# pygda-team/pygda

Measured on AMD Instinct MI355X. Metric: edges_aggregated_per_sec, higher is better.
Workload: dtype f32

## Files before the change

### include/gda_hip.h

```cpp
#ifndef GDA_HIP_H
#define GDA_HIP_H

#include <stddef.h>
#include <stdint.h>

#ifdef __cplusplus
extern "C" {
#endif

#define GDA_OK 0
#define GDA_E_NULL (-1)
#define GDA_E_SIZE (-2)
#define GDA_E_WORKSPACE (-3)
#define GDA_E_UNSUPPORTED (-4)
#define GDA_E_ALIAS (-5)
#define GDA_E_RCCL (-100)

typedef void* gda_stream_t;

int gda_abi_version(void);
const char* gda_status_string(int status);

size_t gda_graph_workspace_bytes(int64_t E, int64_t N);
int gda_build_csr_norm(const int64_t* src, const int64_t* dst, const float* w,
// ... 47 lines not shown

int gda_spmm_csr_interior_kstep_f32(const int32_t* rowptr, const int32_t* colidx, const float* val,
                                    int64_t n_rows, int64_t n_int, int64_t d, int K, int transposed,
                                    const float* x, float* y, float* tmp, float* sacc, const float* bias,
                                    gda_stream_t stream);

int gda_interior_max_rows(void);
int gda_interior_max_width(void);
size_t gda_interior_plan_bytes(void);
size_t gda_interior_kstep_lds_workspace_bytes(int64_t n_int, int64_t d);
int gda_interior_plan_build(const int32_t* rowptr, const int32_t* colidx, const float* val,
                            const int64_t* n_int_dev, void* plan, size_t plan_bytes, int64_t* status_dev,
                            gda_stream_t stream);
int gda_interior_kstep_lds_f32(const int32_t* rowptr, const int32_t* colidx, const float* val,
                               int64_t n_rows, int64_t n_int, int64_t d, int K, int transposed,
                               const void* plan, const float* x, float* y, const float* bias,
                               void* workspace, size_t workspace_bytes, gda_stream_t stream);
int gda_interior_kstep_lds_act_f32(const int32_t* rowptr, const int32_t* colidx, const float* val,
                                   int64_t n_rows, int64_t n_int, int64_t d, int K, const void* plan,
                                   const float* x, float* y0, float* y1, const float* bias,
                                   float p, uint64_t seed, const int64_t* step_dev, uint32_t site0, uint32_t site1,
                                   void* workspace, size_t workspace_bytes, gda_stream_t stream);

int gda_kstep_max_rows(void);
size_t gda_kstep_plan_bytes(int slots);
int gda_kstep_plan_host(const int32_t* rowptr_host, const int32_t* colidx_host, const float* val_host,
                        int64_t n_rows, void* plan_host, size_t plan_bytes);
int gda_kstep_plan_host_ex(const int32_t* rowptr_host, const int32_t* colidx_host, const float* val_host,
                           int64_t n_rows, int flags, void* plan_host, size_t plan_bytes);
int gda_kstep_lds_f32(const void* plan, int slots, int64_t n_rows, int64_t d, int K,
                      const float* x, int64_t ldx, int x_colmajor, float* y, int64_t ldy, int y_colmajor,
                      const float* bias, float* colsum, float* scratchT, gda_stream_t stream);
int gda_kstep_lds_colmajor_f32(const void* plan, int slots, int64_t n_rows, int64_t d, int K,
                               const float* xT, int64_t ldx, float* yT, int64_t ldy,
                               const float* bias, float* colsum, gda_stream_t stream);
int gda_transpose_f32(const float* in, int64_t ldi, float* out, int64_t ldo, int64_t rows, int64_t cols,
                      gda_stream_t stream);

int gda_gat_fwd_f32(const int32_t* rowptr, const int32_t* colidx, int64_t n_rows, int64_t d,
                    const float* h, const float* a_src, const float* a_dst, float slope,
                    float* out, float* alpha, gda_stream_t stream);
int gda_gat_bwd_f32(const int32_t* rowptr, const int32_t* colidx,
                    const int32_t* t_rowptr, const int32_t* t_colidx, const int32_t* t_to_fwd,
                    int64_t n_rows, int64_t d, const float* h, const float* a_src, const float* a_dst,
                    float slope, const float* alpha, const float* gout,
                    float* gh, float* ga_src, float* ga_dst, float* dpre, gda_stream_t stream);

int gda_faconv_fwd_f32(const int32_t* rowptr, const int32_t* colidx, const float* val, int64_t n_rows, int64_t d,
                       const float* h, int64_t ldh, const float* s, const float* r, int64_t ldsr, float eps,
                       const float* bias, float* out, int64_t ldo, float* t, gda_stream_t stream);
int gda_faconv_bwd_f32(const int32_t* rowptr, const int32_t* colidx, const float* val,
                       const int32_t* t_rowptr, const int32_t* t_colidx, const int32_t* t_to_fwd,
                       int64_t n_rows, int64_t d, const float* h, int64_t ldh, const float* t,
                       const float* gout, int64_t ldgo, float eps, float* gh, int64_t ldgh, float* gs,
                       float* gr, int64_t ldgsr, float* dpre, gda_stream_t stream);

size_t gda_closs_workspace_bytes(int64_t n, int64_t c);
int gda_closs_fwd_f32(const float* z, int64_t ldz, const int64_t* y, int64_t n, int64_t c, float* loss, float* weight,
                      float* factor, void* workspace, size_t workspace_bytes, gda_stream_t stream);
int gda_closs_bwd_f32(const float* z, int64_t ldz, const int64_t* y, const float* factor, const float* gloss,
                      int64_t n, int64_t c, float* gz, int64_t ldgz, gda_stream_t stream);
size_t gda_colstats_workspace_bytes(int64_t n, int64_t d);
int gda_weighted_moments_f32(const float* x, int64_t ldx, const float* w, int64_t n, int64_t d, float* mean,
                             float* std, void* workspace, size_t workspace_bytes, gda_stream_t stream);
int gda_std_mean_match_fwd_f32(const float* x, int64_t ldx, int64_t n, int64_t d, const float* mean_s,
                               const float* std_s, float* loss, float* mean_t, float* std_t, float* coef,
                               void* workspace, size_t workspace_bytes, gda_stream_t stream);
int gda_std_mean_match_bwd_f32(const float* x, int64_t ldx, int64_t n, int64_t d, const float* mean_t,
                               const float* coef, const float* gloss, float* gx, int64_t ldgx, gda_stream_t stream);

#define GDA_ACDNE_MAX_HALF 128
size_t gda_acdne_ppmi_workspace_bytes(int64_t n);
int gda_acdne_ppmi_f32(const int32_t* rowptr, const int32_t* col, const float* cnt, int64_t n, int step, float* pval,
                       float* buf_a, float* buf_b, float* buf_c, void* workspace, size_t workspace_bytes,
                       gda_stream_t stream);
int gda_acdne_xnei_f32(const float* na, int64_t n, int64_t ld, const int32_t* xrowptr, const int32_t* xcol,
                       const float* xval, int64_t f, float* out, int64_t ldo, gda_stream_t stream);
size_t gda_acdne_prox_workspace_bytes(int64_t h);
int gda_acdne_prox_f32(const float* ppmi_s, int64_t ld_s, int64_t ns, const float* ppmi_t, int64_t ld_t, int64_t nt,
                       const int64_t* pidx, const float* z, int64_t h, int64_t e, float pair_weight, double* loss,
                       float* gz, void* workspace, size_t workspace_bytes, gda_stream_t stream);
size_t gda_acdne_heads_workspace_bytes(int64_t h, int64_t e, int64_t c);
int gda_acdne_heads_f32(const float* z, const float* gprox, int64_t h, int64_t e, int64_t c, const float* const* w,
                        const int64_t* y, int64_t ny, const int64_t* rows, const float* alpha, const double* prox,
                        float pair_weight, float* dz, float* const* g, double* loss, double* loss_acc,
                        void* workspace, size_t workspace_bytes, gda_stream_t stream);
int gda_acdne_predict_f32(const float* z, int64_t n, int64_t e, const float* wc, const float* bc, int64_t c,
                          float* prob, gda_stream_t stream);

size_t gda_dmgnn_prox_workspace_bytes(int64_t h, int64_t e);
int gda_dmgnn_prox_f32(const float* ppmi_s, int64_t ld_s, int64_t ns, const float* ppmi_t, int64_t ld_t, int64_t nt,
                       const int64_t* pidx, const float* z, int64_t h, int64_t e, float pair_weight, double* loss,
                       float* gz, float* a_blocks, void* workspace, size_t workspace_bytes, gda_stream_t stream);
size_t gda_dmgnn_heads_workspace_bytes(int64_t h, int64_t e, int64_t c);
int gda_dmgnn_heads_f32(const float* z, const float* gprox, const float* a_blocks, int64_t h, int64_t e, int64_t c,
                        const float* const* w, const int64_t* y, int64_t ny, const int64_t* rows, const float* alpha,
                        const double* prox, float pair_weight, float* dz, float* const* g, double* loss,
                        double* loss_acc, void* workspace, size_t workspace_bytes, gda_stream_t stream);
size_t gda_dmgnn_predict_workspace_bytes(int64_t n, int64_t c);
int gda_dmgnn_predict_f32(const float* z, int64_t n, int64_t e, const float* wc, const float* bc, int64_t c,
                          const float* ppmi, int64_t ld, float* out, void* workspace, size_t workspace_bytes,
                          gda_stream_t stream);

size_t gda_mmd_workspace_bytes(int times, int64_t n, int64_t d);
int gda_mmd_fwd_f32(const float* src, int64_t ld_src, const float* tgt, int64_t ld_tgt,
                    int64_t d, const int64_t* src_idx, const int64_t* tgt_idx,
                    int times, int64_t n, float kernel_mul, int kernel_num, float fix_sigma,
                    float* loss, float* bandwidth, float* l2_saved,
                    void* workspace, size_t workspace_bytes, gda_stream_t stream);
int gda_mmd_bwd_f32(const float* src, int64_t ld_src, const float* tgt, int64_t ld_tgt,
                    int64_t d, const int64_t* src_idx, const int64_t* tgt_idx,
                    int times, int64_t n, float kernel_mul, int kernel_num,
                    const float* bandwidth, const float* l2_saved, const float* grad_loss,
                    float* grad_rows, void* workspace, size_t workspace_bytes, gda_stream_t stream);
int gda_mmd_fwd_ex_f32(const float* src, int64_t ld_src, const float* tgt, int64_t ld_tgt,
                       int64_t d, const int64_t* src_idx, const int64_t* tgt_idx,
                       int times, int64_t n, float kernel_mul, int kernel_num, float fix_sigma,
                       float scale, const float* add, float* loss, float* bandwidth, float* l2_saved,
                       void* workspace, size_t workspace_bytes, gda_stream_t stream);
int gda_mmd_fwd_gather_f32(const float* src, int64_t ld_src, const float* tgt, int64_t ld_tgt,
                           int64_t d, const int64_t* src_idx, const int64_t* tgt_idx,
                           int times, int64_t n, float kernel_mul, int kernel_num, float fix_sigma,
                           float scale, const float* add, float* rows_src, float* rows_tgt,
                           float* loss, float* bandwidth, float* l2_saved,
                           void* workspace, size_t workspace_bytes, gda_stream_t stream);
int gda_mmd_bwd_ex_f32(const float* src, int64_t ld_src, const float* tgt, int64_t ld_tgt,
                       int64_t d, const int64_t* src_idx, const int64_t* tgt_idx,
                       int times, int64_t n, float kernel_mul, int kernel_num,
                       const float* bandwidth, const float* l2_saved, const float* grad_loss, float scale,
                       float* grad_rows,
                       const int32_t* sel_s_rowptr, const int32_t* sel_s_col, int64_t n_src_rows, float* gsrc,
                       const int32_t* sel_t_rowptr, const int32_t* sel_t_col, int64_t n_tgt_rows, float* gtgt,
                       void* workspace, size_t workspace_bytes, gda_stream_t stream);

int gda_mmd_fused_nseg(int times, int64_t n, int64_t d, float kernel_mul, int kernel_num);
int gda_mmd_fused_layout(int times, int64_t n, int64_t d, int64_t* out, int n_out);
int gda_mmd_fused_fwd_f32(const float* src, int64_t ld_src, const float* tgt, int64_t ld_tgt,
                          int64_t d, const int64_t* src_idx, const int64_t* tgt_idx,
                          int times, int64_t n, float kernel_mul, int kernel_num, float fix_sigma,
                          float scale, const float* add, float* rows_src, float* rows_tgt,
                          float* loss, float* bandwidth, float* grad_part, int nseg,
                          void* workspace, size_t workspace_bytes, gda_stream_t stream);
int gda_mmd_fused_bwd_f32(const float* grad_part, int nseg, int times, int64_t n, int64_t d,
                          const float* grad_loss, float scale, float* grad_rows,
                          const int32_t* sel_s_rowptr, const int32_t* sel_s_col, int64_t n_src_rows, float* gsrc,
                          const int32_t* sel_t_rowptr, const int32_t* sel_t_col, int64_t n_tgt_rows, float* gtgt,
                          gda_stream_t stream);
int gda_mmd_fused_bwd_mask_f32(const float* grad_part, int nseg, int times, int64_t n, int64_t d,
                               const float* grad_loss, float scale, float* grad_rows,
                               const int32_t* sel_s_rowptr, const int32_t* sel_s_col, int64_t n_src_rows, float* gsrc,
                               const int32_t* sel_t_rowptr, const int32_t* sel_t_col, int64_t n_tgt_rows, float* gtgt,
                               const float* mask_src, float p_src, const float* mask_tgt, float p_tgt,
                               gda_stream_t stream);

int gda_mmd_chunked_plan(int times, int64_t n, int64_t d, float kernel_mul, int kernel_num, int64_t* out, int n_out);
size_t gda_mmd_chunked_workspace_bytes(int times, int64_t n, int64_t d);
int gda_mmd_chunked_fwd_f32(const float* src, int64_t ld_src, const float* tgt, int64_t ld_tgt,
                            int64_t d, const int64_t* src_idx, const int64_t* tgt_idx,
                            int times, int64_t n, float kernel_mul, int kernel_num, float fix_sigma,
                            float scale, const float* add, float* rows_src, float* rows_tgt, int64_t ld_rows,
                            float* loss, float* bandwidth, float* grad_part, int64_t ld_part, int nseg,
                            void* workspace, size_t workspace_bytes, gda_stream_t stream);
int gda_mmd_fused_bwd_ld_f32(const float* grad_part, int64_t ld_part, int nseg, int times, int64_t n, int64_t d,
                             const float* grad_loss, float scale, float* grad_rows,
                             const int32_t* sel_s_rowptr, const int32_t* sel_s_col, int64_t n_src_rows, float* gsrc,
                             const int32_t* sel_t_rowptr, const int32_t* sel_t_col, int64_t n_tgt_rows, float* gtgt,
                             const float* mask_src, float p_src, const float* mask_tgt, float p_tgt,
                             gda_stream_t stream);

int gda_grl_disc_ce_fwd_f32(const float* feat_src, int64_t ld_src, int64_t n_src,
                            const float* feat_tgt, int64_t ld_tgt, int64_t n_tgt,
                            int64_t h, int C, const float* W, const float* b,
                            const int64_t* labels, float* probs, float* loss,
                            void* workspace, size_t workspace_bytes, gda_stream_t stream);
int gda_grl_disc_ce_bwd_f32(const float* feat_src, int64_t ld_src, int64_t n_src,
                            const float* feat_tgt, int64_t ld_tgt, int64_t n_tgt,
                            int64_t h, int C, const float* W, const int64_t* labels,
                            const float* probs, const float* grad_loss, float alpha,
                            float* gfeat_src, float* gfeat_tgt, float* gW, float* gb,
                            void* workspace, size_t workspace_bytes, gda_stream_t stream);
size_t gda_grl_disc_workspace_bytes(int64_t n_rows, int64_t h, int C);

size_t gda_grl_mlp_ce_workspace_bytes(int64_t h, int64_t a);
int gda_grl_mlp_ce_fwd_f32(const float* es, int64_t ld_s, int64_t n_s, const float* et, int64_t ld_t, int64_t n_t,
                           int64_t h, int64_t a, const float* W1, const float* b1, const float* W2, const float* b2,
                           float dropout_p, uint64_t seed, const int64_t* step, uint32_t site,
                           float* losses, void* workspace, size_t workspace_bytes, gda_stream_t stream);
int gda_grl_mlp_ce_bwd_f32(const float* es, int64_t ld_s, int64_t n_s, const float* et, int64_t ld_t, int64_t n_t,
                           int64_t h, int64_t a, const float* W1, const float* b1, const float* W2, const float* b2,
                           float dropout_p, uint64_t seed, const int64_t* step, uint32_t site,
                           const float* grad_losses, int grad_stride, float alpha, const float* alpha_dev,
                           float* g_es, float* g_et, float* gW1, float* gb1, float* gW2, float* gb2,
                           void* workspace, size_t workspace_bytes, gda_stream_t stream);
int gda_mlp_head_fwd_f32(int head, const float* es, int64_t ld_s, int64_t n_s, const float* et, int64_t ld_t, int64_t n_t,
                         int64_t h, int64_t a, const float* W1, const float* b1, const float* W2, const float* b2,
                         float dropout_p, uint64_t seed, const int64_t* step, uint32_t site,
                         float* losses, void* workspace, size_t workspace_bytes, gda_stream_t stream);
int gda_mlp_head_bwd_f32(int head, const float* es, int64_t ld_s, int64_t n_s, const float* et, int64_t ld_t, int64_t n_t,
                         int64_t h, int64_t a, const float* W1, const float* b1, const float* W2, const float* b2,
                         float dropout_p, uint64_t seed, const int64_t* step, uint32_t site,
                         const float* grad_losses, int grad_stride, float alpha, const float* alpha_dev,
                         float* g_es, float* g_et, float* gW1, float* gb1, float* gW2, float* gb2,
                         void* workspace, size_t workspace_bytes, gda_stream_t stream);

size_t gda_lsgan_head_workspace_bytes(int64_t a);
int gda_lsgan_head_fwd_f32(const float* Z, int64_t ldz, int64_t rows, int64_t a, const float* w2, const float* b2,
                           float target, float* pre, float* loss, void* workspace, size_t workspace_bytes,
                           gda_stream_t stream);
int gda_lsgan_head_bwd_f32(const float* Z, int64_t ldz, int64_t rows, int64_t a, const float* w2, const float* pre,
                           float target, const float* grad_loss, float* gZ, int64_t ldg, float* gw2, float* gb2,
                           void* workspace, size_t workspace_bytes, gda_stream_t stream);

size_t gda_wgan_critic_workspace_bytes(int64_t n_s, int64_t n_t, int64_t n_i, int h, int a);
int gda_wgan_critic_f32(const float* es, int64_t n_s, const float* et, int64_t n_t, int h,
                        const int32_t* idx_s, const int32_t* idx_t, const float* alpha, int64_t n_i,
                        const float* W1, const float* b1, const float* w2, const float* b2, int a,
                        float dropout_p, uint64_t seed, const int64_t* step, uint32_t site,
                        float gp_weight, float* loss, float* gW1, float* gb1, float* gw2, float* gb2,
                        void* workspace, size_t workspace_bytes, gda_stream_t stream);

int gda_relu_dropout_fwd_f32(const float* x, float* y, int64_t n, float p, uint64_t seed,
                             const int64_t* step, uint32_t site, gda_stream_t stream);
int gda_relu_dropout_bwd_f32(const float* gy, const float* y, float* gx, int64_t n, float p,
                             gda_stream_t stream);
int gda_relu_dropout_tiled_fwd_f32(const float* x, int64_t period, int64_t copies, float* y, float p, uint64_t seed,
                                   const int64_t* step, uint32_t site, gda_stream_t stream);
int gda_relu_dropout_fwd_cm_f32(const float* xT, int64_t ldT, float* y, int64_t n, int64_t d, float p,
                               uint64_t seed, const int64_t* step, uint32_t site, gda_stream_t stream);
int gda_relu_dropout_bwd_cm_f32(const float* gy, const float* y, float* gxT, int64_t ldT, int64_t n, int64_t d,
                               float p, gda_stream_t stream);

int gda_relu_dropout_pair_fwd_f32(const float* x, float* y, int64_t n, int64_t d, float p, uint64_t seed,
                                  const int64_t* step, uint32_t site_a, uint32_t site_b, gda_stream_t stream);
size_t gda_relu_dropout_pair_workspace_bytes(int64_t d);
int gda_relu_dropout_pair_bwd_f32(const float* gy, const float* y, float* gx, int64_t n, int64_t d, float p,
                                  float* colsum, void* workspace, size_t workspace_bytes, gda_stream_t stream);
int gda_stack2_f32(const float* a, const float* b, float* out, int64_t half_elems, gda_stream_t stream);
int gda_relu_dropout_bwd2_f32(const float* ga, const float* gb, const float* y, float* gx, int64_t half_elems,
                              float p, gda_stream_t stream);

size_t gda_colsum_workspace_bytes(int64_t n, int64_t d);
int gda_colsum_f32(const float* x, int64_t ldx, int64_t n, int64_t d, float* out, void* workspace,
                   size_t workspace_bytes, gda_stream_t stream);

size_t gda_mixup_combine_workspace_bytes(int64_t n, int64_t h);
int gda_mixup_combine_fwd_f32(const float* P, const float* Pb, const float* CC, int first, const float* bias,
                              const int64_t* perm, int64_t n, int64_t h, float lam, float p, uint64_t seed,
                              const int64_t* step, uint32_t site_x, uint32_t site_m, float* XX, uint8_t* mask,
                              gda_stream_t stream);
int gda_mixup_combine_bwd_f32(const float* gXX, const float* XX, const uint8_t* mask, const int64_t* inv_perm,
                              int first, int64_t n, int64_t h, float lam, float p, float* gP, float* gPb,
                              float* gCC, float* gbias, void* workspace, size_t workspace_bytes,
                              gda_stream_t stream);

int gda_gather_rows_f32(const float* x, int64_t ldx, int64_t d, const int64_t* idx,
                        int64_t n_out, float* out, int64_t ldo, gda_stream_t stream);

int gda_segment_mean_fwd_f32(const float* x, int64_t ldx, const int64_t* seg_ptr, int64_t G, int64_t d,
                             float* out, int64_t ldo, gda_stream_t stream);
int gda_segment_mean_bwd_f32(const float* gout, int64_t ldg, const int64_t* seg_ptr, const int64_t* batch,
                             int64_t n, int64_t d, float* gx, int64_t ldx, gda_stream_t stream);

typedef struct gda_sampler gda_sampler;
int gda_sampler_create(const int64_t* src_host, const int64_t* dst_host, int64_t E, int64_t N,
                       gda_sampler** out);
void gda_sampler_destroy(gda_sampler* s);
int gda_sampler_set_threads(gda_sampler* s, int workers);
int gda_sampler_sample(gda_sampler* s, const int64_t* seeds_host, int64_t n_seeds,
                       const int32_t* fanouts, int L, uint64_t rng_seed,
                       int64_t* n_nodes_out, int64_t* n_edges_out);
int gda_sampler_fetch(const gda_sampler* s, int64_t* nodes_out, int64_t* esrc_out,
                      int64_t* edst_out);
int gda_sampler_csr_norm(const gda_sampler* s, int32_t* rowptr, int32_t* colidx, float* val,
                         int32_t* t_rowptr, int32_t* t_colidx, float* t_val);

size_t gda_dsampler_graph_workspace_bytes(int64_t E, int64_t N);
int gda_dsampler_build_graph(const int64_t* src, const int64_t* dst, int64_t E, int64_t N,
                             int64_t* in_ptr, int32_t* in_src, int32_t* status,
                             void* workspace, size_t workspace_bytes, gda_stream_t stream);
int gda_dsampler_caps(int64_t n_seeds, const int32_t* fanouts_host, int L, int64_t max_in_degree, int64_t E,
                      int64_t N, int64_t* node_cap, int64_t* edge_cap);
size_t gda_dsampler_workspace_bytes(int64_t n_seeds, const int32_t* fanouts_host, int L, int64_t max_in_degree,
                                    int64_t E, int64_t N);
int gda_dsampler_sample(const int64_t* in_ptr, const int32_t* in_src, int64_t N, int64_t E, int64_t max_in_degree,
                        const int64_t* seeds, int64_t n_seeds, const int32_t* fanouts_host, int L, uint64_t rng_seed,
                        int64_t* nodes, int64_t* esrc, int64_t* edst,
                        int32_t* rowptr, int32_t* colidx, float* val,
                        int32_t* t_rowptr, int32_t* t_colidx, float* t_val,
                        int64_t* counts, void* workspace, size_t workspace_bytes, gda_stream_t stream);

int gda_copy_from_pinned(void* dst, const void* src_host, size_t bytes, gda_stream_t stream);

int gda_event_create(void** event_out);
int gda_event_destroy(void* event);
int gda_event_record(void* event, gda_stream_t stream);
int gda_event_synchronize(void* event);
int gda_stream_wait_event(gda_stream_t stream, void* event);
int gda_dsampler_batch(const int64_t* in_ptr, const int32_t* in_src, int64_t N, int64_t E, int64_t max_in_degree,
                       const int64_t* seeds, int64_t n_seeds, int64_t* seeds_dev,
                       const int32_t* fanouts_host, int L, uint64_t rng_seed,
                       int64_t* nodes, int64_t* esrc, int64_t* edst,
                       int32_t* rowptr, int32_t* colidx, float* val,
                       int32_t* t_rowptr, int32_t* t_colidx, float* t_val,
                       int64_t* counts, void* plan_fwd, void* plan_bwd, size_t plan_bytes,
                       int64_t* counts_host, void* wait_event, void* done_event,
                       void* workspace, size_t workspace_bytes, gda_stream_t stream);
// ... 301 lines not shown
```

### pygda_amd/_lib.py

```python
import ctypes
import os
from ctypes import c_char_p, c_float, c_int, c_int64, c_size_t, c_void_p

import torch

HERE = os.path.dirname(os.path.abspath(__file__))
LIB_PATH = os.path.join(HERE, "libgda_hip.so")

class _P(c_void_p):

    @classmethod
    def from_param(cls, obj):
        if isinstance(obj, torch.Tensor):
            return c_void_p(obj.data_ptr())
        if obj is None:
            return None
        if isinstance(obj, str):
            raise TypeError("a str is not a pointer argument")
        return c_void_p.from_param(obj)


_SIGNATURES = {
    "gda_abi_version": (c_int, []),
    "gda_status_string": (c_char_p, [c_int]),
    "gda_graph_workspace_bytes": (c_size_t, [c_int64, c_int64]),
    "gda_build_csr_norm": (c_int, [_P, _P, _P, c_int64, c_int64, c_float, c_int, c_int, c_int,
                                   _P, _P, _P, _P, _P, _P, _P, c_size_t, _P]),
    "gda_build_csr_norm_map": (c_int, [_P, _P, _P, c_int64, c_int64, c_float, c_int, c_int, c_int,
                                       _P, _P, _P, _P, _P, _P, _P, _P, c_size_t, _P]),
    "gda_gat_fwd_f32": (c_int, [_P, _P, c_int64, c_int64, _P, _P, _P, c_float, _P, _P, _P]),
    "gda_gat_bwd_f32": (c_int, [_P, _P, _P, _P, _P, c_int64, c_int64, _P, _P, _P, c_float, _P, _P,
                                _P, _P, _P, _P, _P]),
    "gda_faconv_fwd_f32": (c_int, [_P, _P, _P, c_int64, c_int64, _P, c_int64, _P, _P, c_int64, c_float, _P, _P,
                                   c_int64, _P, _P]),
    "gda_faconv_bwd_f32": (c_int, [_P, _P, _P, _P, _P, _P, c_int64, c_int64, _P, c_int64, _P, _P, c_int64, c_float,
                                   _P, c_int64, _P, _P, c_int64, _P, _P]),
    "gda_closs_workspace_bytes": (c_size_t, [c_int64, c_int64]),
    "gda_closs_fwd_f32": (c_int, [_P, c_int64, _P, c_int64, c_int64, _P, _P, _P, _P, c_size_t, _P]),
    "gda_closs_bwd_f32": (c_int, [_P, c_int64, _P, _P, _P, c_int64, c_int64, _P, c_int64, _P]),
    "gda_colstats_workspace_bytes": (c_size_t, [c_int64, c_int64]),
    "gda_weighted_moments_f32": (c_int, [_P, c_int64, _P, c_int64, c_int64, _P, _P, _P, c_size_t, _P]),
    "gda_std_mean_match_fwd_f32": (c_int, [_P, c_int64, c_int64, c_int64, _P, _P, _P, _P, _P, _P, _P, c_size_t, _P]),
    "gda_std_mean_match_bwd_f32": (c_int, [_P, c_int64, c_int64, c_int64, _P, _P, _P, _P, c_int64, _P]),
    "gda_acdne_ppmi_workspace_bytes": (c_size_t, [c_int64]),
    "gda_acdne_ppmi_f32": (c_int, [_P, _P, _P, c_int64, c_int, _P, _P, _P, _P, _P, c_size_t, _P]),
    "gda_acdne_xnei_f32": (c_int, [_P, c_int64, c_int64, _P, _P, _P, c_int64, _P, c_int64, _P]),
    "gda_acdne_prox_workspace_bytes": (c_size_t, [c_int64]),
    "gda_acdne_prox_f32": (c_int, [_P, c_int64, c_int64, _P, c_int64, c_int64, _P, _P, c_int64, c_int64, c_float, _P, _P,
                                   _P, c_size_t, _P]),
    "gda_acdne_heads_workspace_bytes": (c_size_t, [c_int64, c_int64, c_int64]),
    "gda_acdne_heads_f32": (c_int, [_P, _P, c_int64, c_int64, c_int64, _P, _P, c_int64, _P, _P, _P, c_float, _P, _P, _P,
                                    _P, _P, c_size_t, _P]),
    "gda_acdne_predict_f32": (c_int, [_P, c_int64, c_int64, _P, _P, c_int64, _P, _P]),
    "gda_dmgnn_prox_workspace_bytes": (c_size_t, [c_int64, c_int64]),
    "gda_dmgnn_prox_f32": (c_int, [_P, c_int64, c_int64, _P, c_int64, c_int64, _P, _P, c_int64, c_int64, c_float, _P, _P,
                                   _P, _P, c_size_t, _P]),
    "gda_dmgnn_heads_workspace_bytes": (c_size_t, [c_int64, c_int64, c_int64]),
    "gda_dmgnn_heads_f32": (c_int, [_P, _P, _P, c_int64, c_int64, c_int64, _P, _P, c_int64, _P, _P, _P, c_float, _P, _P,
                                    _P, _P, _P, c_size_t, _P]),
    "gda_dmgnn_predict_workspace_bytes": (c_size_t, [c_int64, c_int64]),
    "gda_dmgnn_predict_f32": (c_int, [_P, c_int64, c_int64, _P, _P, c_int64, _P, c_int64, _P, _P, c_size_t, _P]),
    "gda_asn_recon_chunks": (c_int, [c_int64]),
    "gda_asn_recon_workspace_bytes": (c_size_t, [c_int64, c_int64]),
    "gda_asn_recon_f32": (c_int, [_P, c_int64, c_int64, c_int64, _P, _P, _P, _P, _P, _P, c_float, c_float, _P, _P,
                                  c_int64, _P, c_size_t, _P]),
    "gda_asn_rows_workspace_bytes": (c_size_t, [c_int64, c_int64, c_int64]),
    "gda_asn_kld_f32": (c_int, [_P, c_int64, _P, c_int64, c_int64, c_int64, ctypes.c_double, _P, _P, _P, _P, c_size_t,
                                _P]),
    "gda_asn_reparam_fwd_f32": (c_int, [_P, c_int64, _P, c_int64, c_int64, c_int64, _P, c_int, ctypes.c_uint64, _P,
                                        ctypes.c_uint32, _P, _P]),
    "gda_asn_reparam_bwd_f32": (c_int, [_P, _P, _P, c_int64, c_int64, c_int64, _P, _P]),
    "gda_asn_dropout_fwd_f32": (c_int, [_P, c_int64, c_float, ctypes.c_uint64, _P, ctypes.c_uint32, _P, _P, _P]),
    "gda_asn_mask_mul_f32": (c_int, [_P, _P, c_int64, _P, _P]),
    "gda_asn_diff_fwd_f32": (c_int, [_P, c_int64, _P, c_int64, c_int64, c_int64, c_int64, _P, _P, _P, c_size_t, _P]),
    "gda_asn_diff_bwd_f32": (c_int, [_P, c_int64, _P, c_int64, c_int64, c_int64, c_int64, _P, _P, _P, _P, _P]),
    "gda_asn_ppmi_count": (c_int, [_P, c_int64, c_int64, _P, _P]),
    "gda_asn_ppmi_fill": (c_int, [_P, c_int64, c_int64, _P, c_int64, _P, _P, _P, _P, _P]),
    "gda_jhgda_prox_workspace_bytes": (c_size_t, [c_int64, c_int64]),
    "gda_jhgda_prox_f32": (c_int, [_P, c_int64, c_int64, c_int64, _P, _P, _P, _P, _P, c_int64, _P, _P, c_int64, _P,
                                   c_int64, _P, c_size_t, _P]),
    "gda_jhgda_pool_rows_fwd_f32": (c_int, [_P, c_int64, c_int64, c_int64, _P, c_int64, _P, _P, _P]),
    "gda_jhgda_pool_rows_bwd_f32": (c_int, [_P, c_int64, _P, c_int64, _P, c_int64, _P, c_int64, c_int64, _P, c_int64,
                                            _P]),
    "gda_csr_to_coo": (c_int, [_P, _P, c_int64, c_int64, _P, _P, _P]),
    "gda_spmm_csr_f32": (c_int, [_P, _P, _P, c_int64, c_int64, _P, c_int64, _P, c_int64, _P, _P]),
    "gda_spmm_csr_tout_f32": (c_int, [_P, _P, _P, c_int64, c_int64, _P, c_int64, _P, c_int64, _P, _P]),
    "gda_spmm_csr_kstep_f32": (c_int, [_P, _P, _P, c_int64, c_int64, c_int, _P, c_int64, _P, c_int64,
                                       _P, _P, _P]),
    "gda_spmm_csr_interior_kstep_f32": (c_int, [_P, _P, _P, c_int64, c_int64, c_int64, c_int, c_int, _P, _P, _P, _P, _P, _P]),
    "gda_interior_max_rows": (c_int, []),
    "gda_interior_max_width": (c_int, []),
    "gda_interior_plan_bytes": (c_size_t, []),
    "gda_interior_kstep_lds_workspace_bytes": (c_size_t, [c_int64, c_int64]),
    "gda_interior_plan_build": (c_int, [_P, _P, _P, _P, _P, c_size_t, _P, _P]),
    "gda_interior_kstep_lds_f32": (c_int, [_P, _P, _P, c_int64, c_int64, c_int64, c_int, c_int, _P, _P, _P, _P, _P,
                                           c_size_t, _P]),
    "gda_interior_kstep_lds_act_f32": (c_int, [_P, _P, _P, c_int64, c_int64, c_int64, c_int, _P, _P, _P, _P, _P,
                                               ctypes.c_float, ctypes.c_uint64, _P, ctypes.c_uint32, ctypes.c_uint32,
                                               _P, c_size_t, _P]),
    "gda_row_split_workspace_bytes": (c_size_t, [c_int64]),
    "gda_row_split_build": (c_int, [_P, c_int64, ctypes.c_int32, _P, _P, _P, _P, _P, c_size_t, _P]),
    "gda_spmm_csr_split_f32": (c_int, [_P, _P, _P, c_int64, c_int64, c_int, _P, c_int64, _P, c_int64,
                                       _P, _P, _P, _P]),
    "gda_mmd_workspace_bytes": (c_size_t, [c_int, c_int64, c_int64]),
    "gda_mmd_fwd_f32": (c_int, [_P, c_int64, _P, c_int64, c_int64, _P, _P, c_int, c_int64, c_float,
                                c_int, c_float, _P, _P, _P, _P, c_size_t, _P]),
    "gda_mmd_bwd_f32": (c_int, [_P, c_int64, _P, c_int64, c_int64, _P, _P, c_int, c_int64, c_float,
                                c_int, _P, _P, _P, _P, _P, c_size_t, _P]),
    "gda_mmd_fwd_ex_f32": (c_int, [_P, c_int64, _P, c_int64, c_int64, _P, _P, c_int, c_int64, c_float, c_int, c_float,
                                   c_float, _P, _P, _P, _P, _P, c_size_t, _P]),
    "gda_mmd_fwd_gather_f32": (c_int, [_P, c_int64, _P, c_int64, c_int64, _P, _P, c_int, c_int64, c_float, c_int, c_float,
                                       c_float, _P, _P, _P, _P, _P, _P, _P, c_size_t, _P]),
    "gda_mmd_bwd_ex_f32": (c_int, [_P, c_int64, _P, c_int64, c_int64, _P, _P, c_int, c_int64, c_float, c_int,
                                   _P, _P, _P, c_float, _P, _P, _P, c_int64, _P, _P, _P, c_int64, _P,
                                   _P, c_size_t, _P]),
    "gda_mmd_fused_nseg": (c_int, [c_int, c_int64, c_int64, c_float, c_int]),
    "gda_mmd_fused_layout": (c_int, [c_int, c_int64, c_int64, _P, c_int]),
    "gda_mmd_fused_fwd_f32": (c_int, [_P, c_int64, _P, c_int64, c_int64, _P, _P, c_int, c_int64, c_float, c_int, c_float,
                                      c_float, _P, _P, _P, _P, _P, _P, c_int, _P, c_size_t, _P]),
    "gda_mmd_fused_bwd_f32": (c_int, [_P, c_int, c_int, c_int64, c_int64, _P, c_float, _P,
                                      _P, _P, c_int64, _P, _P, _P, c_int64, _P, _P]),
    "gda_mmd_fused_bwd_mask_f32": (c_int, [_P, c_int, c_int, c_int64, c_int64, _P, c_float, _P,
                                           _P, _P, c_int64, _P, _P, _P, c_int64, _P, _P, c_float, _P, c_float, _P]),
    "gda_copy_from_pinned": (c_int, [_P, _P, c_size_t, _P]),
    "gda_softmax_entropy_fwd_f32": (c_int, [_P, c_int64, c_int64, c_int, c_float, _P, _P, c_size_t, _P]),
    "gda_softmax_entropy_bwd_f32": (c_int, [_P, c_int64, c_int64, c_int, c_float, _P, _P, c_int64, _P]),
    "gda_mmd_chunked_plan": (c_int, [c_int, c_int64, c_int64, c_float, c_int, _P, c_int]),
    "gda_mmd_chunked_workspace_bytes": (c_size_t, [c_int, c_int64, c_int64]),
    "gda_mmd_chunked_fwd_f32": (c_int, [_P, c_int64, _P, c_int64, c_int64, _P, _P, c_int, c_int64, c_float, c_int, c_float,
                                        c_float, _P, _P, _P, c_int64, _P, _P, _P, c_int64, c_int, _P, c_size_t, _P]),
    "gda_mmd_fused_bwd_ld_f32": (c_int, [_P, c_int64, c_int, c_int, c_int64, c_int64, _P, c_float, _P,
                                         _P, _P, c_int64, _P, _P, _P, c_int64, _P, _P, c_float, _P, c_float, _P]),
    "gda_gemm_tall_fwd_ex_f32": (c_int, [c_int64, c_int64, c_int64, _P, c_int64, _P, _P, c_int64, _P, c_int64, _P, c_int,
                                         c_float, ctypes.c_uint64, _P, ctypes.c_uint32, ctypes.c_uint32, _P]),
    "gda_gemm_tall_wgrad_gather_f32": (c_int, [c_int64, c_int64, _P, c_int64, _P, c_int64, _P, _P, c_int64, _P, _P, c_size_t, _P]),
    "gda_gemm_nn_mask_f32": (c_int, [c_int64, c_int64, c_int64, _P, c_int64, _P, c_int64, _P, c_int64, _P, c_int64, c_float, _P]),
    "gda_gemm_act_cm_f32": (c_int, [c_int64, c_int64, c_int64, _P, c_int64, _P, c_int64, _P, _P, c_int64, c_float,
                                    ctypes.c_uint64, _P, ctypes.c_uint32, _P]),
    "gda_gemm_act_cm_bwd_f32": (c_int, [c_int64, c_int64, c_int64, _P, c_int64, _P, c_int64, _P, c_float, _P, _P, _P, c_size_t,
                                        _P]),
    "gda_gemm_skinny_act_cm_f32": (c_int, [c_int64, c_int64, c_int64, _P, c_int64, _P, c_int64, _P, c_int64, c_float,
                                           ctypes.c_uint64, _P, ctypes.c_uint32, _P]),
    "gda_grl_disc_workspace_bytes": (c_size_t, [c_int64, c_int64, c_int]),
    "gda_grl_mlp_ce_workspace_bytes": (c_size_t, [c_int64, c_int64]),
    "gda_lsgan_head_workspace_bytes": (c_size_t, [c_int64]),
    "gda_lsgan_head_fwd_f32": (c_int, [_P, c_int64, c_int64, c_int64, _P, _P, c_float, _P, _P, _P, c_size_t, _P]),
    "gda_lsgan_head_bwd_f32": (c_int, [_P, c_int64, c_int64, c_int64, _P, _P, c_float, _P, _P, c_int64, _P, _P,
                                       _P, c_size_t, _P]),
    "gda_grl_mlp_ce_fwd_f32": (c_int, [_P, c_int64, c_int64, _P, c_int64, c_int64, c_int64, c_int64, _P, _P, _P, _P,
                                       c_float, ctypes.c_uint64, _P, ctypes.c_uint32, _P, _P, c_size_t, _P]),
    "gda_grl_mlp_ce_bwd_f32": (c_int, [_P, c_int64, c_int64, _P, c_int64, c_int64, c_int64, c_int64, _P, _P, _P, _P,
                                       c_float, ctypes.c_uint64, _P, ctypes.c_uint32, _P, c_int, c_float, _P,
                                       _P, _P, _P, _P, _P, _P, _P, c_size_t, _P]),
    "gda_mlp_head_fwd_f32": (c_int, [c_int, _P, c_int64, c_int64, _P, c_int64, c_int64, c_int64, c_int64, _P, _P, _P, _P,
                                     c_float, ctypes.c_uint64, _P, ctypes.c_uint32, _P, _P, c_size_t, _P]),
    "gda_mlp_head_bwd_f32": (c_int, [c_int, _P, c_int64, c_int64, _P, c_int64, c_int64, c_int64, c_int64, _P, _P, _P, _P,
                                     c_float, ctypes.c_uint64, _P, ctypes.c_uint32, _P, c_int, c_float, _P,
                                     _P, _P, _P, _P, _P, _P, _P, c_size_t, _P]),
    "gda_grl_disc_ce_fwd_f32": (c_int, [_P, c_int64, c_int64, _P, c_int64, c_int64, c_int64, c_int,
                                        _P, _P, _P, _P, _P, _P, c_size_t, _P]),
    "gda_grl_disc_ce_bwd_f32": (c_int, [_P, c_int64, c_int64, _P, c_int64, c_int64, c_int64, c_int,
                                        _P, _P, _P, _P, c_float, _P, _P, _P, _P, _P, c_size_t, _P]),
    "gda_relu_dropout_fwd_f32": (c_int, [_P, _P, c_int64, c_float, ctypes.c_uint64, _P, ctypes.c_uint32, _P]),
    "gda_relu_dropout_bwd_f32": (c_int, [_P, _P, _P, c_int64, c_float, _P]),
    "gda_relu_dropout_tiled_fwd_f32": (c_int, [_P, c_int64, c_int64, _P, c_float, ctypes.c_uint64, _P, ctypes.c_uint32, _P]),
    "gda_gather_rows_f32": (c_int, [_P, c_int64, c_int64, _P, c_int64, _P, c_int64, _P]),
    "gda_segment_mean_fwd_f32": (c_int, [_P, c_int64, _P, c_int64, c_int64, _P, c_int64, _P]),
    "gda_segment_mean_bwd_f32": (c_int, [_P, c_int64, _P, _P, c_int64, c_int64, _P, c_int64, _P]),
    "gda_sampler_create": (c_int, [_P, _P, c_int64, c_int64, ctypes.POINTER(c_void_p)]),
    "gda_sampler_destroy": (None, [_P]),
    "gda_sampler_set_threads": (c_int, [_P, c_int]),
    "gda_sampler_sample": (c_int, [_P, _P, c_int64, _P, c_int, ctypes.c_uint64,
                                   ctypes.POINTER(c_int64), ctypes.POINTER(c_int64)]),
    "gda_sampler_fetch": (c_int, [_P, _P, _P, _P]),
    "gda_sampler_csr_norm": (c_int, [_P, _P, _P, _P, _P, _P, _P]),
    "gda_dsampler_graph_workspace_bytes": (c_size_t, [c_int64, c_int64]),
    "gda_dsampler_build_graph": (c_int, [_P, _P, c_int64, c_int64, _P, _P, _P, _P, c_size_t, _P]),
    "gda_dsampler_caps": (c_int, [c_int64, _P, c_int, c_int64, c_int64, c_int64, _P, _P]),
    "gda_dsampler_workspace_bytes": (c_size_t, [c_int64, _P, c_int, c_int64, c_int64, c_int64]),
    "gda_dsampler_sample": (c_int, [_P, _P, c_int64, c_int64, c_int64, _P, c_int64, _P, c_int, ctypes.c_uint64,
                                    _P, _P, _P, _P, _P, _P, _P, _P, _P, _P, _P, c_size_t, _P]),
    "gda_event_create": (c_int, [_P]),
    "gda_event_destroy": (c_int, [_P]),
    "gda_event_record": (c_int, [_P, _P]),
    "gda_event_synchronize": (c_int, [_P]),
    "gda_stream_wait_event": (c_int, [_P, _P]),
    "gda_dsampler_batch": (c_int, [_P, _P, c_int64, c_int64, c_int64, _P, c_int64, _P, _P, c_int, ctypes.c_uint64,
                                   _P, _P, _P, _P, _P, _P, _P, _P, _P, _P, _P, _P, c_size_t, _P, _P, _P, _P, c_size_t, _P]),
    "gda_dsampler_batch_ex": (c_int, [_P, _P, c_int64, c_int64, c_int64, _P, c_int64, _P, _P, c_int, ctypes.c_uint64,
                                      _P, _P, _P, _P, _P, _P, _P, _P, _P, _P, _P, _P, c_size_t, _P, _P, _P, c_int64, _P,
                                      c_size_t, _P]),
    "gda_selection_csr_host": (c_int, [_P, c_int, c_int64, c_int64, c_int64, c_int64, _P, _P]),
    "gda_ppmi_build_host": (c_int, [_P, _P, c_int64, c_int64, c_int, c_int, ctypes.c_uint64,
                                    ctypes.POINTER(c_void_p)]),
    "gda_ppmi_workspace_bytes": (c_size_t, [c_int64, c_int64, c_int, c_int]),
    "gda_ppmi_build": (c_int, [_P, _P, c_int64, c_int64, c_int, c_int, ctypes.c_uint64, _P, _P, _P, _P, _P,
                               c_size_t, _P]),
    "gda_edge_list_size": (c_int64, [_P]),
    "gda_edge_list_fetch": (c_int, [_P, _P, _P, _P]),
    "gda_edge_list_destroy": (None, [_P]),
    "gda_spmm_csr_axpby_f32": (c_int, [_P, _P, _P, c_int64, c_int64, _P, c_int64, _P, c_int64, c_float, c_float,
                                       _P, c_int64, c_float, _P, _P, _P]),
    "gda_kstep_max_rows": (c_int, []),
    "gda_kstep_plan_bytes": (c_size_t, [c_int]),
    "gda_kstep_plan_host": (c_int, [_P, _P, _P, c_int64, _P, c_size_t]),
    "gda_kstep_plan_host_ex": (c_int, [_P, _P, _P, c_int64, c_int, _P, c_size_t]),
    "gda_kstep_lds_f32": (c_int, [_P, c_int, c_int64, c_int64, c_int, _P, c_int64, c_int, _P, c_int64, c_int,
                                  _P, _P, _P, _P]),
    "gda_kstep_lds_colmajor_f32": (c_int, [_P, c_int, c_int64, c_int64, c_int, _P, c_int64, _P, c_int64, _P, _P, _P]),
    "gda_relu_dropout_pair_fwd_f32": (c_int, [_P, _P, c_int64, c_int64, c_float, ctypes.c_uint64, _P, ctypes.c_uint32,
                                              ctypes.c_uint32, _P]),
    "gda_relu_dropout_pair_workspace_bytes": (ctypes.c_size_t, [c_int64]),
    "gda_relu_dropout_pair_bwd_f32": (c_int, [_P, _P, _P, c_int64, c_int64, c_float, _P, _P, ctypes.c_size_t, _P]),
    "gda_stack2_f32": (c_int, [_P, _P, _P, c_int64, _P]),
    "gda_relu_dropout_bwd2_f32": (c_int, [_P, _P, _P, _P, c_int64, ctypes.c_float, _P]),
    "gda_colsum_workspace_bytes": (ctypes.c_size_t, [c_int64, c_int64]),
    "gda_colsum_f32": (c_int, [_P, c_int64, c_int64, c_int64, _P, _P, ctypes.c_size_t, _P]),
    "gda_softmax_nll_fwd_ex_f32": (c_int, [_P, c_int64, _P, c_int64, c_int, _P, _P, _P, ctypes.c_size_t, _P]),
    "gda_mixup_combine_workspace_bytes": (ctypes.c_size_t, [c_int64, c_int64]),
    "gda_mixup_combine_fwd_f32": (c_int, [_P, _P, _P, c_int, _P, _P, c_int64, c_int64, c_float, c_float, ctypes.c_uint64,
                                          _P, ctypes.c_uint32, ctypes.c_uint32, _P, _P, _P]),
    "gda_mixup_combine_bwd_f32": (c_int, [_P, _P, _P, _P, c_int, c_int64, c_int64, c_float, c_float, _P, _P, _P, _P, _P,
                                          ctypes.c_size_t, _P]),
    "gda_relu_dropout_fwd_cm_f32": (c_int, [_P, c_int64, _P, c_int64, c_int64, c_float, ctypes.c_uint64, _P,
                                           ctypes.c_uint32, _P]),
    "gda_relu_dropout_bwd_cm_f32": (c_int, [_P, _P, _P, c_int64, c_int64, c_int64, c_float, _P]),
    "gda_transpose_f32": (c_int, [_P, c_int64, _P, c_int64, c_int64, c_int64, _P]),
    "gda_wgan_critic_workspace_bytes": (c_size_t, [c_int64, c_int64, c_int64, c_int, c_int]),
    "gda_wgan_critic_f32": (c_int, [_P, c_int64, _P, c_int64, c_int, _P, _P, _P, c_int64, _P, _P, _P, _P, c_int,
                                    c_float, ctypes.c_uint64, _P, ctypes.c_uint32, c_float, _P, _P, _P, _P, _P,
                                    _P, c_size_t, _P]),
    "gda_wgan_critic_adam_f32": (c_int, [_P, c_int64, _P, c_int64, c_int, _P, _P, _P, c_int64, c_int,
                                         c_float, ctypes.c_uint64, _P, ctypes.c_uint32, c_float, _P, _P,
                                         c_float, c_float, c_float, c_float, c_float, _P, c_size_t, _P]),
    "gda_laplacian_workspace_bytes": (c_size_t, [c_int64]),
    "gda_laplacian_fwd_f32": (c_int, [_P, _P, c_int64, c_int, _P, c_int64, _P, _P, _P, c_size_t, _P]),
    "gda_laplacian_bwd_f32": (c_int, [_P, _P, _P, _P, c_int64, c_int, _P, c_int64, _P, _P, _P, c_int64, _P]),
    "gda_softmax_nll_workspace_bytes": (c_size_t, []),
    "gda_softmax_nll_fwd_f32": (c_int, [_P, c_int64, _P, c_int64, c_int, _P, _P, c_size_t, _P]),
    "gda_softmax_nll_bwd_f32": (c_int, [_P, c_int64, _P, c_int64, c_int, _P, _P, c_int64, _P]),
    "gda_softmax_nll_fwd_nv_f32": (c_int, [_P, c_int64, _P, c_int64, c_int, _P, _P, _P, _P, c_size_t, _P]),
    "gda_softmax_nll_bwd_nv_f32": (c_int, [_P, c_int64, _P, c_int64, c_int, _P, _P, _P, c_int64, _P]),
    "gda_gemm_workspace_bytes": (c_size_t, [c_int, c_int64, c_int64, c_int64]),
    "gda_gemm_f32": (c_int, [c_int, c_int64, c_int64, c_int64, _P, c_int64, _P, c_int64, _P, c_int64,
                             _P, c_size_t, _P]),
    "gda_gemm_ex_f32": (c_int, [c_int, c_int64, c_int64, c_int64, _P, c_int64, _P, c_int64, _P, c_int64, _P, _P,
                                _P, c_size_t, _P]),
    "gda_gemm_skinny_workspace_bytes": (c_size_t, [c_int, c_int64, c_int64, c_int64]),
    "gda_gemm_skinny_f32": (c_int, [c_int, c_int64, c_int64, c_int64, _P, c_int64, _P, c_int64, _P, c_int64, _P, _P,
                                    _P, c_size_t, _P]),
    "gda_gemm_tall_workspace_bytes": (c_size_t, [c_int, c_int64, c_int64, c_int64]),
    "gda_gemm_tall_f32": (c_int, [c_int, c_int64, c_int64, c_int64, _P, c_int64, _P, c_int64, _P, c_int64, _P, _P,
                                  _P, c_size_t, _P]),
    "gda_attention_workspace_bytes": (c_size_t, [c_int64, c_int64]),
    "gda_attention_fuse_fwd_f32": (c_int, [c_int, _P, _P, c_int64, c_int64, _P, _P, _P, c_int64, _P, _P]),
    "gda_attention_fuse_bwd_f32": (c_int, [c_int, _P, _P, c_int64, c_int64, _P, _P, _P, c_int64, _P, _P, _P, _P, c_size_t, _P]),
    "gda_adam_multi_f32": (c_int, [_P, c_int, c_float, c_float, c_float, c_float, c_float, _P]),
    "gda_adam_multi_ex_f32": (c_int, [_P, c_int, c_float, c_float, c_float, c_float, c_float, c_int, _P]),
    "gda_adam_multi_sum_f32": (c_int, [_P, _P, c_int, c_float, c_float, c_float, c_float, c_float, c_int, _P]),
    "gda_step_bump": (c_int, [_P, _P, c_int, _P]),
    "gda_rccl_load": (c_int, [ctypes.c_char_p]),
    "gda_comm_unique_id": (c_int, [_P, c_size_t]),
    "gda_comm_init_rank": (c_int, [_P, c_size_t, c_int, c_int, ctypes.POINTER(c_void_p)]),
    "gda_comm_destroy": (c_int, [_P]),
    "gda_allreduce_f32": (c_int, [_P, c_int64, _P, _P]),
    "gda_allgather_f32": (c_int, [_P, _P, c_int64, _P, _P]),
    "gda_two_hop_host": (c_int, [_P, _P, c_int64, c_int64, c_int, c_int, ctypes.POINTER(c_void_p)]),
    "gda_sepa_workspace_bytes": (c_size_t, [c_int64, c_int64, c_int64]),
    "gda_sepa_stats_f32": (c_int, [_P, c_int64, c_int64, _P, _P, _P, _P]),
    "gda_sepa_group_sum_f32": (c_int, [_P, c_int64, _P, _P, c_int64, c_int64, c_int64, c_int, c_float, _P, _P, _P, _P,
                                       c_size_t, _P]),
    "gda_sepa_class_mean_bwd_f32": (c_int, [_P, _P, _P, _P, c_int64, c_int64, c_int64, c_float, _P, _P]),
    "gda_sepa_mid_f32": (c_int, [_P, _P, _P, _P, c_int64, c_int64, c_int64, _P, _P, _P, _P]),
    "gda_sepa_unbias_rows_f32": (c_int, [_P, _P, _P, _P, c_int64, c_int64, c_int64, _P, _P]),
    "gda_sepa_row_weight_f32": (c_int, [_P, _P, c_int64, c_int64, _P, _P]),
    "gda_sepa_center_rows_bwd_f32": (c_int, [_P, _P, _P, _P, _P, _P, c_int64, c_int64, c_int64, _P, _P, _P]),
# ... 138 lines not shown
```

### pygda_amd/csrc/gda_act.hip

```cpp
#include "gda_common.h"
#include "gda_dropout.h"

namespace {

constexpr int TB = 256;

__global__ void __launch_bounds__(TB)
k_relu_dropout_fwd(const float* __restrict__ x, float* __restrict__ y, int64_t n, float p, float scale,
                   uint64_t seed, const int64_t* __restrict__ step, uint32_t site, int64_t period) {
    const uint64_t st = (uint64_t)step[0];
    const uint32_t thresh = dropout_thresh(p);
    const int64_t quads = (n + 3) / 4;
    for (int64_t q = (int64_t)blockIdx.x * TB + threadIdx.x; q < quads; q += (int64_t)gridDim.x * TB) {
        uint32_t r[4];
        dropout_draw(seed, st, site, (uint64_t)q, r);
        const int64_t i = q * 4;
        if (period) {
            const float4 v = *reinterpret_cast<const float4*>(x + i % period);
            *reinterpret_cast<float4*>(y + i) = relu_keep(v, r, thresh, scale);
        } else if (i + 3 < n) {
            const float4 v = *reinterpret_cast<const float4*>(x + i);
            *reinterpret_cast<float4*>(y + i) = relu_keep(v, r, thresh, scale);
        } else {
            for (int e = 0; e < 4 && i + e < n; ++e)
// ... 256 lines not shown
            const float v0 = x[i * ldx + tc], v1 = x[(i + stride) * ldx + tc];
            const float v2 = x[(i + 2 * stride) * ldx + tc], v3 = x[(i + 3 * stride) * ldx + tc];
            const float v4 = x[(i + 4 * stride) * ldx + tc], v5 = x[(i + 5 * stride) * ldx + tc];
            const float v6 = x[(i + 6 * stride) * ldx + tc], v7 = x[(i + 7 * stride) * ldx + tc];
            a0 += v0; a1 += v1; a2 += v2; a3 += v3;
            a0 += v4; a1 += v5; a2 += v6; a3 += v7;
        }
        for (; i < n; i += stride) a0 += x[i * ldx + tc];
        red[tr * d + tc] = (a0 + a1) + (a2 + a3);
    }
    __syncthreads();
    for (int w = slots >> 1; w > 0; w >>= 1) {
        if (tr < w) red[tr * d + tc] += red[(tr + w) * d + tc];
        __syncthreads();
    }
    if (tr == 0) out[tc] = red[tc];
}

int colsum_blocks(int64_t n, int d) {
    const int rpb = d <= TB ? TB / d : 1;
    const int64_t g = gda_cdiv(n, (int64_t)rpb * 8);
    return (int)(g > COLSUM_BLOCKS ? COLSUM_BLOCKS : (g < 1 ? 1 : g));
}

unsigned grid_for(int64_t n) {
    int64_t g = gda_cdiv((n + 3) / 4, TB);
    if (g > 256 * 8) g = 256 * 8;
    return (unsigned)(g < 1 ? 1 : g);
}

}

extern "C" int gda_relu_dropout_fwd_f32(const float* x, float* y, int64_t n, float p, uint64_t seed,
                                        const int64_t* step, uint32_t site, gda_stream_t stream) {
    if (n < 0 || !(p >= 0.f && p < 1.f)) return GDA_E_SIZE;
    if (n == 0) return GDA_OK;
    if (!x || !y || !step) return GDA_E_NULL;
    if (((uintptr_t)x | (uintptr_t)y) % 16 != 0) return GDA_E_UNSUPPORTED;
    k_relu_dropout_fwd<<<grid_for(n), TB, 0, (hipStream_t)stream>>>(x, y, n, p, 1.f / (1.f - p), seed, step, site, 0);
    GDA_LAUNCH_CHECK();
    return GDA_OK;
}

extern "C" int gda_relu_dropout_tiled_fwd_f32(const float* x, int64_t period, int64_t copies, float* y, float p, uint64_t seed,
                                              const int64_t* step, uint32_t site, gda_stream_t stream) {
    if (period < 0 || copies < 0 || !(p >= 0.f && p < 1.f) || period % 4 != 0) return GDA_E_SIZE;
    if (period == 0 || copies == 0) return GDA_OK;
    if (!x || !y || !step) return GDA_E_NULL;
    if (((uintptr_t)x | (uintptr_t)y) % 16 != 0) return GDA_E_UNSUPPORTED;
    const int64_t n = period * copies;
    k_relu_dropout_fwd<<<grid_for(n), TB, 0, (hipStream_t)stream>>>(x, y, n, p, 1.f / (1.f - p), seed, step, site, period);
    GDA_LAUNCH_CHECK();
    return GDA_OK;
}

extern "C" int gda_relu_dropout_bwd_f32(const float* gy, const float* y, float* gx, int64_t n, float p,
                                        gda_stream_t stream) {
    if (n < 0 || !(p >= 0.f && p < 1.f)) return GDA_E_SIZE;
    if (n == 0) return GDA_OK;
    if (!gy || !y || !gx) return GDA_E_NULL;
    if (((uintptr_t)gy | (uintptr_t)y | (uintptr_t)gx) % 16 != 0) return GDA_E_UNSUPPORTED;
    k_relu_dropout_bwd<<<grid_for(n), TB, 0, (hipStream_t)stream>>>(gy, y, gx, n, 1.f / (1.f - p));
    GDA_LAUNCH_CHECK();
    return GDA_OK;
}

extern "C" int gda_relu_dropout_fwd_cm_f32(const float* xT, int64_t ldT, float* y, int64_t n, int64_t d, float p,
                                          uint64_t seed, const int64_t* step, uint32_t site, gda_stream_t stream) {
    if (n < 0 || d < 0 || n >= INT32_MAX || d >= INT32_MAX || ldT < n || !(p >= 0.f && p < 1.f)) return GDA_E_SIZE;
    if (n == 0 || d == 0) return GDA_OK;
    if (!xT || !y || !step) return GDA_E_NULL;
    if (d % 4 != 0 || (uintptr_t)y % 16 != 0) return GDA_E_UNSUPPORTED;
    const dim3 grid((unsigned)gda_cdiv(n, TT), (unsigned)gda_cdiv(d, TT));
    if (grid.y > 65535) return GDA_E_SIZE;
    GDA_UNLESS_SKIPPED("k_relu_dropout_fwd_T") k_relu_dropout_fwd_T<<<grid, TB, 0, (hipStream_t)stream>>>(xT, ldT, y, (int)n, (int)d, p, 1.f / (1.f - p), seed,
                                                               step, site);
    GDA_LAUNCH_CHECK();
    return GDA_OK;
}

extern "C" int gda_relu_dropout_bwd_cm_f32(const float* gy, const float* y, float* gxT, int64_t ldT, int64_t n,
                                          int64_t d, float p, gda_stream_t stream) {
    if (n < 0 || d < 0 || n >= INT32_MAX || d >= INT32_MAX || ldT < n || !(p >= 0.f && p < 1.f)) return GDA_E_SIZE;
    if (n == 0 || d == 0) return GDA_OK;
    if (!gy || !y || !gxT) return GDA_E_NULL;
    if (d % 4 != 0 || ((uintptr_t)gy | (uintptr_t)y) % 16 != 0) return GDA_E_UNSUPPORTED;
    const dim3 grid((unsigned)gda_cdiv(n, TT), (unsigned)gda_cdiv(d, TT));
    if (grid.y > 65535) return GDA_E_SIZE;
    GDA_UNLESS_SKIPPED("k_relu_dropout_bwd_T") k_relu_dropout_bwd_T<<<grid, TB, 0, (hipStream_t)stream>>>(gy, y, gxT, ldT, (int)n, (int)d, 1.f / (1.f - p));
    GDA_LAUNCH_CHECK();
    return GDA_OK;
}

extern "C" int gda_relu_dropout_pair_fwd_f32(const float* x, float* y, int64_t n, int64_t d, float p, uint64_t seed,
                                             const int64_t* step, uint32_t site_a, uint32_t site_b,
                                             gda_stream_t stream) {
    if (n < 0 || d < 0 || !(p >= 0.f && p < 1.f)) return GDA_E_SIZE;
    if (n == 0 || d == 0) return GDA_OK;
    if (!x || !y || (p > 0.f && !step)) return GDA_E_NULL;
    if (d % 4 != 0 || ((uintptr_t)x | (uintptr_t)y) % 16 != 0) return GDA_E_UNSUPPORTED;
    k_relu_dropout_pair_fwd<<<grid_for(n * d), TB, 0, (hipStream_t)stream>>>(x, y, n * d, p, 1.f / (1.f - p), seed, step,
                                                                           site_a, site_b);
    GDA_LAUNCH_CHECK();
    return GDA_OK;
}

extern "C" size_t gda_relu_dropout_pair_workspace_bytes(int64_t d) {
    return d > 0 ? (size_t)PAIR_BLOCKS * (size_t)d * sizeof(float) : 0;
}

extern "C" int gda_relu_dropout_pair_bwd_f32(const float* gy, const float* y, float* gx, int64_t n, int64_t d, float p,
                                             float* colsum, void* workspace, size_t workspace_bytes,
                                             gda_stream_t stream) {
    if (n < 0 || d < 0 || !(p >= 0.f && p < 1.f)) return GDA_E_SIZE;
    if (n == 0 || d == 0) return GDA_OK;
    if (!gy || !y || !gx) return GDA_E_NULL;
    if (d % 4 != 0 || ((uintptr_t)gy | (uintptr_t)y | (uintptr_t)gx) % 16 != 0) return GDA_E_UNSUPPORTED;
    hipStream_t s = (hipStream_t)stream;
    if (!colsum) {
        k_relu_dropout_pair_bwd<<<grid_for(n * d), TB, 0, s>>>(gy, y, gx, n * d, 1.f / (1.f - p));
        GDA_LAUNCH_CHECK();
        return GDA_OK;
    }
    if (d > 4 * TB) return GDA_E_UNSUPPORTED;
    if (!workspace) return GDA_E_NULL;
    if (workspace_bytes < gda_relu_dropout_pair_workspace_bytes(d) || (uintptr_t)workspace % 16 != 0) return GDA_E_WORKSPACE;
    const int rpb = TB / (int)(d >> 2);
    const int64_t want = gda_cdiv(n, rpb);
    const int blocks = (int)(want > PAIR_BLOCKS ? PAIR_BLOCKS : want);
    float* partial = static_cast<float*>(workspace);
    k_relu_dropout_pair_bwd_colsum<<<blocks, TB, 0, s>>>(gy, y, gx, n, (int)d, 1.f / (1.f - p), partial);
    GDA_LAUNCH_CHECK();
    GDA_UNLESS_SKIPPED("k_colsum_final") k_colsum_final<<<(unsigned)gda_cdiv(d, CF_COLS), TB, 0, s>>>(partial, blocks, (int)d, colsum);
    GDA_LAUNCH_CHECK();
    return GDA_OK;
}

extern "C" int gda_stack2_f32(const float* a, const float* b, float* out, int64_t half_elems, gda_stream_t stream) {
    if (half_elems < 0) return GDA_E_SIZE;
    if (half_elems == 0) return GDA_OK;
    if (!out) return GDA_E_NULL;
    if (half_elems % 4 != 0 || ((uintptr_t)a | (uintptr_t)b | (uintptr_t)out) % 16 != 0) return GDA_E_UNSUPPORTED;
    GDA_UNLESS_SKIPPED("k_stack2") k_stack2<<<grid_for(2 * half_elems), TB, 0, (hipStream_t)stream>>>(a, b, out, half_elems);
    GDA_LAUNCH_CHECK();
    return GDA_OK;
}

extern "C" int gda_relu_dropout_bwd2_f32(const float* ga, const float* gb, const float* y, float* gx, int64_t half_elems,
                                         float p, gda_stream_t stream) {
    if (half_elems < 0 || !(p >= 0.f && p < 1.f)) return GDA_E_SIZE;
    if (half_elems == 0) return GDA_OK;
    if (!y || !gx) return GDA_E_NULL;
    if (half_elems % 4 != 0 || ((uintptr_t)ga | (uintptr_t)gb | (uintptr_t)y | (uintptr_t)gx) % 16 != 0) return GDA_E_UNSUPPORTED;
    k_relu_dropout_bwd2<<<grid_for(2 * half_elems), TB, 0, (hipStream_t)stream>>>(ga, gb, y, gx, half_elems, 1.f / (1.f - p));
    GDA_LAUNCH_CHECK();
    return GDA_OK;
}

extern "C" size_t gda_colsum_workspace_bytes(int64_t n, int64_t d) {
    if (n <= 0 || d <= 0 || d > COLSUM_MAXD) return 0;
    return (size_t)colsum_blocks(n, (int)d) * (size_t)d * sizeof(float);
}

extern "C" int gda_colsum_f32(const float* x, int64_t ldx, int64_t n, int64_t d, float* out, void* workspace,
                              size_t workspace_bytes, gda_stream_t stream) {
    if (n < 0 || d < 0 || ldx < d) return GDA_E_SIZE;
    if (d == 0) return GDA_OK;
    if (d > COLSUM_MAXD) return GDA_E_UNSUPPORTED;
    if (!out) return GDA_E_NULL;
    hipStream_t s = (hipStream_t)stream;
    if (n == 0) {
        GDA_HIP_TRY(hipMemsetAsync(out, 0, (size_t)d * sizeof(float), s));
        return GDA_OK;
    }
    if (!x) return GDA_E_NULL;
    if (d <= CO_MAX_D && n * d <= CO_MAX_ELEMS) {
        int slots = 1;
        while (slots * 2 * (int)d <= CO_TB) slots *= 2;
        k_colsum_one<<<1, CO_TB, 0, s>>>(x, ldx, n, (int)d, slots, out);
        GDA_LAUNCH_CHECK();
        return GDA_OK;
    }
    if (!workspace) return GDA_E_NULL;
    if (workspace_bytes < gda_colsum_workspace_bytes(n, d)) return GDA_E_WORKSPACE;
    const int blocks = colsum_blocks(n, (int)d);
    k_colsum_partial<<<blocks, TB, 0, s>>>(x, ldx, n, (int)d, static_cast<float*>(workspace));
    GDA_LAUNCH_CHECK();
    GDA_UNLESS_SKIPPED("k_colsum_final") k_colsum_final<<<(unsigned)gda_cdiv(d, CF_COLS), TB, 0, s>>>(static_cast<const float*>(workspace), blocks, (int)d, out);
    GDA_LAUNCH_CHECK();
    return GDA_OK;
}
```

### pygda_amd/csrc/gda_mmd.hip

```cpp
#include "gda_common.h"
#include "gda_dropout.h"

#include <cstdlib>

namespace {

constexpr int TB = 256;
constexpr int TILE = 64;
constexpr int DK = 32;
constexpr int LDT = TILE + 1;
constexpr int DC = 128;
constexpr int MAXQ = 8;

struct Rows {
    const float* src; int64_t ld_src;
    const float* tgt; int64_t ld_tgt;
    const int64_t* src_idx; const int64_t* tgt_idx;
    int64_t n;
    bool vec4;
};

__device__ __forceinline__ const float* row_ptr(const Rows& R, int t, int64_t r) {
    if (r < R.n) {
        const int64_t g = R.src_idx ? R.src_idx[(int64_t)t * R.n + r] : (int64_t)t * R.n + r;
// ... 512 lines not shown
#pragma unroll
        for (int half = 0; half < 2; ++half)
#pragma unroll
            for (int r = 0; r < 16; ++r) {
                const int64_t i = i0 + wr + (r & 3) + 8 * (r >> 2) + 4 * ka;
                tiv[half][r] = row_direct(R, t, i < m ? i : m - 1)[c0 + wc + 32 * half + la];
            }
#pragma unroll
        for (int half = 0; half < 2; ++half)
#pragma unroll
            for (int r = 0; r < 16; ++r) {
                const int il = wr + (r & 3) + 8 * (r >> 2) + 4 * ka;
                const int64_t i = i0 + il;
                const float ti = tiv[half][r] - (half == 0 ? pv0 : pv1);
                const float a = half == 0 ? acc0[r] : acc1[r];
                if (i < m) out[i * d + c0 + wc + 32 * half + la] = coef * fmaf(rowsum[il], ti, -a);
            }
        return;
    }
#pragma unroll
    for (int half = 0; half < 2; ++half) {
        const int64_t c = c0 + wc + 32 * half + la;
#pragma unroll
        for (int r = 0; r < 16; ++r) {
            const int il = wr + (r & 3) + 8 * (r >> 2) + 4 * ka;
            const int64_t i = i0 + il;
            if (i < m && c < d) {
                const float ti = row_ptr(R, t, i)[c] - pivot[c];
                const float a = half == 0 ? acc0[r] : acc1[r];
                out[i * d + c] = coef * fmaf(rowsum[il], ti, -a);
            }
        }
    }
}

__global__ void __launch_bounds__(TB)
k_bwd_reduce_ld(const float* __restrict__ part, int64_t m, int64_t d, int64_t ldp, int nseg, int times,
                float* __restrict__ grad_rows, const float* __restrict__ grad_loss, float cmul) {
    const float c4 = grad_loss ? 4.f * (grad_loss[0] * cmul) : 4.f;
    const int64_t total = m * d * times;
    for (int64_t k = (int64_t)blockIdx.x * TB + threadIdx.x; k < total; k += (int64_t)gridDim.x * TB) {
        const int64_t t = k / (m * d), r = k % (m * d), i = r / d, c = r % d;
        float s = 0.f;
        for (int g = 0; g < nseg; ++g) s += part[((t * nseg + g) * m + i) * ldp + c];
        grad_rows[k] = c4 * s;
    }
}

__global__ void __launch_bounds__(TB)
k_bwd_reduce(const float* __restrict__ part, int64_t per_t, int nseg, int times,
             float* __restrict__ grad_rows, const float* __restrict__ grad_loss, float cmul) {
    const float c4 = grad_loss ? 4.f * (grad_loss[0] * cmul) : 4.f;
    const int64_t total = per_t * times;
    for (int64_t k = (int64_t)blockIdx.x * TB + threadIdx.x; k < total; k += (int64_t)gridDim.x * TB) {
        const int64_t t = k / per_t, r = k % per_t;
        float s = 0.f;
        for (int g = 0; g < nseg; ++g) s += part[(t * nseg + g) * per_t + r];
        grad_rows[k] = c4 * s;
    }
}

template <int NSEG>
__global__ void __launch_bounds__(TB)
k_bwd_scatter(const float* __restrict__ part, int64_t m, int64_t d, int64_t ldp, bool vec_out, int nseg_rt,
              const int32_t* __restrict__ s_rowptr, const int32_t* __restrict__ s_col, int64_t n_src_rows,
              float* __restrict__ gsrc, const int32_t* __restrict__ t_rowptr, const int32_t* __restrict__ t_col,
              int64_t n_tgt_rows, float* __restrict__ gtgt, const float* __restrict__ grad_loss, float cmul,
              const float* __restrict__ mask_s = nullptr, float mscale_s = 1.f,
              const float* __restrict__ mask_t = nullptr, float mscale_t = 1.f) {
    const float c4 = grad_loss ? 4.f * (grad_loss[0] * cmul) : 4.f;
    const int nseg = NSEG > 0 ? NSEG : nseg_rt;
    const int64_t rows_per_block = TB / 32;
    const int lane = threadIdx.x % 32;
    const int64_t r = (int64_t)blockIdx.x * rows_per_block + threadIdx.x / 32;
    const bool tgt = blockIdx.y == 1;
    const int64_t n_rows = tgt ? n_tgt_rows : n_src_rows;
    if (r >= n_rows) return;
    const int32_t* rp = tgt ? t_rowptr : s_rowptr;
    const int32_t* ci = tgt ? t_col : s_col;
    float* out = (tgt ? gtgt : gsrc) + r * d;
    const float* mk = tgt ? mask_t : mask_s;
    const float msc = tgt ? mscale_t : mscale_s;
    if (mk) mk += r * d;
    const int32_t b = rp[r], e = rp[r + 1];
    if constexpr (NSEG > 0) {
        const int mi = (int)m;
        for (int64_t c = (int64_t)lane * 4; c < d; c += 128) {
            float4 acc = make_float4(0.f, 0.f, 0.f, 0.f);
            int32_t pn = b < e ? ci[b] : 0;
            for (int32_t k = b; k < e; ++k) {
                const int p = pn;
                if (k + 1 < e) pn = ci[k + 1];
                const int t = p / mi, i = p - t * mi;
                const float* q = part + (((int64_t)t * NSEG) * m + i) * ldp + c;
                float4 v[NSEG];
#pragma unroll
                for (int g = 0; g < NSEG; ++g) v[g] = *reinterpret_cast<const float4*>(q + (int64_t)g * m * ldp);
                float4 sg = make_float4(0.f, 0.f, 0.f, 0.f);
#pragma unroll
                for (int g = 0; g < NSEG; ++g) { sg.x += v[g].x; sg.y += v[g].y; sg.z += v[g].z; sg.w += v[g].w; }
                acc.x = __fadd_rn(acc.x, c4 * sg.x); acc.y = __fadd_rn(acc.y, c4 * sg.y);
                acc.z = __fadd_rn(acc.z, c4 * sg.z); acc.w = __fadd_rn(acc.w, c4 * sg.w);
            }
            if (!vec_out) {
                const float a4[4] = {acc.x, acc.y, acc.z, acc.w};
#pragma unroll
                for (int v2 = 0; v2 < 4; ++v2)
                    if (c + v2 < d) out[c + v2] = mk ? (mk[c + v2] > 0.f ? a4[v2] * msc : 0.f) : a4[v2];
                continue;
            }
            if (mk) {
                acc = relu_keep_bwd(*reinterpret_cast<const float4*>(mk + c), acc, msc);
            }
            *reinterpret_cast<float4*>(out + c) = acc;
        }
        return;
    }
    for (int64_t c = (int64_t)lane * 4; c < d; c += 128) {
        float acc[4] = {0.f, 0.f, 0.f, 0.f};
        for (int32_t k = b; k < e; ++k) {
            const int64_t p = ci[k], t = p / m, i = p % m;
            float sg[4] = {0.f, 0.f, 0.f, 0.f};
            for (int g = 0; g < nseg; ++g) {
                const float* q = part + (((int64_t)t * nseg + g) * m + i) * ldp + c;
#pragma unroll
                for (int v = 0; v < 4; ++v) if (c + v < d) sg[v] += q[v];
            }
#pragma unroll
            for (int v = 0; v < 4; ++v) acc[v] = __fadd_rn(acc[v], __fmul_rn(1.0f, c4 * sg[v]));
        }
#pragma unroll
        for (int v = 0; v < 4; ++v) if (c + v < d) out[c + v] = mk ? (mk[c + v] > 0.f ? acc[v] * msc : 0.f) : acc[v];
    }
}

constexpr int BWD_NSEG = 4;
constexpr int BWD_NSEG_MAX = 8;

struct BwdVariant { int tile, nseg; };
BwdVariant bwd_variant(int64_t m) { return m >= 512 ? BwdVariant{128, 6} : BwdVariant{64, BWD_NSEG}; }

template <bool FAST, int BI_>
int launch_bwd(dim3 grid, hipStream_t stream, Rows R, int64_t d, int64_t m, const float* l2, const float* grad_loss, float scale,
               int times, int nseg, float* part) {
    const size_t lds = sizeof(float) * (2 * BJ * (BI_ + DC) + BI_);
    GDA_LDS_ATTR_ONCE((k_bwd<FAST, BI_>), lds);
    k_bwd<FAST, BI_><<<grid, BI_ * 4, lds, stream>>>(R, d, m, l2, grad_loss, scale, times, nseg, part);
    GDA_LAUNCH_CHECK();
    return GDA_OK;
}

#include "gda_mmd_fused.inc"
#include "gda_mmd_chunked.inc"

struct MmdWs {
    double* kpartial; double* part_s1; float* part_col; float* bwd_part; float* norms;
    float* part_max; unsigned char* images;
    size_t total;
};

MmdWs carve(void* base, int times, int64_t n, int64_t d) {
    const int64_t m = 2 * n, nt = gda_cdiv(m, TILE);
    MmdWs w{};
    size_t off = 0;
    auto take = [&](size_t bytes) {
        void* p = base ? (void*)((char*)base + off) : nullptr;
        off += gda_align_up(bytes, 256);
        return p;
    };
    const int64_t chunks = gda_cdiv(m, SR);
    FusedPlan fp;
    const bool fused = fused_plan(times, n, d, 2.0f, 5, &fp);
    const int64_t per_t = fused && (int64_t)fp.njb * fp.nseg > nt * nt ? (int64_t)fp.njb * fp.nseg : nt * nt;
    w.kpartial = (double*)take(sizeof(double) * times * per_t);
    w.part_s1 = (double*)take(sizeof(double) * times * chunks);
    w.part_col = (float*)take(sizeof(float) * times * chunks * (d > 0 ? d : 1));
    w.bwd_part = (float*)take(sizeof(float) * times * BWD_NSEG_MAX * m * (d > 0 ? d : 1));
    w.norms = (float*)take(sizeof(float) * times * m);
    if (fused) {
        w.part_max = (float*)take(sizeof(float) * times * chunks);
        w.images = (unsigned char*)take((size_t)times * fp.ntiles * fp.img);
    }
    w.total = off;
    return w;
}

int check_common(const float* src, int64_t ld_src, const float* tgt, int64_t ld_tgt, int64_t d,
                 const int64_t* src_idx, const int64_t* tgt_idx, int times, int64_t n, int kernel_num) {
    if (!src || !tgt) return GDA_E_NULL;
    if (d <= 0 || n <= 0 || times <= 0 || ld_src < d || ld_tgt < d) return GDA_E_SIZE;
    if (2 * n >= 46340 * 2) return GDA_E_SIZE;
    if (kernel_num < 1 || kernel_num > MAXQ) return GDA_E_UNSUPPORTED;
    if ((src_idx == nullptr) != (tgt_idx == nullptr)) return GDA_E_NULL;
    return GDA_OK;
}

Rows make_rows(const float* src, int64_t ld_src, const float* tgt, int64_t ld_tgt,
               const int64_t* src_idx, const int64_t* tgt_idx, int64_t n) {
    Rows R{src, ld_src, tgt, ld_tgt, src_idx, tgt_idx, n, false};
    R.vec4 = (ld_src % 4 == 0) && (ld_tgt % 4 == 0) && ((uintptr_t)src % 16 == 0) && ((uintptr_t)tgt % 16 == 0);
    return R;
}

}

extern "C" size_t gda_mmd_workspace_bytes(int times, int64_t n, int64_t d) {
    if (times <= 0 || n <= 0 || d <= 0) return 0;
    return carve(nullptr, times, n, d).total;
}

extern "C" int gda_mmd_fwd_f32(const float* src, int64_t ld_src, const float* tgt, int64_t ld_tgt,
                               int64_t d, const int64_t* src_idx, const int64_t* tgt_idx,
                               int times, int64_t n, float kernel_mul, int kernel_num, float fix_sigma,
                               float* loss, float* bandwidth, float* l2_saved,
                               void* workspace, size_t workspace_bytes, gda_stream_t stream_) {
    return gda_mmd_fwd_ex_f32(src, ld_src, tgt, ld_tgt, d, src_idx, tgt_idx, times, n, kernel_mul, kernel_num, fix_sigma,
                              1.0f, nullptr, loss, bandwidth, l2_saved, workspace, workspace_bytes, stream_);
}

extern "C" int gda_mmd_fwd_ex_f32(const float* src, int64_t ld_src, const float* tgt, int64_t ld_tgt,
                                  int64_t d, const int64_t* src_idx, const int64_t* tgt_idx,
                                  int times, int64_t n, float kernel_mul, int kernel_num, float fix_sigma,
                                  float scale, const float* add, float* loss, float* bandwidth, float* l2_saved,
                                  void* workspace, size_t workspace_bytes, gda_stream_t stream_) {
    return gda_mmd_fwd_gather_f32(src, ld_src, tgt, ld_tgt, d, src_idx, tgt_idx, times, n, kernel_mul, kernel_num,
                                  fix_sigma, scale, add, nullptr, nullptr, loss, bandwidth, l2_saved, workspace,
                                  workspace_bytes, stream_);
}

extern "C" int gda_mmd_fwd_gather_f32(const float* src, int64_t ld_src, const float* tgt, int64_t ld_tgt,
                                      int64_t d, const int64_t* src_idx, const int64_t* tgt_idx,
                                      int times, int64_t n, float kernel_mul, int kernel_num, float fix_sigma,
                                      float scale, const float* add, float* rows_src, float* rows_tgt,
                                      float* loss, float* bandwidth, float* l2_saved,
                                      void* workspace, size_t workspace_bytes, gda_stream_t stream_) {
    int st = check_common(src, ld_src, tgt, ld_tgt, d, src_idx, tgt_idx, times, n, kernel_num);
    if (st != GDA_OK) return st;
    if (!loss || !bandwidth || !l2_saved || !workspace) return GDA_E_NULL;
    if ((rows_src == nullptr) != (rows_tgt == nullptr) || (rows_src && !src_idx)) return GDA_E_NULL;
    if (rows_src && (rows_src == src || rows_tgt == tgt)) return GDA_E_ALIAS;
    MmdWs ws = carve(workspace, times, n, d);
    if (workspace_bytes < ws.total) return GDA_E_WORKSPACE;
    hipStream_t stream = (hipStream_t)stream_;
    const int64_t m = 2 * n;
    const unsigned nt = (unsigned)gda_cdiv(m, TILE);
    const KParams kp{kernel_mul, kernel_num, fix_sigma};
    const unsigned chunks = (unsigned)gda_cdiv(m, SR);
    Rows R = make_rows(src, ld_src, tgt, ld_tgt, src_idx, tgt_idx, n);
    const bool fast = (rows_src || !src_idx) && d % DK == 0 && d <= 2048 && m >= 1 &&
                      (rows_src ? (d % 4 == 0 && (uintptr_t)rows_src % 16 == 0 && (uintptr_t)rows_tgt % 16 == 0) : R.vec4) &&
                      kernel_num == 5 && kernel_mul == 2.0f;
    const size_t rs_lds = fast ? sizeof(float) * SR * (size_t)(d + 1) : 0;
    if (fast && rs_lds > 48 * 1024) {
        GDA_LDS_ATTR_ONCE(k_rowstats, sizeof(float) * SR * 2049);
    }
    k_rowstats<<<dim3(chunks, (unsigned)times), TB, rs_lds, stream>>>(R, d, m, ws.part_s1, ws.part_col, rows_src, rows_tgt,
                                                                    fast ? ws.norms : nullptr, nullptr);
    GDA_LAUNCH_CHECK();
    if (rows_src) R = make_rows(rows_src, d, rows_tgt, d, nullptr, nullptr, n);
    k_bandwidth<<<(unsigned)times, BW_TB, 0, stream>>>(ws.part_s1, ws.part_col, (int)chunks, d, m, kp, bandwidth);
    GDA_LAUNCH_CHECK();
    const unsigned ntri = nt * (nt + 1) / 2;
    const dim3 grid(ntri, 1, (unsigned)times);
    if (fast)
        k_pairdist<5, true, true><<<grid, TB, 0, stream>>>(R, d, m, (int)nt, bandwidth, kp, l2_saved, ws.kpartial, ws.norms);
    else if (kernel_num == 5 && kernel_mul == 2.0f)
        k_pairdist<5, true, false><<<grid, TB, 0, stream>>>(R, d, m, (int)nt, bandwidth, kp, l2_saved, ws.kpartial, nullptr);
    else if (kernel_num == 5)
        k_pairdist<5, false, false><<<grid, TB, 0, stream>>>(R, d, m, (int)nt, bandwidth, kp, l2_saved, ws.kpartial, nullptr);
    else
        k_pairdist<0, false, false><<<grid, TB, 0, stream>>>(R, d, m, (int)nt, bandwidth, kp, l2_saved, ws.kpartial, nullptr);
    GDA_LAUNCH_CHECK();
    GDA_UNLESS_SKIPPED("k_finalize") k_finalize<<<1, TB, 0, stream>>>(ws.kpartial, (int)ntri, times, n, scale, add, loss);
    GDA_LAUNCH_CHECK();
    return GDA_OK;
}

extern "C" int gda_mmd_bwd_f32(const float* src, int64_t ld_src, const float* tgt, int64_t ld_tgt,
                               int64_t d, const int64_t* src_idx, const int64_t* tgt_idx,
                               int times, int64_t n, float kernel_mul, int kernel_num,
                               const float* bandwidth, const float* l2_saved, const float* grad_loss,
                               float* grad_rows, void* workspace, size_t workspace_bytes,
                               gda_stream_t stream_) {
    if (!grad_rows) return GDA_E_NULL;
    return gda_mmd_bwd_ex_f32(src, ld_src, tgt, ld_tgt, d, src_idx, tgt_idx, times, n, kernel_mul, kernel_num, bandwidth,
                              l2_saved, grad_loss, 1.0f, grad_rows, nullptr, nullptr, 0, nullptr, nullptr, nullptr, 0,
                              nullptr, workspace, workspace_bytes, stream_);
}

extern "C" int gda_mmd_bwd_ex_f32(const float* src, int64_t ld_src, const float* tgt, int64_t ld_tgt,
                                  int64_t d, const int64_t* src_idx, const int64_t* tgt_idx,
                                  int times, int64_t n, float kernel_mul, int kernel_num,
                                  const float* bandwidth, const float* l2_saved, const float* grad_loss, float scale,
                                  float* grad_rows,
                                  const int32_t* sel_s_rowptr, const int32_t* sel_s_col, int64_t n_src_rows, float* gsrc,
                                  const int32_t* sel_t_rowptr, const int32_t* sel_t_col, int64_t n_tgt_rows, float* gtgt,
                                  void* workspace, size_t workspace_bytes, gda_stream_t stream_) {
    int st = check_common(src, ld_src, tgt, ld_tgt, d, src_idx, tgt_idx, times, n, kernel_num);
    if (st != GDA_OK) return st;
    const bool scatter = sel_s_rowptr != nullptr;
    if (!bandwidth || !l2_saved || !grad_loss || !workspace || (!scatter && !grad_rows)) return GDA_E_NULL;
    if (scatter && (!sel_s_col || !sel_t_rowptr || !sel_t_col || !gsrc || !gtgt || n_src_rows < 0 || n_tgt_rows < 0))
        return GDA_E_NULL;
    MmdWs ws = carve(workspace, times, n, d);
    if (workspace_bytes < ws.total) return GDA_E_WORKSPACE;
    hipStream_t stream = (hipStream_t)stream_;
    const int64_t m = 2 * n;
    const Rows R = make_rows(src, ld_src, tgt, ld_tgt, src_idx, tgt_idx, n);
    const KParams kp{kernel_mul, kernel_num, 0.f};
    const int64_t ntiles = gda_cdiv(m, BJ);
    const BwdVariant var = bwd_variant(m);
    const int nseg = (int)(ntiles < var.nseg ? ntiles : var.nseg);
    const dim3 grid((unsigned)gda_cdiv(m, var.tile), (unsigned)(gda_cdiv(d, DC) * nseg), (unsigned)times);
    const bool fast = R.vec4 && !R.src_idx && m % 4 == 0 && m >= 4 && d % DC == 0 && ((uintptr_t)l2_saved % 16 == 0);
    (void)kp;
    if (var.tile == 128)
        st = fast ? launch_bwd<true, 128>(grid, stream, R, d, m, l2_saved, grad_loss, scale, times, nseg, ws.bwd_part)
                  : launch_bwd<false, 128>(grid, stream, R, d, m, l2_saved, grad_loss, scale, times, nseg, ws.bwd_part);
    else
        st = fast ? launch_bwd<true, 64>(grid, stream, R, d, m, l2_saved, grad_loss, scale, times, nseg, ws.bwd_part)
                  : launch_bwd<false, 64>(grid, stream, R, d, m, l2_saved, grad_loss, scale, times, nseg, ws.bwd_part);
    if (st != GDA_OK) return st;
    if (scatter) {
        const int64_t most = n_src_rows > n_tgt_rows ? n_src_rows : n_tgt_rows;
        if (most > 0) {
            const dim3 sg((unsigned)gda_cdiv(most, TB / 32), 2);
            const bool quads = d % 4 == 0 && ((uintptr_t)ws.bwd_part % 16 == 0) && ((uintptr_t)gsrc % 16 == 0) &&
                               ((uintptr_t)gtgt % 16 == 0);
#define GDA_SCATTER(NS) k_bwd_scatter<NS><<<sg, TB, 0, stream>>>(ws.bwd_part, m, d, d, true, nseg, sel_s_rowptr, sel_s_col, \
                                                              n_src_rows, gsrc, sel_t_rowptr, sel_t_col, n_tgt_rows, gtgt, nullptr, 1.f)
            if (quads && nseg == 6) GDA_SCATTER(6);
            else if (quads && nseg == 4) GDA_SCATTER(4);
            else GDA_SCATTER(0);
#undef GDA_SCATTER
            GDA_LAUNCH_CHECK();
        }
        return GDA_OK;
    }
    const int64_t total = (int64_t)times * m * d;
    int64_t rg = gda_cdiv(total, TB);
    if (rg > 4096) rg = 4096;
    k_bwd_reduce<<<(unsigned)rg, TB, 0, stream>>>(ws.bwd_part, m * d, nseg, times, grad_rows, nullptr, 1.f);
    GDA_LAUNCH_CHECK();
    return GDA_OK;
}

extern "C" int gda_mmd_fused_nseg(int times, int64_t n, int64_t d, float kernel_mul, int kernel_num) {
    FusedPlan fp;
    return fused_plan(times, n, d, kernel_mul, kernel_num, &fp) ? fp.nseg : 0;
}

extern "C" int gda_mmd_fused_layout(int times, int64_t n, int64_t d, int64_t* out, int n_out) {
    if (!out) return GDA_E_NULL;
    if (n_out < 16) return GDA_E_SIZE;
    FusedPlan fp;
    if (!fused_plan(times, n, d, 2.0f, 5, &fp)) return GDA_E_UNSUPPORTED;
    const MmdWs w = carve((void*)(uintptr_t)4096, times, n, d);
    const int di = (int)d;
    const int64_t v[16] = {fp.nb, fp.ntiles, fp.njb, fp.nseg, fp.total, (int64_t)fp.img,
                           f_off_rl(di), f_off_th(di), f_off_tl(di), f_off_n(di), F_OFF_XS, F_TAIL_FLOATS,
                           (int64_t)((uintptr_t)w.images - 4096), (int64_t)((uintptr_t)w.part_max - 4096),
                           (int64_t)((uintptr_t)w.kpartial - 4096), (int64_t)w.total};
    for (int i = 0; i < 16; ++i) out[i] = v[i];
    return GDA_OK;
}

template <int NB>
static int launch_fused(hipStream_t stream, const Rows& Rin, float* rows_src, float* rows_tgt, int64_t m, int64_t d, const MmdWs& ws,
                        const FusedPlan& fp, int times, float* bandwidth, float* grad_part) {
    GDA_UNLESS_SKIPPED("k_tile_split") k_tile_split<NB><<<dim3((unsigned)fp.ntiles, (unsigned)times), TB, 0, stream>>>(Rin, m, ws.part_s1, ws.part_col, ws.part_max,
                                                                               rows_src, rows_tgt, ws.images);
    GDA_LAUNCH_CHECK();
    const Rows R = rows_src ? make_rows(rows_src, d, rows_tgt, d, nullptr, nullptr, Rin.n) : Rin;
    static const bool pp = [] { const char* e = std::getenv("PYGDA_AMD_MMD_FUSED_SCHED"); return !(e && e[0] == '0'); }();
    if (pp) {
        const int npair = times * fp.nseg * (int)gda_cdiv(fp.njb, 2);
        const size_t lds = F_NBUF * fp.img + sizeof(float) * 32 * (2 * TB / 64);
        GDA_LDS_ATTR_ONCE((k_mmd_fused_pp<NB>), lds);
        const unsigned grid = 8u * (unsigned)gda_cdiv(npair, 8);
        GDA_UNLESS_SKIPPED("k_mmd_fused") k_mmd_fused_pp<NB><<<grid, 2 * TB, lds, stream>>>(R, m, fp.ntiles, fp.njb, fp.nseg, npair, ws.images, ws.part_s1,
                                                                                     ws.part_col, ws.part_max, bandwidth, grad_part, ws.kpartial);
        GDA_LAUNCH_CHECK();
        return GDA_OK;
    }
    const size_t lds = 2 * fp.img + sizeof(float) * 32 * (TB / 64);
    GDA_LDS_ATTR_ONCE((k_mmd_fused<NB>), lds);
    const unsigned grid = 8u * (unsigned)gda_cdiv(fp.total, 8);
    GDA_UNLESS_SKIPPED("k_mmd_fused") k_mmd_fused<NB><<<grid, TB, lds, stream>>>(R, m, fp.ntiles, fp.njb, fp.nseg, fp.total, ws.images, ws.part_s1, ws.part_col,
                                              ws.part_max, bandwidth, grad_part, ws.kpartial);
    GDA_LAUNCH_CHECK();
    return GDA_OK;
}

extern "C" int gda_mmd_fused_fwd_f32(const float* src, int64_t ld_src, const float* tgt, int64_t ld_tgt,
                                     int64_t d, const int64_t* src_idx, const int64_t* tgt_idx,
                                     int times, int64_t n, float kernel_mul, int kernel_num, float fix_sigma,
                                     float scale, const float* add, float* rows_src, float* rows_tgt,
                                     float* loss, float* bandwidth, float* grad_part, int nseg,
                                     void* workspace, size_t workspace_bytes, gda_stream_t stream_) {
    int st = check_common(src, ld_src, tgt, ld_tgt, d, src_idx, tgt_idx, times, n, kernel_num);
    if (st != GDA_OK) return st;
    if (!loss || !bandwidth || !grad_part || !workspace) return GDA_E_NULL;
    if ((rows_src == nullptr) != (rows_tgt == nullptr) || (rows_src && !src_idx)) return GDA_E_NULL;
    if (rows_src && (rows_src == src || rows_tgt == tgt)) return GDA_E_ALIAS;
    FusedPlan fp;
    if (!fused_plan(times, n, d, kernel_mul, kernel_num, &fp)) return GDA_E_UNSUPPORTED;
    if (fix_sigma > 0.f) return GDA_E_UNSUPPORTED;
    if (nseg != fp.nseg) return GDA_E_SIZE;
    if (src_idx && !rows_src) return GDA_E_UNSUPPORTED;
    Rows R = make_rows(src, ld_src, tgt, ld_tgt, src_idx, tgt_idx, n);
    if (!R.vec4 || (rows_src && ((uintptr_t)rows_src % 16 != 0 || (uintptr_t)rows_tgt % 16 != 0))) return GDA_E_UNSUPPORTED;
    if ((uintptr_t)grad_part % 16 != 0) return GDA_E_UNSUPPORTED;
    MmdWs ws = carve(workspace, times, n, d);
    if (workspace_bytes < ws.total) return GDA_E_WORKSPACE;
    const int64_t m = 2 * n;
    hipStream_t stream = (hipStream_t)stream_;
    switch (fp.nb) {
        case 1: st = launch_fused<1>(stream, R, rows_src, rows_tgt, m, d, ws, fp, times, bandwidth, grad_part); break;
        case 2: st = launch_fused<2>(stream, R, rows_src, rows_tgt, m, d, ws, fp, times, bandwidth, grad_part); break;
        case 3: st = launch_fused<3>(stream, R, rows_src, rows_tgt, m, d, ws, fp, times, bandwidth, grad_part); break;
        default: st = launch_fused<4>(stream, R, rows_src, rows_tgt, m, d, ws, fp, times, bandwidth, grad_part); break;
    }
    if (st != GDA_OK) return st;
    GDA_UNLESS_SKIPPED("k_finalize") k_finalize<<<1, TB, 0, stream>>>(ws.kpartial, fp.njb * fp.nseg, times, n, scale, add, loss);
    GDA_LAUNCH_CHECK();
    return GDA_OK;
}

extern "C" int gda_mmd_chunked_plan(int times, int64_t n, int64_t d, float kernel_mul, int kernel_num, int64_t* out, int n_out) {
    if (!out) return GDA_E_NULL;
    if (n_out < 8) return GDA_E_SIZE;
    ChunkPlan fp;
    if (!chunk_plan(times, n, d, kernel_mul, kernel_num, &fp)) return GDA_E_UNSUPPORTED;
    const int64_t v[8] = {fp.nseg, fp.dp, fp.nb, fp.nc, fp.ntiles, fp.njb, fp.total, (int64_t)fp.img};
    for (int i = 0; i < 8; ++i) out[i] = v[i];
    return GDA_OK;
}

#ifdef GDA_MMD_TRACE
extern "C" int gda_dbg_mmd_trace(unsigned long long* buf) {
    GDA_HIP_TRY(hipMemcpyToSymbol(HIP_SYMBOL(gda_mmd_trace_buf), &buf, sizeof(buf)));
    return GDA_OK;
}
#endif

extern "C" size_t gda_mmd_chunked_workspace_bytes(int times, int64_t n, int64_t d) {
    ChunkPlan fp;
    if (!chunk_plan(times, n, d, 2.0f, 5, &fp)) return 0;
    return chunk_carve(nullptr, times, fp).total;
}

template <int NB>
static int launch_chunked(hipStream_t stream, const Rows& Rin, float* rows_src, float* rows_tgt, int64_t ldr, int64_t m, int64_t d,
                          const ChunkWs& ws, const ChunkPlan& fp, int times, float* bandwidth, float* grad_part, int64_t ldp) {
    GDA_UNLESS_SKIPPED("k_tile_split") k_tile_split_c<NB><<<dim3((unsigned)fp.ntiles, (unsigned)times), TB, 0, stream>>>(
        Rin, m, d, fp.nc, ws.part_s1, ws.part_col, ws.part_max, rows_src, rows_tgt, ldr, ws.images);
    GDA_LAUNCH_CHECK();
    k_bw_fold<<<dim3((unsigned)gda_cdiv(fp.dp, 64), (unsigned)times), TB, 0, stream>>>(fp.ntiles, fp.dp, ws.part_s1, ws.part_col, ws.part_max, ws.bwstat);
    GDA_LAUNCH_CHECK();
    const Rows R = make_rows(rows_src, ldr, rows_tgt, ldr, nullptr, nullptr, Rin.n);
    constexpr int D = 32 * NB, PR = 2 * FT * f_rstride(D), PC = 2 * D * F_TSTRIDE;
    const size_t lds = FC_NBUF * (size_t)(PC > PR ? PC : PR) + sizeof(float) * (FC_NI * 36 + 32 * (TB / 64) + FC_STG * (TB / 64));
    GDA_LDS_ATTR_ONCE((k_mmd_chunked<NB>), lds);
    const unsigned grid = 8u * (unsigned)gda_cdiv(fp.total, 8);
    GDA_UNLESS_SKIPPED("k_mmd_fused") k_mmd_chunked<NB><<<grid, TB, lds, stream>>>(R, m, fp.ntiles, fp.nc, fp.njb, fp.nseg, fp.total, ws.images,
                                                                                  ws.bwstat, bandwidth, grad_part, ldp, ws.kpartial);
    GDA_LAUNCH_CHECK();
    return GDA_OK;
}

extern "C" int gda_mmd_chunked_fwd_f32(const float* src, int64_t ld_src, const float* tgt, int64_t ld_tgt,
                                       int64_t d, const int64_t* src_idx, const int64_t* tgt_idx,
                                       int times, int64_t n, float kernel_mul, int kernel_num, float fix_sigma,
                                       float scale, const float* add, float* rows_src, float* rows_tgt, int64_t ld_rows,
                                       float* loss, float* bandwidth, float* grad_part, int64_t ld_part, int nseg,
                                       void* workspace, size_t workspace_bytes, gda_stream_t stream_) {
    int st = check_common(src, ld_src, tgt, ld_tgt, d, src_idx, tgt_idx, times, n, kernel_num);
    if (st != GDA_OK) return st;
    if (!loss || !bandwidth || !grad_part || !workspace || !rows_src || !rows_tgt) return GDA_E_NULL;
    if (rows_src == src || rows_tgt == tgt || rows_src == rows_tgt) return GDA_E_ALIAS;
    ChunkPlan fp;
    if (!chunk_plan(times, n, d, kernel_mul, kernel_num, &fp)) return GDA_E_UNSUPPORTED;
    if (fix_sigma > 0.f) return GDA_E_UNSUPPORTED;
    if (nseg != fp.nseg || ld_rows != fp.dp || ld_part != fp.dp) return GDA_E_SIZE;
    if (((uintptr_t)rows_src | (uintptr_t)rows_tgt | (uintptr_t)grad_part) % 16 != 0) return GDA_E_UNSUPPORTED;
    Rows R = make_rows(src, ld_src, tgt, ld_tgt, src_idx, tgt_idx, n);
    ChunkWs ws = chunk_carve(workspace, times, fp);
    if (workspace_bytes < ws.total) return GDA_E_WORKSPACE;
    if ((uintptr_t)ws.images % 16 != 0) return GDA_E_UNSUPPORTED;
    const int64_t m = 2 * n;
    hipStream_t stream = (hipStream_t)stream_;
    switch (fp.nb) {
        case 1: st = launch_chunked<1>(stream, R, rows_src, rows_tgt, ld_rows, m, d, ws, fp, times, bandwidth, grad_part, ld_part); break;
        case 2: st = launch_chunked<2>(stream, R, rows_src, rows_tgt, ld_rows, m, d, ws, fp, times, bandwidth, grad_part, ld_part); break;
        case 3: st = launch_chunked<3>(stream, R, rows_src, rows_tgt, ld_rows, m, d, ws, fp, times, bandwidth, grad_part, ld_part); break;
        default: st = launch_chunked<4>(stream, R, rows_src, rows_tgt, ld_rows, m, d, ws, fp, times, bandwidth, grad_part, ld_part); break;
    }
    if (st != GDA_OK) return st;
    GDA_UNLESS_SKIPPED("k_finalize") k_finalize<<<1, TB, 0, stream>>>(ws.kpartial, fp.njb * fp.nseg, times, n, scale, add, loss);
    GDA_LAUNCH_CHECK();
    return GDA_OK;
}

extern "C" int gda_mmd_fused_bwd_mask_f32(const float* grad_part, int nseg, int times, int64_t n, int64_t d,
                                          const float* grad_loss, float scale, float* grad_rows,
                                          const int32_t* sel_s_rowptr, const int32_t* sel_s_col, int64_t n_src_rows, float* gsrc,
                                          const int32_t* sel_t_rowptr, const int32_t* sel_t_col, int64_t n_tgt_rows, float* gtgt,
                                          const float* mask_src, float p_src, const float* mask_tgt, float p_tgt,
                                          gda_stream_t stream_) {
    return gda_mmd_fused_bwd_ld_f32(grad_part, d, nseg, times, n, d, grad_loss, scale, grad_rows, sel_s_rowptr, sel_s_col,
                                    n_src_rows, gsrc, sel_t_rowptr, sel_t_col, n_tgt_rows, gtgt, mask_src, p_src, mask_tgt, p_tgt,
                                    stream_);
}

extern "C" int gda_mmd_fused_bwd_ld_f32(const float* grad_part, int64_t ld_part, int nseg, int times, int64_t n, int64_t d,
                                        const float* grad_loss, float scale, float* grad_rows,
                                        const int32_t* sel_s_rowptr, const int32_t* sel_s_col, int64_t n_src_rows, float* gsrc,
                                        const int32_t* sel_t_rowptr, const int32_t* sel_t_col, int64_t n_tgt_rows, float* gtgt,
                                        const float* mask_src, float p_src, const float* mask_tgt, float p_tgt,
                                        gda_stream_t stream_) {
    if (ld_part < d) return GDA_E_SIZE;
    if ((mask_src && !(p_src >= 0.f && p_src < 1.f)) || (mask_tgt && !(p_tgt >= 0.f && p_tgt < 1.f))) return GDA_E_SIZE;
    if ((mask_src || mask_tgt) && !sel_s_rowptr) return GDA_E_UNSUPPORTED;
    if ((((uintptr_t)mask_src | (uintptr_t)mask_tgt) % 16) && d % 4 == 0) return GDA_E_UNSUPPORTED;
    const float ms_s = mask_src ? 1.f / (1.f - p_src) : 1.f, ms_t = mask_tgt ? 1.f / (1.f - p_tgt) : 1.f;
    if (!grad_part || !grad_loss) return GDA_E_NULL;
    if (times <= 0 || n <= 0 || d <= 0 || nseg < 1 || nseg > F_NSEG_MAX) return GDA_E_SIZE;
    const bool scatter = sel_s_rowptr != nullptr;
    if (!scatter && !grad_rows) return GDA_E_NULL;
    if (scatter && (!sel_s_col || !sel_t_rowptr || !sel_t_col || !gsrc || !gtgt || n_src_rows < 0 || n_tgt_rows < 0))
        return GDA_E_NULL;
    hipStream_t stream = (hipStream_t)stream_;
    const int64_t m = 2 * n;
    const float cmul = scale / ((float)n * (float)n) / (float)times;
    if (scatter) {
        const int64_t most = n_src_rows > n_tgt_rows ? n_src_rows : n_tgt_rows;
        if (most <= 0) return GDA_OK;
        const dim3 sg((unsigned)gda_cdiv(most, TB / 32), 2);
        const bool vec_out = d % 4 == 0 && ((uintptr_t)gsrc % 16 == 0) && ((uintptr_t)gtgt % 16 == 0);
        const bool quads = ld_part % 4 == 0 && ((uintptr_t)grad_part % 16 == 0) && (vec_out || ld_part > d);
#define GDA_SCATTER(NS) k_bwd_scatter<NS><<<sg, TB, 0, stream>>>(grad_part, m, d, ld_part, vec_out, nseg, sel_s_rowptr, sel_s_col, n_src_rows, gsrc, \
                                                              sel_t_rowptr, sel_t_col, n_tgt_rows, gtgt, grad_loss, cmul,    \
                                                              mask_src, ms_s, mask_tgt, ms_t)
        if (!quads) GDA_SCATTER(0);
        else switch (nseg) {
            case 1: GDA_SCATTER(1); break;
            case 2: GDA_SCATTER(2); break;
            case 3: GDA_SCATTER(3); break;
            case 4: GDA_SCATTER(4); break;
            case 5: GDA_SCATTER(5); break;
            case 6: GDA_SCATTER(6); break;
            case 7: GDA_SCATTER(7); break;
            default: GDA_SCATTER(8); break;
        }
#undef GDA_SCATTER
        GDA_LAUNCH_CHECK();
        return GDA_OK;
    }
    const int64_t total = (int64_t)times * m * d;
    int64_t rg = gda_cdiv(total, TB);
    if (rg > 4096) rg = 4096;
    if (ld_part == d) k_bwd_reduce<<<(unsigned)rg, TB, 0, stream>>>(grad_part, m * d, nseg, times, grad_rows, grad_loss, cmul);
    else k_bwd_reduce_ld<<<(unsigned)rg, TB, 0, stream>>>(grad_part, m, d, ld_part, nseg, times, grad_rows, grad_loss, cmul);
    GDA_LAUNCH_CHECK();
    return GDA_OK;
}

extern "C" int gda_mmd_fused_bwd_f32(const float* grad_part, int nseg, int times, int64_t n, int64_t d,
                                     const float* grad_loss, float scale, float* grad_rows,
                                     const int32_t* sel_s_rowptr, const int32_t* sel_s_col, int64_t n_src_rows, float* gsrc,
                                     const int32_t* sel_t_rowptr, const int32_t* sel_t_col, int64_t n_tgt_rows, float* gtgt,
                                     gda_stream_t stream_) {
    return gda_mmd_fused_bwd_mask_f32(grad_part, nseg, times, n, d, grad_loss, scale, grad_rows, sel_s_rowptr, sel_s_col,
                                      n_src_rows, gsrc, sel_t_rowptr, sel_t_col, n_tgt_rows, gtgt, nullptr, 0.f, nullptr, 0.f,
                                      stream_);
}

// ... 1 lines not shown
```

### pygda_amd/csrc/gda_mmd_fused.inc

```
using half8 = __attribute__((ext_vector_type(8))) _Float16;
using half2v = __attribute__((ext_vector_type(2))) _Float16;

constexpr int FT = 32;
constexpr int F_TSTRIDE = 80;
__host__ __device__ constexpr int f_rstride(int d) { return (d + 8) * 2; }
__host__ __device__ constexpr int f_off_rl(int d) { return FT * f_rstride(d); }
__host__ __device__ constexpr int f_off_th(int d) { return 2 * FT * f_rstride(d); }
__host__ __device__ constexpr int f_off_tl(int d) { return f_off_th(d) + d * F_TSTRIDE; }
__host__ __device__ constexpr int f_off_n(int d) { return f_off_th(d) + 2 * d * F_TSTRIDE; }
constexpr int F_OFF_XS = 32;
constexpr int F_TAIL_FLOATS = FT + 1;
__host__ __device__ constexpr int f_img_bytes(int d) { return (f_off_n(d) + F_TAIL_FLOATS * 4 + 1023) / 1024 * 1024; }
static_assert(F_OFF_XS == FT && F_OFF_XS < F_TAIL_FLOATS, "the tile scale sits right behind the FT norms, inside the reserved tail");
static_assert(f_off_n(32) + F_TAIL_FLOATS * 4 <= f_img_bytes(32) && f_off_n(64) + F_TAIL_FLOATS * 4 <= f_img_bytes(64) &&
              f_off_n(96) + F_TAIL_FLOATS * 4 <= f_img_bytes(96) && f_off_n(128) + F_TAIL_FLOATS * 4 <= f_img_bytes(128),
              "norms + scale must lie inside the image for every covered width");
static_assert(f_off_n(32) % 16 == 0 && f_off_n(64) % 16 == 0 && f_off_n(96) % 16 == 0 && f_off_n(128) % 16 == 0,
              "the norm block is read with 16-byte LDS-DMA pieces");
constexpr int F_JB = 4;
constexpr int F_NSEG_MAX = 8;

#ifdef GDA_MMD_TRACE
__device__ unsigned long long* gda_mmd_trace_buf = nullptr;
constexpr int FZ_TR_TILES = 16, FZ_TR_SLOT = 2 + 6 * FZ_TR_TILES + 2;
#define FZ_STAMP(SLOT, I) { if (gda_mmd_trace_buf && lane == 0) gda_mmd_trace_buf[((int64_t)(SLOT)) * FZ_TR_SLOT + (I)] = __builtin_readcyclecounter(); }
#define FZ_STAMP_T(SLOT, K, I) { if ((K) < FZ_TR_TILES) FZ_STAMP(SLOT, 2 + 6 * (K) + (I)) }
#else
#define FZ_STAMP(SLOT, I) {}
#define FZ_STAMP_T(SLOT, K, I) {}
#endif

template <int NB>
__global__ void __launch_bounds__(TB)
k_tile_split(Rows R, int64_t m, double* __restrict__ part_s1, float* __restrict__ part_col, float* __restrict__ part_max,
             float* __restrict__ rows_src, float* __restrict__ rows_tgt, unsigned char* __restrict__ images) {
    constexpr int D = 32 * NB, RS = f_rstride(D), IMG = f_img_bytes(D), NG = D / 8;
    __shared__ float nrm[NG][FT];
    __shared__ float redm[TB / 64];
    __shared__ float xs_sh;
    const int t = blockIdx.y, tau = blockIdx.x, tid = threadIdx.x, lane = tid % 64, wave = tid / 64;
    const int r16 = tid & 15, g = tid >> 4, c8 = g * 8;
    const bool act = c8 < D;
    float v[2][8];
    float mx = 0.f;
    float csum[8] = {0.f, 0.f, 0.f, 0.f, 0.f, 0.f, 0.f, 0.f};
    if (act) {
        const float* pivot = row_ptr(R, t, 0) + c8;
        const float4 p0 = *reinterpret_cast<const float4*>(pivot), p1 = *reinterpret_cast<const float4*>(pivot + 4);
#pragma unroll
        for (int q = 0; q < 2; ++q) {
            const int64_t row = (int64_t)FT * tau + r16 + 16 * q;
            const bool ok = row < m;
            const float* src = row_ptr(R, t, ok ? row : m - 1) + c8;
            const float4 a0 = *reinterpret_cast<const float4*>(src), a1 = *reinterpret_cast<const float4*>(src + 4);
            if (rows_src && ok) {
                float* dst = (row < R.n ? rows_src + ((int64_t)t * R.n + row) * D : rows_tgt + ((int64_t)t * R.n + (row - R.n)) * D) + c8;
                *reinterpret_cast<float4*>(dst) = a0;
                *reinterpret_cast<float4*>(dst + 4) = a1;
            }
            const float raw[8] = {a0.x - p0.x, a0.y - p0.y, a0.z - p0.z, a0.w - p0.w, a1.x - p1.x, a1.y - p1.y, a1.z - p1.z, a1.w - p1.w};
            float nq = 0.f;
#pragma unroll
            for (int e = 0; e < 8; ++e) {
                v[q][e] = ok ? raw[e] : 0.f;
                nq = fmaf(v[q][e], v[q][e], nq);
                mx = fmaxf(mx, fabsf(v[q][e]));
                csum[e] += v[q][e];
            }
            nrm[g][r16 + 16 * q] = nq;
        }
#pragma unroll
        for (int e = 0; e < 8; ++e) {
            float c = csum[e];
            c += __shfl_xor(c, 1, 64); c += __shfl_xor(c, 2, 64); c += __shfl_xor(c, 4, 64); c += __shfl_xor(c, 8, 64);
            csum[e] = c;
        }
        if (r16 == 0) {
            float* pc = part_col + ((int64_t)t * gridDim.x + tau) * D + c8;
            *reinterpret_cast<float4*>(pc) = make_float4(csum[0], csum[1], csum[2], csum[3]);
            *reinterpret_cast<float4*>(pc + 4) = make_float4(csum[4], csum[5], csum[6], csum[7]);
        }
    }
    for (int off = 32; off > 0; off >>= 1) mx = fmaxf(mx, __shfl_down(mx, off, 64));
    if (lane == 0) redm[wave] = mx;
    __syncthreads();
    unsigned char* img = images + ((int64_t)t * gridDim.x + tau) * IMG;
    if (tid < FT) {
        float nv = 0.f;
#pragma unroll
        for (int k = 0; k < NG; ++k) nv += nrm[k][tid];
        const int64_t row = (int64_t)FT * tau + tid;
        reinterpret_cast<float*>(img + f_off_n(D))[tid] = row < m ? nv : INFINITY;
        double s1 = (double)nv;
        for (int off = 16; off > 0; off >>= 1) s1 += __shfl_down(s1, off, 64);
        if (tid == 0) {
            const float M = fmaxf(fmaxf(redm[0], redm[1]), fmaxf(redm[2], redm[3]));
            int e = 0;
            if (M > 0.f) { e = 13 - ilogbf(M); e = e < -60 ? -60 : (e > 60 ? 60 : e); }
            const float xs = ldexpf(1.f, e);
            xs_sh = xs;
            reinterpret_cast<float*>(img + f_off_n(D))[F_OFF_XS] = xs;
            part_s1[(int64_t)t * gridDim.x + tau] = s1;
            part_max[(int64_t)t * gridDim.x + tau] = M;
        }
    }
    __syncthreads();
    if (!act) return;
    const float xs = xs_sh;
    half8 hi[2], lo[2];
#pragma unroll
    for (int q = 0; q < 2; ++q) {
#pragma unroll
        for (int e = 0; e < 8; ++e) {
            const float x = v[q][e] * xs;
            const _Float16 hh = (_Float16)x;
            hi[q][e] = hh;
            lo[q][e] = (_Float16)(x - (float)hh);
        }
        *reinterpret_cast<half8*>(img + (r16 + 16 * q) * RS + c8 * 2) = hi[q];
        *reinterpret_cast<half8*>(img + f_off_rl(D) + (r16 + 16 * q) * RS + c8 * 2) = lo[q];
    }
#pragma unroll
    for (int e = 0; e < 8; ++e) {
        half2v ph, pl;
        ph[0] = hi[0][e]; ph[1] = hi[1][e];
        pl[0] = lo[0][e]; pl[1] = lo[1][e];
        *reinterpret_cast<half2v*>(img + f_off_th(D) + (c8 + e) * F_TSTRIDE + 4 * r16) = ph;
        *reinterpret_cast<half2v*>(img + f_off_tl(D) + (c8 + e) * F_TSTRIDE + 4 * r16) = pl;
    }
}

template <int NB>
__global__ void __launch_bounds__(TB, 2)
k_mmd_fused(Rows R, int64_t m, int ntiles, int njb, int nseg, int total_wg, const unsigned char* __restrict__ images,
            const double* __restrict__ part_s1, const float* __restrict__ part_col, const float* __restrict__ part_max,
            float* __restrict__ bandwidth, float* __restrict__ part, double* __restrict__ kpartial) {
    constexpr int D = 32 * NB, KB = 2 * NB, RS = f_rstride(D), IMG = f_img_bytes(D);
    constexpr int OFF_RL = f_off_rl(D), OFF_TH = f_off_th(D), OFF_TL = f_off_tl(D), OFF_N = f_off_n(D);
    extern __shared__ __attribute__((aligned(16))) unsigned char fz_lds[];
    __shared__ double red[TB / 64];
    const int per_xcd = (int)gridDim.x / 8;
    const int w = ((int)blockIdx.x % 8) * per_xcd + (int)blockIdx.x / 8;
    if (w >= total_wg) return;
    const int jb = w % njb, seg = (w / njb) % nseg, t = w / (njb * nseg);
    const int tid = threadIdx.x, wave = tid / 64, lane = tid % 64, h = lane >> 5, ln = lane & 31;
    const int it0 = (int)((int64_t)seg * ntiles / nseg), it1 = (int)((int64_t)(seg + 1) * ntiles / nseg);
    const int jt = jb * F_JB + wave;
    const int64_t tslot = wave == 0 ? 2 * (int64_t)w : -1;
#define FZ_ST(I) { if (tslot >= 0) FZ_STAMP(tslot, I) }
#define FZ_ST_T(K, I) { if (tslot >= 0) FZ_STAMP_T(tslot, K, I) }
    FZ_ST(0)
    const bool live = jt < ntiles;
    const unsigned char* timg = images + (int64_t)t * ntiles * IMG;
    const int n = (int)R.n;

    half8 bh[KB], bl[KB];
    float nj = INFINITY;
    {
        const unsigned char* ji = timg + (int64_t)(live ? jt : 0) * IMG;
#pragma unroll
        for (int kb = 0; kb < KB; ++kb) {
            bh[kb] = *reinterpret_cast<const half8*>(ji + ln * RS + (kb * 16 + 8 * h) * 2);
            bl[kb] = *reinterpret_cast<const half8*>(ji + OFF_RL + ln * RS + (kb * 16 + 8 * h) * 2);
        }
        if (live) nj = reinterpret_cast<const float*>(ji + OFF_N)[ln];
    }
    const bool sj = FT * jt + ln < n;
    float inv_xs_j = 1.f;
    if (live) inv_xs_j = 1.f / reinterpret_cast<const float*>(timg + (int64_t)jt * IMG + OFF_N)[F_OFF_XS];

#define FZ_DMA(IT, B)                                                                                                   \
    {                                                                                                                   \
        const unsigned char* g_ = timg + (int64_t)(IT) * IMG + lane * 16;                                               \
        unsigned char* l_ = fz_lds + (B) * IMG;                                                                         \
        const uint32_t l0_ = (uint32_t)(uintptr_t)(__attribute__((address_space(3))) unsigned char*)l_;                 \
        for (int c = wave; c < IMG / 1024; c += TB / 64) {                                                              \
            const unsigned char* gp_ = g_ + c * 1024;                                                                   \
            const uint32_t lp_ = __builtin_amdgcn_readfirstlane(l0_ + (uint32_t)c * 1024u);                            \
            uint32_t keep_;                                                                                             \
            asm volatile("s_mov_b32 %0, m0\n\ts_mov_b32 m0, %2\n\ts_nop 0\n\tglobal_load_lds_dwordx4 %1, off\n\ts_mov_b32 m0, %0" \
                         : "=&s"(keep_) : "v"(gp_), "s"(lp_) : "memory");                                               \
        }                                                                                                               \
    }
    FZ_DMA(it0, 0)

    float bw0, mmax;
    {
        double (*colpart)[D] = reinterpret_cast<double (*)[D]>(fz_lds + IMG);
        double* sred = reinterpret_cast<double*>(fz_lds + IMG + sizeof(double) * 8 * D);
        float* fred = reinterpret_cast<float*>(sred + 2 * (TB / 64));
        const int g = tid >> 5, c4 = (tid & 31) * 4;
        if (c4 < D) {
            double cs[4] = {0.0, 0.0, 0.0, 0.0};
            const float* pc = part_col + (int64_t)t * ntiles * D + c4;
            int k = g;
            for (; k + 56 < ntiles; k += 64) {
                float4 v[8];
#pragma unroll
                for (int u = 0; u < 8; ++u) v[u] = *reinterpret_cast<const float4*>(pc + (int64_t)(k + 8 * u) * D);
#pragma unroll
                for (int u = 0; u < 8; ++u) { cs[0] += (double)v[u].x; cs[1] += (double)v[u].y; cs[2] += (double)v[u].z; cs[3] += (double)v[u].w; }
            }
            for (; k < ntiles; k += 8) {
                const float4 v = *reinterpret_cast<const float4*>(pc + (int64_t)k * D);
                cs[0] += (double)v.x; cs[1] += (double)v.y; cs[2] += (double)v.z; cs[3] += (double)v.w;
            }
#pragma unroll
            for (int e = 0; e < 4; ++e) colpart[g][c4 + e] = cs[e];
        }
        double s1 = 0.0, s2 = 0.0;
        float mx = 0.f;
        for (int k = tid; k < ntiles; k += TB) {
            s1 += part_s1[(int64_t)t * ntiles + k];
            mx = fmaxf(mx, part_max[(int64_t)t * ntiles + k]);
        }
        __syncthreads();
        if (tid < D) {
// ... 522 lines not shown
```

### pygda_amd/models/a2gnn.py

```python
import numpy as np
import torch
import torch.nn.functional as F

from ..nn import A2GNNBase
from ..ops import grl_disc_ce, source_ce
from ..utils import MMD
from .base import BaseGDA


import contextlib

_null = contextlib.nullcontext


EARLY_CE_BACKWARD = True


class A2GNN(BaseGDA):
    def __init__(self, in_dim, hid_dim, num_classes, mode='node', num_layers=3, dropout=0.,
                 act=F.relu, s_pnums=0, t_pnums=30, adv=False, weight=5, weight_decay=0., lr=4e-3,
                 epoch=200, device='cuda:0', batch_size=0, num_neigh=-1, verbose=2, **kwargs):
        super().__init__(in_dim=in_dim, hid_dim=hid_dim, num_classes=num_classes, num_layers=num_layers,
                         dropout=dropout, act=act, weight_decay=weight_decay, lr=lr, epoch=epoch,
                         device=device, batch_size=batch_size, num_neigh=num_neigh, verbose=verbose,
                         **kwargs)
        self.s_pnums, self.t_pnums, self.adv, self.weight, self.mode = s_pnums, t_pnums, adv, weight, mode
        self.compute_target_logits = True
        self.overlap_streams = True
        self.overlap_sampled = True
        self._auto_reorder_ok = type(self) is A2GNN

    def init_model(self, **kwargs):
        return A2GNNBase(in_dim=self.in_dim, hid_dim=self.hid_dim, num_classes=self.num_classes,
                         num_layers=self.num_layers, adv=self.adv, dropout=self.dropout, act=self.act,
                         mode=self.mode, **kwargs).to(self.device)

    def _target_logits_async(self, net, target_data, h0, after):
        main = torch.cuda.current_stream()
        side = getattr(self, "_side_stream", None)
        if side is None:
            side = self._side_stream = torch.cuda.Stream()
        side.wait_event(after)
        with torch.cuda.stream(side), torch.no_grad():
            feats = net.feat_bottleneck_from(h0.detach(), target_data.edge_index, None, self.t_pnums, draw=1,
                                             preact_out=True)
            out = net.feat_classifier(feats, target_data.edge_index, None, 1)
        out.record_stream(main)
        return out, side

    def _source_branch(self, source_data):
        net = self.a2gnn
        sb = None if self.mode == 'node' else source_data.batch
        h0_s = net.first_conv(source_data.x, source_data.edge_index, self.s_pnums,
                              draws="stacked" if (self.s_pnums <= 0 and getattr(source_data, "n_id", None) is not None) else 0)
        source_features, feats = net.feat_pair_from(h0_s, source_data.edge_index, sb, self.s_pnums)
        source_logits = net.feat_classifier(feats, source_data.edge_index, sb, 1)
        loss = self._gmean(source_ce(source_logits, source_data.y), source_logits.size(0))
        from .. import hipgraph
        self._early = self._src_ready = None
        if (EARLY_CE_BACKWARD and hipgraph.defer_total and type(self) is A2GNN and not self.adv and self.mode == 'node'
                and torch.is_grad_enabled() and feats.requires_grad):
            cls_params = [p for p in net.cls.parameters() if p.requires_grad]
            self._src_ready = torch.cuda.Event()
            self._src_ready.record()
            grads = torch.autograd.grad(loss, [feats] + cls_params)
            self._early = (feats, grads[0], cls_params, grads[1:])
            loss = loss.detach()
        return loss, source_logits, source_features

    def _target_branch(self, target_data, fork, h0_t=None):
        net = self.a2gnn
        tb = None if self.mode == 'node' else target_data.batch
        table = getattr(self, "_grad_aliases", None)
        with (net.second_leaves(table) if table is not None and torch.is_grad_enabled() else _null()):
            if h0_t is None:
                h0_t = net.first_conv(target_data.x, target_data.edge_index, self.t_pnums,
                                      draws=(2 if self.compute_target_logits else 1)
                                      if getattr(target_data, "n_id", None) is not None else 0)
            pending = None
            if self.compute_target_logits and fork:
                ready = torch.cuda.Event()
                ready.record()
                target_features = net.feat_bottleneck_from(h0_t, target_data.edge_index, tb, self.t_pnums)
                pending = self._target_logits_async(net, target_data, h0_t, after=ready)
                return h0_t, pending, target_features
            target_features = net.feat_bottleneck_from(h0_t, target_data.edge_index, tb, self.t_pnums)
        return h0_t, pending, target_features

    def _domain_loss(self, loss, source_features, target_features, alpha):
        net = self.a2gnn
        if self.adv and self.mode != 'node':
            raise ValueError(f"Expected input batch_size ({source_features.size(0) + target_features.size(0)}) to match "
                             "target batch_size (the node count): adv=True is not defined for mode='graph' in pygda "
                             "(a2gnn.py:199-204)")
        if self.adv:
            disc = net.domain_discriminator
            dom = grl_disc_ce(source_features, target_features, disc.weight, disc.bias, alpha)
            return loss + self.weight * self._gmean(dom, source_features.size(0) + target_features.size(0))
        mmd = MMD(source_features, target_features, scale=self.weight)
        from .. import hipgraph
        if hipgraph.defer_total and type(self) is A2GNN:
            terms = hipgraph.LossTerms((loss, mmd))
            early = getattr(self, "_early", None)
            if early is not None:
                feats, g_feats, cls_params, g_cls = early
                terms.extra_roots, terms.preset_grads = [(feats, g_feats)], list(zip(cls_params, g_cls))
                self._early = None
            return terms
        return loss + mmd

    def _branches(self, source_data, target_data):
        net = self.a2gnn
        node = self.mode == 'node'
        sb = None if node else source_data.batch
        tb = None if node else target_data.batch
        sampled = getattr(target_data, "n_id", None) is not None or getattr(source_data, "n_id", None) is not None
        fork = node and source_data.x.is_cuda and self.overlap_streams and (not sampled or self.overlap_sampled)
        main = torch.cuda.current_stream() if fork else None
        if fork:
            src_stream = getattr(self, "_src_stream", None)
            if src_stream is None:
                src_stream = self._src_stream = torch.cuda.Stream()
                quiet = getattr(torch.autograd.graph, "set_warn_on_accumulate_grad_stream_mismatch", None)
                if quiet is not None:
                    quiet(False)
            src_stream.wait_stream(main)
        with (torch.cuda.stream(src_stream) if fork else _null()):
            loss, source_logits, source_features = self._source_branch(source_data)
        h0_t, pending, target_features = self._target_branch(target_data, fork)
        if fork:
            ready = getattr(self, "_src_ready", None)
            if ready is not None:
                main.wait_event(ready)
            else:
                main.wait_stream(src_stream)
            for t in (loss, source_logits, source_features):
                t.record_stream(main)
        return loss, source_logits, source_features, target_features, h0_t, pending, (sb, tb)

    def forward_model(self, source_data, target_data, alpha):
        if (not self.adv and self.mode == 'node' and source_data.x.is_cuda
                and (getattr(source_data, "n_id", None) is not None or getattr(target_data, "n_id", None) is not None)):
            from ..utils.mmd import prefetch_samples
            prefetch_samples(source_data.x.size(0), target_data.x.size(0), source_data.x.device)
        from .. import ops as _ops
        sinks = (type(self) is A2GNN and not self.adv and self.mode == 'node' and source_data.x.is_cuda
                 and getattr(source_data, "n_id", None) is not None and getattr(target_data, "n_id", None) is not None)
        with (_ops.grad_sinks() if sinks else _null()):
            loss, source_logits, source_features, target_features, h0_t, pending, (sb, tb) = \
                self._branches(source_data, target_data)
        net = self.a2gnn
        loss = self._domain_loss(loss, source_features, target_features, alpha)
        if pending is not None:
            target_logits, side = pending
            torch.cuda.current_stream().wait_stream(side)
        elif self.compute_target_logits:
            feats_t = net.feat_bottleneck_from(h0_t, target_data.edge_index, tb, self.t_pnums, draw=1)
            target_logits = net.feat_classifier(feats_t, target_data.edge_index, tb, 1)
        else:
            target_logits = None
        return loss, source_logits, target_logits

    def _dp_graph_parts(self):
        if self.adv:
            return None
        from ..ops import mmd_loss_rows, sample_rows

        def part1(src, tgt, idx_s, idx_t, sel_s=None, sel_t=None):
            loss_ce, source_logits, sf, tf, _, pending, _ = self._branches(src, tgt)
            rows_s, rows_t = sample_rows(sf, idx_s, sel_s), sample_rows(tf, idx_t, sel_t)
            if pending is not None:
                torch.cuda.current_stream().wait_stream(pending[1])
            return loss_ce, source_logits, rows_s, rows_t

        def part2(rows_s_all, rows_t_all):
            return mmd_loss_rows(rows_s_all, rows_t_all) * self.weight

        return part1, part2

    def _prepare(self, source_data, target_data):
        self._sampled_graph_ok = type(self) is A2GNN and not self.adv and self.mode == 'node'
        self._loaders(source_data, target_data)
        self.a2gnn = self.init_model(**self.kwargs)
        self._graph_safe_step, self._graph_uses_scalars = self.mode == 'node', bool(self.adv)
        self._graph_unroll_ok = not self.adv and type(self) is A2GNN
        self._graph_forks = self.overlap_streams
        on_gpu = torch.device(self.device).type == "cuda"
        self._grad_aliases = None
        if on_gpu:
            from ..optim import Adam
            optimizer = Adam(self.a2gnn.parameters(), lr=self.lr, weight_decay=self.weight_decay)
            from .. import distributed
            if type(self) is A2GNN and not distributed.active():
                self._grad_aliases = optimizer.grad_aliases
        else:
            optimizer = torch.optim.Adam(self.a2gnn.parameters(), lr=self.lr, weight_decay=self.weight_decay)

        def step(src, tgt, alpha, epoch):
            loss, source_logits, _ = self.forward_model(src, tgt, alpha)
            return loss, source_logits

        def alpha(e):
            return 2. / (1. + np.exp(-10. * float(e) / self.epoch)) - 1

        return self.a2gnn, optimizer, step, alpha

    def fit(self, source_data, target_data):
        self._train_epochs(*self._prepare(source_data, target_data))

    def process_graph(self, data):
        pass

    def predict(self, data, source=False, reference_compat=None):
        self.a2gnn.eval()
        loader, k = (self.source_loader, self.s_pnums) if source else (self.target_loader, self.t_pnums)
        return self._predict_loader(loader, lambda batch: self.a2gnn(batch, k), reference_compat)
```

### pygda_amd/ops.py

```python
import ctypes
import weakref

import os as _os

import torch

from . import _lib, profiler
from .graph import CSRGraph, build_csr


def _f32c(t, name):
    _lib.require_gpu_tensor(t, name)
    if t.dtype != torch.float32:
        raise _lib.GdaError(f"{name}: the aggregation path computes in fp32, got {t.dtype}")
    return t.contiguous()


GRAD_SINKS = True
_sinks_on = False
sink_hits = 0


class grad_sinks:

# ... 608 lines not shown
        raise ValueError("K must be >= 1")
    if isinstance(x, ColMajor):
        return ColMajor(_PropagateT.apply(x.t, bias, graph, int(K), True), x.n)
    if colmajor_out and lds_colmajor_ok(x, graph, K):
        return ColMajor(_PropagateT.apply(x, bias, graph, int(K)), x.size(0))
    return _Propagate.apply(x, bias, graph, int(K))


def propagate_act_ok(x, graph, K, bias):
    return (isinstance(x, torch.Tensor) and x.is_cuda and x.dim() == 2 and x.dtype == torch.float32
            and x.is_contiguous() and _takes_interior_path(graph, x, bias, False)
            and _interior_lds_plan(graph, x, x, int(K), False) is not None)


class _PropagateAct(torch.autograd.Function):

    @staticmethod
    def forward(ctx, x, bias, graph, K, p, pair):
        x = _f32c(x, "x")
        n, d = x.shape
        n_int = graph.n_interior
        y0 = torch.empty_like(x)
        y1 = torch.empty_like(x) if pair else None
        b = None if bias is None else _f32c(bias, "bias")
        plan = _interior_lds_plan(graph, x, y0, K, False)
        gen = dropout_state.generator(x.device, sites=2) if pair else (*dropout_state.generator(x.device), 0)
        if aggregation_log is not None:
            nnz_h, T = getattr(graph, "_nnz", None), getattr(graph, "iplan_T", None)
            executed = None
            if nnz_h is not None:
                executed = (nnz_h + (int(K) - 1) * (T + n_int) if T is not None
                            else int(K) * (nnz_h - (n - n_int)) + (n - n_int))
            aggregation_log.append((_logged(graph), int(K), executed, "interior-lds"))
        _note_path("interior-lds", int(K))
        if profiler.enabled:
            global aggregated_edges
            aggregated_edges += int(K) * graph.nnz
            nnz, n_leaf, row = graph.nnz, n - n_int, 4 * d
            alg = K * (nnz * 8 + (n + 1) * 4 + 2 * n * d * 4)
            real = nnz * 8 + min(nnz, n) * row + 6 * n_int * row + (2 + bool(pair)) * n_leaf * row
            region = profiler.region(f"interior_lds_f32[d={d}]", 3, real, K * 2 * nnz * d, alg_equiv_bytes=alg,
                                     step_loop_launches=1)
        else:
            region = profiler.region("", 0)
        ws, nbytes = _lib.scratch("gda_interior_kstep_lds_workspace_bytes", x.device, "interior_lds",
                                  _interior_lds_limits()[0], d)
        with region:
            _lib.call("gda_interior_kstep_lds_act_f32", graph.rowptr, graph.colidx, graph.val, n, n_int, d, int(K),
                      plan, x, y0, y1, b, float(p), *gen, ws, nbytes, _lib.stream())
        ctx.graph, ctx.K, ctx.has_bias, ctx.p = graph, K, bias is not None, float(p)
        ctx.save_for_backward(y0)
        ctx.sink = _offer_sink(y0, p, wanted=ctx.needs_input_grad[0] or ctx.needs_input_grad[1])
        if pair:
            ctx.mark_non_differentiable(y1)
            return y0, y1
        return y0

    @staticmethod
    def backward(ctx, g0, g1=None):
        (y0,) = ctx.saved_tensors
        if ctx.sink is not None and ctx.sink.mine(g0):
            gpre = g0
        else:
            g0 = g0.contiguous()
            gpre = torch.empty_like(g0)
            _lib.call("gda_relu_dropout_bwd_f32", g0, y0, gpre, g0.numel(), ctx.p, _lib.stream())
        gx = spmm_kstep(ctx.graph, gpre, ctx.K, None, transposed=True) if ctx.needs_input_grad[0] else None
        gb = colsum(gpre) if ctx.has_bias and ctx.needs_input_grad[1] else None
        return gx, gb, None, None, None, None


def propagate_act(x, graph, K, bias, p, training, pair=False):
    return _PropagateAct.apply(x, bias, graph, int(K), float(p) if training else 0.0, bool(pair))


def lds_colmajor_ok(x, graph, K):
    return (x.dim() == 2 and x.size(1) % 4 == 0 and x.is_cuda and x.dtype == torch.float32
            and lds_kstep_plan(graph, int(K), False) is not None and lds_kstep_plan(graph, int(K), True) is not None)


MMD_ONE_PASS = _os.environ.get("PYGDA_AMD_MMD_ONE_PASS", "1") == "1"


MMD_CHUNKED = _os.environ.get("PYGDA_AMD_MMD_CHUNKED", "auto")


def mmd_chunked_plan(times, n, d, kernel_mul=2.0, kernel_num=5):
    if not MMD_ONE_PASS or MMD_CHUNKED == "0" or not (MMD_CHUNKED == "always" or d > 128 or d % 32):
        return None
    import ctypes
    out = (ctypes.c_int64 * 8)()
    if _lib.lib().gda_mmd_chunked_plan(int(times), int(n), int(d), float(kernel_mul), int(kernel_num), out, 8) != 0:
        return None
    return int(out[0]), int(out[1])


def mmd_one_pass_segments(times, n, d, kernel_mul=2.0, kernel_num=5):
    if not MMD_ONE_PASS:
        return 0
    plan = mmd_chunked_plan(times, n, d, kernel_mul, kernel_num)
    if plan is not None:
        return plan[0]
    return int(_lib.lib().gda_mmd_fused_nseg(int(times), int(n), int(d), float(kernel_mul), int(kernel_num)))


_one_pass_checked = {}


def mmd_one_pass_ok(dev):
    global MMD_ONE_PASS
    key = dev.index if dev.index is not None else torch.cuda.current_device()
    state = _one_pass_checked.get(key)
    if state is not None:
        return state is not False
    if torch.cuda.is_current_stream_capturing():
        return True
    _one_pass_checked[key] = "running"
    gen = torch.Generator().manual_seed(20240521)
    ok, why = True, ""
    try:
        for d in (128, 64, 200):
            times, n = 2, 80
            a = (torch.randn(times * n, d, generator=gen) * 0.7 + 0.3).to(dev).requires_grad_(True)
            b = (torch.randn(times * n, d, generator=gen) * 0.9 - 0.1).to(dev).requires_grad_(True)
            got = []
            for one in (True, False):
                MMD_ONE_PASS = one
                with torch.enable_grad():
                    loss = _MMD.apply(a, b, None, None, times, n, 2.0, 5, None)
                    ga, gb = torch.autograd.grad(loss, (a, b))
                got.append((loss.detach().double(), torch.cat([ga, gb]).double()))
            MMD_ONE_PASS = True
            (l1, g1), (l2, g2) = got
            dl = float((l1 - l2).abs() / l2.abs().clamp_min(1e-30))
            dg = float((g1 - g2).norm() / g2.norm().clamp_min(1e-30))
            if not (dl <= 1e-4 and dg <= 1e-4):
                ok, why = False, f"d={d}: loss differs by {dl:.3g}, row gradients by {dg:.3g} (relative)"
                break
    except Exception as exc:
        ok, why = False, f"{type(exc).__name__}: {exc}"
    finally:
        MMD_ONE_PASS = True
    _one_pass_checked[key] = ok
    if not ok:
        import warnings
        warnings.warn("one-pass MMD kernel declined by its first-use self-check (" + why +
                      "); this process uses the two-pass fp32-MFMA kernels")
    return ok


class _MMD(torch.autograd.Function):
    @staticmethod
    def forward(ctx, src, tgt, src_idx, tgt_idx, times, n, kernel_mul, kernel_num, fix_sigma, sel=None, scale=1.0,
                add=None):
        ctx.sel, ctx.scale, ctx.has_add = sel, float(scale), add is not None
        ctx.sinks = (sink_of(src), sink_of(tgt))
        src, tgt = _f32c(src, "source_feat"), _f32c(tgt, "target_feat")
        d = src.size(1)
        if tgt.size(1) != d:
            raise ValueError("source and target features must have the same width")
        dev = src.device
        m = 2 * n
        ctx.feat_rows = (src.size(0), tgt.size(0))
        idx_s = idx_t = rows_s = rows_t = None
        plan = mmd_chunked_plan(times, n, d, kernel_mul, kernel_num) if not fix_sigma else None
        if plan is not None and not mmd_one_pass_ok(dev):
            plan = None
        if src_idx is not None:
            idx_s, idx_t = src_idx.contiguous(), tgt_idx.contiguous()
            if plan is None:
                rows_s = torch.empty(times * n, d, dtype=torch.float32, device=dev)
                rows_t = torch.empty(times * n, d, dtype=torch.float32, device=dev)
        loss = torch.empty(1, dtype=torch.float32, device=dev)
        bw = torch.empty(times, dtype=torch.float32, device=dev)
        addc = None if add is None else add.detach().to(torch.float32).reshape(1).contiguous()
        nseg = 0
        if plan is not None:
            nseg, dp = plan
            rows_s = torch.empty(times * n, dp, dtype=torch.float32, device=dev)
            rows_t = torch.empty(times * n, dp, dtype=torch.float32, device=dev)
            part = torch.empty(times, nseg, m, dp, dtype=torch.float32, device=dev)
            ws, _ = _lib.scratch("gda_mmd_chunked_workspace_bytes", dev, "mmd_chunked", times, n, d)
            with profiler.region("mmd_fwd", 5, 0, times * 3 * 4 * m * m * dp):
                _lib.call("gda_mmd_chunked_fwd_f32", src, d, tgt, d, d, idx_s, idx_t, times, n, float(kernel_mul),
                          int(kernel_num), 0.0, float(scale), addc, rows_s, rows_t, dp, loss, bw, part, dp, nseg, ws,
                          ws.numel(), _lib.stream())
            ctx.one_pass, ctx.ldp = nseg, dp
            ctx.save_for_backward(src_idx, tgt_idx, part)
            ctx.cfg = (times, n, d, float(kernel_mul), int(kernel_num))
            return loss.reshape(())
        ws, _ = _lib.scratch("gda_mmd_workspace_bytes", dev, "mmd", times, n, d)
        if not fix_sigma:
            nseg = mmd_one_pass_segments(times, n, d, kernel_mul, kernel_num)
            aligned = src.data_ptr() % 16 == 0 and tgt.data_ptr() % 16 == 0
            nseg = nseg if aligned and (not nseg or mmd_one_pass_ok(dev)) else 0
        ctx.one_pass, ctx.ldp = nseg, d
        if nseg:
            part = torch.empty(times, nseg, m, d, dtype=torch.float32, device=dev)
            with profiler.region("mmd_fwd", 4, 0, times * 3 * 4 * m * m * d):
                _lib.call("gda_mmd_fused_fwd_f32", src, d, tgt, d, d, idx_s, idx_t, times, n, float(kernel_mul),
                          int(kernel_num), float(fix_sigma) if fix_sigma else 0.0, float(scale), addc, rows_s, rows_t,
                          loss, bw, part, nseg, ws, ws.numel(), _lib.stream())
            ctx.save_for_backward(src_idx, tgt_idx, part)
            ctx.cfg = (times, n, d, float(kernel_mul), int(kernel_num))
            return loss.reshape(())
        l2 = torch.empty(times, m, m, dtype=torch.float32, device=dev)
        with profiler.region("mmd_fwd", 4, 0, times * (3 * m * m * d // 2 + 12 * m * m)):
            _lib.call("gda_mmd_fwd_gather_f32", src, d, tgt, d, d, idx_s, idx_t, times, n, float(kernel_mul),
                      int(kernel_num), float(fix_sigma) if fix_sigma else 0.0, float(scale), addc, rows_s, rows_t, loss,
                      bw, l2, ws, ws.numel(), _lib.stream())
        if rows_s is not None:
            src, tgt = rows_s, rows_t
        ctx.save_for_backward(src, tgt, src_idx, tgt_idx, bw, l2)
        ctx.cfg = (times, n, float(kernel_mul), int(kernel_num))
        return loss.reshape(())

    @staticmethod
    def backward(ctx, gl):
        if ctx.one_pass:
            return _MMD._backward_one_pass(ctx, gl)
        src, tgt, src_idx, tgt_idx, bw, l2 = ctx.saved_tensors
        times, n, kernel_mul, kernel_num = ctx.cfg
        d, dev, m = src.size(1), src.device, 2 * n
        glc = gl.reshape(1).to(torch.float32).contiguous()
        ws, _ = _lib.scratch("gda_mmd_workspace_bytes", dev, "mmd", times, n, d)
        g_add = gl if ctx.has_add else None
        tail = (None,) * 9 + (g_add,)
        if src_idx is not None and ctx.sel is not None:
            s_rp, s_ci, t_rp, t_ci, _ones = ctx.sel
            gs = torch.empty(ctx.feat_rows[0], d, dtype=torch.float32, device=dev)
            gt = torch.empty(ctx.feat_rows[1], d, dtype=torch.float32, device=dev)
            with profiler.region("mmd_bwd", 2, 0, times * (3 * m * m * d + 12 * m * m)):
                _lib.call("gda_mmd_bwd_ex_f32", src, d, tgt, d, d, None, None, times, n, kernel_mul, kernel_num, bw,
                          l2, glc, ctx.scale, None, s_rp, s_ci, ctx.feat_rows[0], gs, t_rp, t_ci, ctx.feat_rows[1], gt,
                          ws, ws.numel(), _lib.stream())
            return (gs if ctx.needs_input_grad[0] else None, gt if ctx.needs_input_grad[1] else None) + tail
        grad_rows = torch.empty(times, m, d, dtype=torch.float32, device=dev)
        with profiler.region("mmd_bwd", 2, 0, times * (3 * m * m * d + 12 * m * m)):
            _lib.call("gda_mmd_bwd_ex_f32", src, d, tgt, d, d, None, None, times, n, kernel_mul, kernel_num, bw, l2,
                      glc, ctx.scale, grad_rows, None, None, 0, None, None, None, 0, None, ws, ws.numel(),
                      _lib.stream())
        if src_idx is None:
            gs, gt = grad_rows[:, :n].reshape(times * n, d), grad_rows[:, n:].reshape(times * n, d)
        else:
            gs = _scatter_rows(grad_rows, src_idx, 0, n, ctx.feat_rows[0])
            gt = _scatter_rows(grad_rows, tgt_idx, n, n, ctx.feat_rows[1])
        return (gs if ctx.needs_input_grad[0] else None, gt if ctx.needs_input_grad[1] else None) + tail


def _mmd_backward_one_pass(ctx, gl):
    src_idx, tgt_idx, part = ctx.saved_tensors
    times, n, d, _, _ = ctx.cfg
    dev, m = part.device, 2 * n
    glc = gl.reshape(1).to(torch.float32).contiguous()
    g_add = gl if ctx.has_add else None
    tail = (None,) * 9 + (g_add,)
    if src_idx is not None and ctx.sel is not None:
        s_rp, s_ci, t_rp, t_ci, _ones = ctx.sel
        ok = lambda k, rows: (k is not None and k.buf.shape == (rows, d) and k.buf.data_ptr() % 16 == 0
                              and k.y.data_ptr() % 16 == 0)
        ks = ctx.sinks[0] if ok(ctx.sinks[0], ctx.feat_rows[0]) and ctx.needs_input_grad[0] else None
        kt = ctx.sinks[1] if ok(ctx.sinks[1], ctx.feat_rows[1]) and ctx.needs_input_grad[1] else None
        gs = ks.buf if ks is not None else torch.empty(ctx.feat_rows[0], d, dtype=torch.float32, device=dev)
        gt = kt.buf if kt is not None else torch.empty(ctx.feat_rows[1], d, dtype=torch.float32, device=dev)
        with profiler.region("mmd_bwd", 1, 0, 0):
            _lib.call("gda_mmd_fused_bwd_ld_f32", part, ctx.ldp, ctx.one_pass, times, n, d, glc, ctx.scale, None, s_rp,
                      s_ci, ctx.feat_rows[0], gs, t_rp, t_ci, ctx.feat_rows[1], gt, ks.y if ks is not None else None,
                      ks.p if ks is not None else 0.0, kt.y if kt is not None else None,
                      kt.p if kt is not None else 0.0, _lib.stream())
        for k in (ks, kt):
            if k is not None:
                k.written = True
        return (gs if ctx.needs_input_grad[0] else None, gt if ctx.needs_input_grad[1] else None) + tail
    grad_rows = torch.empty(times, m, d, dtype=torch.float32, device=dev)
    with profiler.region("mmd_bwd", 1, 0, 0):
        _lib.call("gda_mmd_fused_bwd_ld_f32", part, ctx.ldp, ctx.one_pass, times, n, d, glc, ctx.scale, grad_rows, None,
                  None, 0, None, None, None, 0, None, None, 0.0, None, 0.0, _lib.stream())
    if src_idx is None:
        gs, gt = grad_rows[:, :n].reshape(times * n, d), grad_rows[:, n:].reshape(times * n, d)
    else:
        gs = _scatter_rows(grad_rows, src_idx, 0, n, ctx.feat_rows[0])
        gt = _scatter_rows(grad_rows, tgt_idx, n, n, ctx.feat_rows[1])
    return (gs if ctx.needs_input_grad[0] else None, gt if ctx.needs_input_grad[1] else None) + tail


_MMD._backward_one_pass = staticmethod(_mmd_backward_one_pass)


class _PinnedRing:

    def __init__(self, slots=4):
        self.slots, self.turn = [None] * slots, 0

    def take(self, nbytes):
        i = self.turn
        self.turn = (i + 1) % len(self.slots)
        hit = self.slots[i]
        if hit is not None and hit[1] is not None:
            hit[1].synchronize()
        if hit is None or hit[0].numel() < nbytes:
            cap = 1 << 16
            while cap < nbytes + nbytes // 2:
                cap <<= 1
            hit = [torch.empty(cap, dtype=torch.uint8).pin_memory(), None]
            self.slots[i] = hit
        return i, hit[0]

    def sent(self, i, stream):
        ev = torch.cuda.Event()
        ev.record(stream)
        self.slots[i][1] = ev


_pinned_ring = _PinnedRing()


def mmd_samples_to_device(source_sample, target_sample, ns, nt, dev, stacked=True):
    times, n = source_sample.shape
    m = 2 * n if stacked else n
    a16 = lambda v: (v + 15) // 16 * 16
    sizes = [8 * times * n, 8 * times * n, 4 * (ns + 1), 4 * times * n, 4 * (nt + 1), 4 * times * n]
    offs = [0]
    for sz in sizes:
        offs.append(offs[-1] + a16(sz))
    slot, host = _pinned_ring.take(offs[-1])
    view = lambda k, dt, cnt: host[offs[k]:offs[k] + sizes[k]].view(dt)[:cnt]
    view(0, torch.int64, times * n).copy_(source_sample.reshape(-1))
    view(1, torch.int64, times * n).copy_(target_sample.reshape(-1))
    selection_csr_host(source_sample, ns, 0, m, out=(view(2, torch.int32, ns + 1), view(3, torch.int32, times * n)))
    selection_csr_host(target_sample, nt, n if stacked else 0, m,
                       out=(view(4, torch.int32, nt + 1), view(5, torch.int32, times * n)))
    block = torch.empty(offs[-1], dtype=torch.uint8, device=dev)
    from .hipgraph import _ship
    _ship(block, host[:offs[-1]])
    _pinned_ring.sent(slot, torch.cuda.current_stream())
    dview = lambda k, dt, cnt: block[offs[k]:offs[k] + sizes[k]].view(dt)[:cnt]
    sel = (dview(2, torch.int32, ns + 1), dview(3, torch.int32, times * n),
           dview(4, torch.int32, nt + 1), dview(5, torch.int32, times * n),
           torch.ones(times * n, dtype=torch.float32, device=dev))
    return dview(0, torch.int64, times * n).view(times, n), dview(1, torch.int64, times * n).view(times, n), sel


def selection_csr_host(idx, num_feat_rows, offset, m, out=None):
    idx = idx.contiguous()
    times, n = idx.shape
    if out is None:
        out = (torch.empty(num_feat_rows + 1, dtype=torch.int32), torch.empty(times * n, dtype=torch.int32))
    _lib.call("gda_selection_csr_host", idx.data_ptr(), int(times), int(n), int(num_feat_rows), int(offset), int(m),
              out[0].data_ptr(), out[1].data_ptr())
    return out


def _selection_spmm(rowptr, colidx, ones, flat, num_feat_rows):
    d = flat.size(1)
    out = torch.empty(num_feat_rows, d, dtype=torch.float32, device=flat.device)
    _lib.call("gda_spmm_csr_f32", rowptr, colidx, ones, num_feat_rows, d, flat, d, out, d, None, _lib.stream())
    return out


def _scatter_rows(grad_rows, idx, offset, n, num_feat_rows):
    times, m, d = grad_rows.shape
    dev = grad_rows.device
    pos = (torch.arange(times, device=dev).view(-1, 1) * m + offset +
           torch.arange(n, device=dev).view(1, -1)).reshape(-1)
    n_nodes = max(num_feat_rows, times * m)
    g = build_csr(torch.stack([pos, idx.reshape(-1)]), n_nodes, None, add_self_loops=False,
                  normalize=False, validate=False)
    flat = grad_rows.view(times * m, d)
    if n_nodes > times * m:
        pass
    out = torch.empty(num_feat_rows, d, dtype=torch.float32, device=dev)
    _lib.call("gda_spmm_csr_f32", g.rowptr, g.colidx, g.val, num_feat_rows, d, flat, d, out, d, None, _lib.stream())
    return out


class _SampleRows(torch.autograd.Function):

    @staticmethod
    def forward(ctx, feat, idx, sel=None):
        ctx.save_for_backward(idx)
        ctx.rows, ctx.sel = feat.size(0), sel
        return gather_rows(feat, idx.reshape(-1)).view(idx.size(0), idx.size(1), feat.size(1))

    @staticmethod
    def backward(ctx, g):
        (idx,) = ctx.saved_tensors
        times, n, d = g.shape
        g = g.contiguous()
        if ctx.sel is not None:
            rowptr, colidx, ones = ctx.sel
            return _selection_spmm(rowptr, colidx, ones, g.view(times * n, d), ctx.rows), None, None
        return _scatter_rows(g.view(times, n, d), idx, 0, n, ctx.rows), None, None


def sample_rows(feat, idx, sel=None):
    return _SampleRows.apply(_f32c(feat, "feat"), idx, sel)


def mmd_loss_rows(source_rows, target_rows, kernel_mul=2.0, kernel_num=5, fix_sigma=None):
    if source_rows.shape != target_rows.shape or source_rows.dim() != 3:
        raise RuntimeError("row sets must both be [times, n, d]")
    times, n, d = source_rows.shape
    return _MMD.apply(source_rows.reshape(times * n, d), target_rows.reshape(times * n, d), None, None,
                      int(times), int(n), kernel_mul, kernel_num, fix_sigma)


def mmd_loss(source_feat, target_feat, src_idx=None, tgt_idx=None, kernel_mul=2.0, kernel_num=5,
             fix_sigma=None, sel=None, scale=1.0, add=None):
    if (src_idx is None) != (tgt_idx is None):
        raise ValueError("give both index tensors or neither")
    if src_idx is None:
        if source_feat.size(0) != target_feat.size(0):
            raise RuntimeError("get_MMD needs equally many source and target rows, got "
                               f"{source_feat.size(0)} and {target_feat.size(0)}")
        times, n = 1, source_feat.size(0)
    else:
        _lib.require_gpu_tensor(src_idx, "src_idx", torch.int64)
        _lib.require_gpu_tensor(tgt_idx, "tgt_idx", torch.int64)
        if src_idx.shape != tgt_idx.shape or src_idx.dim() != 2:
            raise RuntimeError("source and target samples must both be [times, sampling_num]")
        times, n = src_idx.shape
        src_idx, tgt_idx = src_idx.contiguous(), tgt_idx.contiguous()
    return _MMD.apply(source_feat, target_feat, src_idx, tgt_idx, int(times), int(n), kernel_mul,
                      kernel_num, fix_sigma, sel, scale, add)


class _GrlDiscCE(torch.autograd.Function):
    @staticmethod
    def forward(ctx, fs, ft, W, b, alpha, labels):
        fs, ft, W, b = _f32c(fs, "source_feat"), _f32c(ft, "target_feat"), _f32c(W, "weight"), _f32c(b, "bias")
        ns, nt, h, C = fs.size(0), ft.size(0), fs.size(1), W.size(0)
        dev = fs.device
        probs = torch.empty(ns + nt, C, dtype=torch.float32, device=dev)
        loss = torch.empty(1, dtype=torch.float32, device=dev)
        ws, _ = _lib.scratch("gda_grl_disc_workspace_bytes", dev, "disc", ns + nt, h, C)
        _lib.call("gda_grl_disc_ce_fwd_f32", fs, h, ns, ft, h, nt, h, C, W, b, labels, probs, loss, ws, ws.numel(),
                  _lib.stream())
        ctx.save_for_backward(fs, ft, W, probs, labels)
        ctx.alpha = float(alpha)
        return loss.reshape(())

    @staticmethod
    def backward(ctx, gl):
        fs, ft, W, probs, labels = ctx.saved_tensors
        ns, nt, h, C = fs.size(0), ft.size(0), fs.size(1), W.size(0)
        dev = fs.device
        gfs = torch.empty_like(fs) if ctx.needs_input_grad[0] else None
        gft = torch.empty_like(ft) if ctx.needs_input_grad[1] else None
        gW, gb = torch.empty_like(W), torch.empty(C, dtype=torch.float32, device=dev)
        gl = gl.reshape(1).to(torch.float32).contiguous()
        ws, _ = _lib.scratch("gda_grl_disc_workspace_bytes", dev, "disc", ns + nt, h, C)
        _lib.call("gda_grl_disc_ce_bwd_f32", fs, h, ns, ft, h, nt, h, C, W, labels, probs, gl, ctx.alpha, gfs, gft, gW,
                  gb, ws, ws.numel(), _lib.stream())
        return gfs, gft, gW, gb, None, None


def grl_disc_ce(source_feat, target_feat, weight, bias, alpha, labels=None):
    if torch.is_tensor(alpha):
        from .nn.reverse_layer import GradReverse
        return _GrlDiscCE.apply(GradReverse.apply(source_feat, alpha), GradReverse.apply(target_feat, alpha),
                                weight, bias, -1.0, labels)
    return _GrlDiscCE.apply(source_feat, target_feat, weight, bias, alpha, labels)


def _grl_mlp_fwd(ctx, es, et, W1, b1, W2, b2, alpha, p, head=0):
    ctx.head = head
    es, et = _f32c(es, "source_feat"), _f32c(et, "target_feat")
    W1, b1, W2, b2 = _f32c(W1, "W1"), _f32c(b1, "b1"), _f32c(W2, "W2"), _f32c(b2, "b2")
    ns, nt, h, a = es.size(0), et.size(0), es.size(1), W1.size(0)
    dev = es.device
    seed, step, site, _ = dropout_state.generator(dev, sites=2)
    losses = torch.empty(3, dtype=torch.float32, device=dev)
    ws, _ = _lib.scratch("gda_grl_mlp_ce_workspace_bytes", dev, "disc_mlp", h, a)
    with profiler.region(f"disc_mlp_fwd[{h}x{a}]", 2, 4 * (ns + nt) * h, 2 * (ns + nt) * a * (h + W2.size(0))):
        _lib.call("gda_mlp_head_fwd_f32", head, es, h, ns, et, h, nt, h, a, W1, b1, W2, b2, float(p), seed, step, site,
                  losses, ws, ws.numel(), _lib.stream())
    ctx.save_for_backward(es, et, W1, b1, W2, b2, alpha if torch.is_tensor(alpha) else None)
    ctx.alpha = None if torch.is_tensor(alpha) else float(alpha)
    ctx.p, ctx.seed, ctx.site = float(p), seed, site
    return losses


def _grl_mlp_bwd(ctx, g, stride):
    es, et, W1, b1, W2, b2, alpha_dev = ctx.saved_tensors
    ns, nt, h, a = es.size(0), et.size(0), es.size(1), W1.size(0)
    dev = es.device
    ges = torch.empty_like(es) if ctx.needs_input_grad[0] else None
    get = torch.empty_like(et) if ctx.needs_input_grad[1] else None
    gW1, gb1, gW2, gb2 = torch.empty_like(W1), torch.empty_like(b1), torch.empty_like(W2), torch.empty_like(b2)
    if alpha_dev is not None:
        alpha_dev = alpha_dev.detach().reshape(1).to(torch.float32)
    ws, _ = _lib.scratch("gda_grl_mlp_ce_workspace_bytes", dev, "disc_mlp", h, a)
    with profiler.region(f"disc_mlp_bwd[{h}x{a}]", 2, 4 * (ns + nt) * h * (2 if ges is not None else 1), 6 * (ns + nt) * a * h):
        _lib.call("gda_mlp_head_bwd_f32", ctx.head, es, h, ns, et, h, nt, h, a, W1, b1, W2, b2, ctx.p, ctx.seed,
                  dropout_state.counter(dev), ctx.site, g, stride, 0.0 if ctx.alpha is None else ctx.alpha, alpha_dev,
                  ges, get, gW1, gb1, gW2, gb2, ws, ws.numel(), _lib.stream())
    return ges, get, gW1, gb1, gW2, gb2, None, None


class _GrlMlpCESum(torch.autograd.Function):

    @staticmethod
    def forward(ctx, es, et, W1, b1, W2, b2, alpha, p):
        return _grl_mlp_fwd(ctx, es, et, W1, b1, W2, b2, alpha, p)[2]

    @staticmethod
    def backward(ctx, g):
        return _grl_mlp_bwd(ctx, g.reshape(1).to(torch.float32).contiguous(), 0)


class _GrlMlpCEPair(torch.autograd.Function):

    @staticmethod
    def forward(ctx, es, et, W1, b1, W2, b2, alpha, p):
        losses = _grl_mlp_fwd(ctx, es, et, W1, b1, W2, b2, alpha, p)
        return losses[0], losses[1]

    @staticmethod
    def backward(ctx, g_s, g_t):
        return _grl_mlp_bwd(ctx, torch.stack([g_s.reshape(()).to(torch.float32), g_t.reshape(()).to(torch.float32)]), 1)


class _CriticMeans(torch.autograd.Function):

    @staticmethod
    def forward(ctx, es, et, W1, b1, W2, b2, p):
        losses = _grl_mlp_fwd(ctx, es, et, W1, b1, W2, b2, -1.0, p, head=1)
        return losses[0], losses[1]

    @staticmethod
    def backward(ctx, g_s, g_t):
        return _grl_mlp_bwd(ctx, torch.stack([g_s.reshape(()).to(torch.float32), g_t.reshape(()).to(torch.float32)]), 1)[:7]


class _CriticMeansVec(torch.autograd.Function):

    @staticmethod
    def forward(ctx, es, et, W1, b1, W2, b2, p):
        return _grl_mlp_fwd(ctx, es, et, W1, b1, W2, b2, -1.0, p, head=1)

    @staticmethod
    def backward(ctx, g):
        return _grl_mlp_bwd(ctx, g.to(torch.float32).contiguous(), 1)[:7]


class _AddAbsGap(torch.autograd.Function):
    _wvec = {}

    @staticmethod
    def forward(ctx, base, v, weight):
        key = (float(weight), v.device, v.numel())
        wv = _AddAbsGap._wvec.get(key)
        if wv is None:
            wv = _AddAbsGap._wvec[key] = torch.tensor([weight, -weight] + [0.0] * (v.numel() - 2), dtype=torch.float32, device=v.device)
        d = v[0] - v[1]
        svec = torch.sign(d) * wv
        ctx.save_for_backward(svec)
        return torch.addcmul(base, d, svec[0])

    @staticmethod
    def backward(ctx, g):
        (svec,) = ctx.saved_tensors
        return g, g * svec, None


def critic_abs_gap_loss(base, source_feat, target_feat, W1, b1, W2, b2, dropout_p, weight):
    v = _CriticMeansVec.apply(source_feat, target_feat, W1, b1, W2, b2, dropout_p)
    return _AddAbsGap.apply(base, v, float(weight))


def critic_means_ok(es, W1, W2):
    return (es.is_cuda and es.dtype == torch.float32 and es.dim() == 2 and es.size(1) <= 128
            and W1.size(0) <= 64 and W2.dim() == 2 and W2.size(0) == 1)


# ... 62 lines not shown
    n_i = 0 if idx_s is None else idx_s.numel()
    ws, _ = _lib.scratch("gda_wgan_critic_workspace_bytes", es.device, "critic", n_s, n_t, n_i, h, a)
    seed, step, site, _, _ = dropout_state.generator(es.device, sites=3)
    loss, gW1, gb1, gW2, gb2 = out
    rows_gp = n_s + n_t + n_i
    with profiler.region(f"wgan_critic[{h}x{a}]", 2 if h in (64, 96, 128) and a % 4 == 0 else 7,
                         4 * h * (n_s + n_t + 2 * n_i), 2 * a * h * (4 * rows_gp + n_s + n_t)):
        _lib.call("gda_wgan_critic_f32", es, n_s, et, n_t, h, idx_s, idx_t,
                  None if alpha is None else _f32c(alpha, "alpha"), n_i, _f32c(W1, "W1"), _f32c(b1, "b1"),
                  _f32c(W2, "W2"), _f32c(b2, "b2"), a, float(dropout_p), seed, step, site, float(gp_weight), loss, gW1, gb1, gW2, gb2, ws, ws.numel(), _lib.stream())
    return loss


def wgan_critic_adam(es, et, idx_s, idx_t, alpha, params, optimizer, dropout_p, gp_weight, loss):
    from .optim import Adam
    if not isinstance(optimizer, Adam) or len(optimizer.param_groups) != 1 or optimizer.grad_aliases:
        return False
    group = optimizer.param_groups[0]
    if len(group["params"]) != 4 or any(a is not b for a, b in zip(group["params"], params)):
        return False
    es, et = _f32c(es, "encoded_source"), _f32c(et, "encoded_target")
    n_s, h = es.shape
    n_t, a = et.size(0), params[0].size(0)
    W1 = params[0]
    if not (h in (64, 96, 128) and a % 4 == 0 and all(p.is_contiguous() and p.dtype == torch.float32 for p in params)
            and (es.data_ptr() | et.data_ptr() | W1.data_ptr()) % 16 == 0):
        return False
    n_i = 0 if idx_s is None else idx_s.numel()
    ws, _ = _lib.scratch("gda_wgan_critic_workspace_bytes", es.device, "critic", n_s, n_t, n_i, h, a)
    table = (_lib.AdamTensorStruct * 4)()
    for k, p in enumerate(params):
        stt = optimizer._state(p)
        if p.grad is None or not p.grad.is_contiguous() or any(stt[n].stride() != p.stride() for n in ("exp_avg", "exp_avg_sq")):
            return False
        table[k] = _lib.AdamTensorStruct(p.data_ptr(), p.grad.data_ptr(), stt["exp_avg"].data_ptr(),
                                         stt["exp_avg_sq"].data_ptr(), stt["step"].data_ptr(), p.numel())
    seed, step, site, _, _ = dropout_state.generator(es.device, sites=3)
    b1_, b2_ = group["betas"]
    rows_gp = n_s + n_t + n_i
    with profiler.region(f"wgan_critic[{h}x{a}]", 2, 4 * h * (n_s + n_t + 2 * n_i), 2 * a * h * (4 * rows_gp + n_s + n_t)):
        _lib.call("gda_wgan_critic_adam_f32", es, n_s, et, n_t, h, idx_s, idx_t,
                  None if alpha is None else _f32c(alpha, "alpha"), n_i, a, float(dropout_p), seed, step, site,
                  float(gp_weight), loss, table, float(group["lr"]), float(b1_), float(b2_), float(group["eps"]),
                  float(group["weight_decay"]), ws, ws.numel(), _lib.stream())
    return True


def gather_rows(x, idx):
    x = _f32c(x, "x")
    _lib.require_gpu_tensor(idx, "idx", torch.int64)
    idx = idx.contiguous()
    out = torch.empty(idx.numel(), x.size(1), dtype=torch.float32, device=x.device)
    _lib.call("gda_gather_rows_f32", x, x.size(1), x.size(1), idx, idx.numel(), out, x.size(1), _lib.stream())
    return out


class _SegmentMean(torch.autograd.Function):
    @staticmethod
    def forward(ctx, x, seg_ptr, batch):
        x = _f32c(x, "x")
        G, d = seg_ptr.numel() - 1, x.size(1)
        out = torch.empty(G, d, dtype=torch.float32, device=x.device)
        _lib.call("gda_segment_mean_fwd_f32", x, d, seg_ptr, G, d, out, d, _lib.stream())
        ctx.save_for_backward(seg_ptr, batch)
        ctx.n = x.size(0)
        return out

    @staticmethod
    def backward(ctx, gout):
        seg_ptr, batch = ctx.saved_tensors
        gout = gout.contiguous()
        d = gout.size(1)
        gx = torch.empty(ctx.n, d, dtype=torch.float32, device=gout.device)
        _lib.call("gda_segment_mean_bwd_f32", gout, d, seg_ptr, batch, ctx.n, d, gx, d, _lib.stream())
        return gx, None, None


def segment_ptr(batch, size=None):
    hit = getattr(batch, "_gda_seg_ptr", None)
    if hit is not None and (size is None or hit.numel() - 1 == size):
        return hit
    _lib.require_gpu_tensor(batch, "batch", torch.int64)
    if batch.numel() > 1 and not getattr(batch, "_gda_sorted", False) and bool((batch[1:] < batch[:-1]).any()):
        raise ValueError("global_mean_pool: `batch` must be sorted (nodes of a graph contiguous), as PyG's DataLoader "
                         "collates it")
    G = (int(batch[-1]) + 1 if batch.numel() else 0) if size is None else int(size)
    seg = torch.zeros(G + 1, dtype=torch.int64, device=batch.device)
    if batch.numel():
        seg[1:] = torch.cumsum(torch.bincount(batch, minlength=G), 0)
    batch._gda_seg_ptr = seg
    return seg


def segment_mean(x, batch, size=None):
    return _SegmentMean.apply(x, segment_ptr(batch, size), batch.contiguous())


class _DropoutState:

    def __init__(self):
        self.step = {}
        self.site = 0
        self.seed = None

    def counter(self, dev):
        t = self.step.get(dev)
        if t is None:
            t = self.step[dev] = torch.zeros(1, dtype=torch.int64, device=dev)
        return t

    def next_step(self, dev):
        self.counter(dev).add_(1)
        self.site = 0

    def next_site(self):
        self.site += 1
        return self.site

    def generator(self, dev, sites=1):
        if self.seed is None:
            self.seed = int(torch.initial_seed()) & (2 ** 63 - 1)
        return (self.seed, self.counter(dev), *[self.next_site() for _ in range(sites)])


dropout_state = _DropoutState()


class _ReluDropout(torch.autograd.Function):
    @staticmethod
    def forward(ctx, x, p):
        x = _f32c(x, "x")
        y = torch.empty_like(x)
        _lib.call("gda_relu_dropout_fwd_f32", x, y, x.numel(), float(p), *dropout_state.generator(x.device),
                  _lib.stream())
        ctx.save_for_backward(y)
        ctx.p = float(p)
        ctx.sink = _offer_sink(y, p, wanted=ctx.needs_input_grad[0])
        return y

    @staticmethod
    def backward(ctx, gy):
        (y,) = ctx.saved_tensors
        if ctx.sink is not None and ctx.sink.mine(gy):
            return gy, None
        gy = gy.contiguous()
        gx = torch.empty_like(gy)
        _lib.call("gda_relu_dropout_bwd_f32", gy, y, gx, gy.numel(), ctx.p, _lib.stream())
        return gx, None


class _ReluDropoutT(torch.autograd.Function):

    @staticmethod
    def forward(ctx, xT, n, p):
        d, n_pad = xT.shape
        y = torch.empty(n, d, dtype=torch.float32, device=xT.device)
        _lib.call("gda_relu_dropout_fwd_cm_f32", xT, n_pad, y, n, d, float(p), *dropout_state.generator(xT.device),
                  _lib.stream())
        ctx.save_for_backward(y)
        ctx.p, ctx.n_pad = float(p), n_pad
        return y

    @staticmethod
    def backward(ctx, gy):
        (y,) = ctx.saved_tensors
        return _relu_dropout_t_backward(y, gy, ctx.p, ctx.n_pad), None, None


def _relu_dropout_t_backward(y, gy, p, n_pad):
    n, d = y.shape
    gy = gy.contiguous()
    gxT = torch.empty(d, n_pad, dtype=torch.float32, device=gy.device)
    if n_pad != n:
        gxT[:, n:].zero_()
    _lib.call("gda_relu_dropout_bwd_cm_f32", gy, y, gxT, n_pad, n, d, p, _lib.stream())
    return gxT


class _ReluDropoutPair(torch.autograd.Function):

    @staticmethod
    def forward(ctx, x, p):
        x = _f32c(x, "x")
        n, d = x.shape
        y = torch.empty(2 * n, d, dtype=torch.float32, device=x.device)
        _lib.call("gda_relu_dropout_pair_fwd_f32", x, y, n, d, float(p), *dropout_state.generator(x.device, sites=2),
                  _lib.stream())
        ctx.save_for_backward(y)
        ctx.p = float(p)
        return y

    @staticmethod
    def backward(ctx, gy):
        (y,) = ctx.saved_tensors
        n, d = y.size(0) // 2, y.size(1)
        gy = gy.contiguous()
        gx = torch.empty(n, d, dtype=torch.float32, device=gy.device)
        cs = ws = None
        nbytes = 0
        if d <= 1024:
            cs = torch.empty(d, dtype=torch.float32, device=gy.device)
            ws, nbytes = _lib.scratch("gda_relu_dropout_pair_workspace_bytes", gy.device, "pair_colsum", d)
        _lib.call("gda_relu_dropout_pair_bwd_f32", gy, y, gx, n, d, ctx.p, cs, ws, nbytes, _lib.stream())
        global _colsum_hint
        _colsum_hint = (gx.data_ptr(), cs, gx) if cs is not None else None
        return gx, None


def relu_dropout_pair_ok(x):
    return torch.is_tensor(x) and x.is_cuda and x.dtype == torch.float32 and x.dim() == 2 and x.size(1) % 4 == 0


def relu_dropout_pair(x, p, training=True):
    return _ReluDropoutPair.apply(x, float(p) if training else 0.0)


class _SplitHalves(torch.autograd.Function):

    @staticmethod
    def forward(ctx, x):
        n = x.size(0) // 2
        ctx.shape = (n, x.size(1))
        ctx.set_materialize_grads(False)
        return x.narrow(0, 0, n), x.narrow(0, n, n)

    @staticmethod
    def backward(ctx, ga, gb):
        n, d = ctx.shape
        ref = ga if ga is not None else gb
        if ref is None:
            return None
        out = torch.empty(2 * n, d, dtype=torch.float32, device=ref.device)
        ga = None if ga is None else ga.contiguous()
        gb = None if gb is None else gb.contiguous()
        _lib.call("gda_stack2_f32", ga, gb, out, n * d, _lib.stream())
        return out


def split_halves(x):
    return _SplitHalves.apply(x)


class _SplitRows(torch.autograd.Function):

    @staticmethod
    def forward(ctx, x, k):
        ctx.k, ctx.shape = int(k), tuple(x.shape)
        ctx.set_materialize_grads(False)
        return x.narrow(0, 0, ctx.k), x.narrow(0, ctx.k, x.size(0) - ctx.k)

    @staticmethod
    def backward(ctx, ga, gb):
        ref = ga if ga is not None else gb
        if ref is None:
            return None, None
        out = torch.empty(ctx.shape, dtype=ref.dtype, device=ref.device)
        for part, g in ((out[:ctx.k], ga), (out[ctx.k:], gb)):
            if g is None:
                part.zero_()
            else:
                part.copy_(g)
        return out, None


def split_rows(x, k):
    return _SplitRows.apply(x, k)


class _ReluDropoutSplit(torch.autograd.Function):

    @staticmethod
    def forward(ctx, x, p):
        x = _f32c(x, "x")
        y = torch.empty_like(x)
        _lib.call("gda_relu_dropout_fwd_f32", x, y, x.numel(), float(p), *dropout_state.generator(x.device),
                  _lib.stream())
        ctx.save_for_backward(y)
        ctx.p = float(p)
        ctx.set_materialize_grads(False)
        n = x.size(0) // 2
        a, b = y.narrow(0, 0, n), y.narrow(0, n, n)
        ctx.sinks, ctx.G = (None, None), None
        if _sinks_on and ctx.needs_input_grad[0]:
            ctx.G = torch.empty_like(y)
            ctx.sinks = (_offer_sink(a, p, ctx.G.narrow(0, 0, n)), _offer_sink(b, p, ctx.G.narrow(0, n, n)))
        return a, b

    @staticmethod
    def backward(ctx, ga, gb):
        (y,) = ctx.saved_tensors
        if ga is None and gb is None:
            return None, None
        n = y.size(0) // 2
        done = [k is not None and k.mine(g) for k, g in zip(ctx.sinks, (ga, gb))]
        if any(done):
            for k, (g, ok) in enumerate(zip((ga, gb), done)):
                if ok:
                    continue
                dst, yh = ctx.G.narrow(0, k * n, n), y.narrow(0, k * n, n)
                if g is None:
                    dst.zero_()
                else:
                    g = g.contiguous()
                    _lib.call("gda_relu_dropout_bwd_f32", g, yh, dst, g.numel(), ctx.p, _lib.stream())
            return ctx.G, None
        ga = None if ga is None else ga.contiguous()
        gb = None if gb is None else gb.contiguous()
        gx = torch.empty_like(y)
        _lib.call("gda_relu_dropout_bwd2_f32", ga, gb, y, gx, y.numel() // 2, ctx.p, _lib.stream())
        return gx, None


TALL_FUSED = True


class GatheredRows:
    __slots__ = ("base", "idx", "_dense")
    requires_grad = False
    _version = 0
# ... 2384 lines not shown
```

Before: 3.523 billion.

## Fuse ReLU-dropout of column-major target activations into fused MMD forward and backward

Adds MMD forward and backward entry points that read the target features straight from the transposed pre-activation buffer. ReLU and dropout are recomputed inside the tile-split kernel and the backward scatter, which writes the transposed gradient through a shared-memory tile. This removes the separate relu-dropout forward and backward kernels and the materialised row-major target activation for the A2GNN node path. In exchange the dropout mask is regenerated in both kernels, which adds PRNG work, and the path depends on many preconditions such as d being 32 to 128 and aligned pointers.

```diff
diff --git a/include/gda_hip.h b/include/gda_hip.h
--- a/include/gda_hip.h
+++ b/include/gda_hip.h
@@ -223,6 +223,20 @@
                                const int32_t* sel_t_rowptr, const int32_t* sel_t_col, int64_t n_tgt_rows, float* gtgt,
                                const float* mask_src, float p_src, const float* mask_tgt, float p_tgt,
                                gda_stream_t stream);
+int gda_mmd_fused_fwd_act_cm_f32(const float* src, int64_t ld_src, const float* tgtT, int64_t ldT, int64_t n_tgt_rows,
+                                 int64_t d, const int64_t* src_idx, const int64_t* tgt_idx,
+                                 int times, int64_t n, float kernel_mul, int kernel_num, float fix_sigma,
+                                 float scale, const float* add, float* rows_src, float* rows_tgt,
+                                 float* loss, float* bandwidth, float* grad_part, int nseg,
+                                 float p, uint64_t seed, const int64_t* step, uint32_t site,
+                                 void* workspace, size_t workspace_bytes, gda_stream_t stream);
+int gda_mmd_fused_bwd_act_cm_f32(const float* grad_part, int nseg, int times, int64_t n, int64_t d,
+                                 const float* grad_loss, float scale,
+                                 const int32_t* sel_s_rowptr, const int32_t* sel_s_col, int64_t n_src_rows, float* gsrc,
+                                 const int32_t* sel_t_rowptr, const int32_t* sel_t_col, int64_t n_tgt_rows,
+                                 const float* tgtT, float* gxT, int64_t ldT,
+                                 float p, uint64_t seed, const int64_t* step, uint32_t site,
+                                 const float* mask_src, float p_src, gda_stream_t stream);
 
 int gda_mmd_chunked_plan(int times, int64_t n, int64_t d, float kernel_mul, int kernel_num, int64_t* out, int n_out);
 size_t gda_mmd_chunked_workspace_bytes(int times, int64_t n, int64_t d);
diff --git a/pygda_amd/_lib.py b/pygda_amd/_lib.py
--- a/pygda_amd/_lib.py
+++ b/pygda_amd/_lib.py
@@ -122,6 +122,12 @@
                                       _P, _P, c_int64, _P, _P, _P, c_int64, _P, _P]),
     "gda_mmd_fused_bwd_mask_f32": (c_int, [_P, c_int, c_int, c_int64, c_int64, _P, c_float, _P,
                                            _P, _P, c_int64, _P, _P, _P, c_int64, _P, _P, c_float, _P, c_float, _P]),
+    "gda_mmd_fused_fwd_act_cm_f32": (c_int, [_P, c_int64, _P, c_int64, c_int64, c_int64, _P, _P, c_int, c_int64, c_float, c_int,
+                                             c_float, c_float, _P, _P, _P, _P, _P, _P, c_int, c_float, ctypes.c_uint64, _P,
+                                             ctypes.c_uint32, _P, c_size_t, _P]),
+    "gda_mmd_fused_bwd_act_cm_f32": (c_int, [_P, c_int, c_int, c_int64, c_int64, _P, c_float, _P, _P, c_int64, _P, _P, _P,
+                                             c_int64, _P, _P, c_int64, c_float, ctypes.c_uint64, _P, ctypes.c_uint32, _P,
+                                             c_float, _P]),
     "gda_copy_from_pinned": (c_int, [_P, _P, c_size_t, _P]),
     "gda_softmax_entropy_fwd_f32": (c_int, [_P, c_int64, c_int64, c_int, c_float, _P, _P, c_size_t, _P]),
     "gda_softmax_entropy_bwd_f32": (c_int, [_P, c_int64, c_int64, c_int, c_float, _P, _P, c_int64, _P]),
diff --git a/pygda_amd/csrc/gda_act.hip b/pygda_amd/csrc/gda_act.hip
--- a/pygda_amd/csrc/gda_act.hip
+++ b/pygda_amd/csrc/gda_act.hip
@@ -432,7 +432,7 @@
     if (half_elems == 0) return GDA_OK;
     if (!y || !gx) return GDA_E_NULL;
     if (half_elems % 4 != 0 || ((uintptr_t)ga | (uintptr_t)gb | (uintptr_t)y | (uintptr_t)gx) % 16 != 0) return GDA_E_UNSUPPORTED;
-    k_relu_dropout_bwd2<<<grid_for(2 * half_elems), TB, 0, (hipStream_t)stream>>>(ga, gb, y, gx, half_elems, 1.f / (1.f - p));
+    GDA_UNLESS_SKIPPED("k_relu_dropout_bwd2") k_relu_dropout_bwd2<<<grid_for(2 * half_elems), TB, 0, (hipStream_t)stream>>>(ga, gb, y, gx, half_elems, 1.f / (1.f - p));
     GDA_LAUNCH_CHECK();
     return GDA_OK;
 }
diff --git a/pygda_amd/csrc/gda_mmd.hip b/pygda_amd/csrc/gda_mmd.hip
--- a/pygda_amd/csrc/gda_mmd.hip
+++ b/pygda_amd/csrc/gda_mmd.hip
@@ -688,6 +688,96 @@
 
 #include "gda_mmd_fused.inc"
 #include "gda_mmd_chunked.inc"
+
+constexpr int SC_ROWS = 16, SC_LD = 132, SC_TB = 32 * SC_ROWS;
+template <int NSEG>
+__global__ void __launch_bounds__(SC_TB)
+k_bwd_scatter_cm(const float* __restrict__ part, int64_t m, int64_t d, int64_t ldp,
+                 const int32_t* __restrict__ s_rowptr, const int32_t* __restrict__ s_col, int64_t n_src_rows,
+                 float* __restrict__ gsrc, const int32_t* __restrict__ t_rowptr, const int32_t* __restrict__ t_col,
+                 int64_t n_tgt_rows, float* __restrict__ gxT, ActCM A, const float* __restrict__ grad_loss, float cmul,
+                 const float* __restrict__ mask_s, float mscale_s) {
+    __shared__ __attribute__((aligned(16))) float tile[SC_ROWS][SC_LD];
+    const float c4 = grad_loss ? 4.f * (grad_loss[0] * cmul) : 4.f;
+    const int lane = threadIdx.x % 32, grp = threadIdx.x / 32;
+    const int mi = (int)m;
+    const int64_t c = (int64_t)lane * 4;
+    if (blockIdx.y == 0) {
+        const int64_t r = (int64_t)blockIdx.x * SC_ROWS + grp;
+        if (r >= n_src_rows || c >= d) return;
+        const int32_t b = s_rowptr[r], e = s_rowptr[r + 1];
+        float4 acc = make_float4(0.f, 0.f, 0.f, 0.f);
+        int32_t pn = b < e ? s_col[b] : 0;
+        for (int32_t k = b; k < e; ++k) {
+            const int p = pn;
+            if (k + 1 < e) pn = s_col[k + 1];
+            const int t = p / mi, i = p - t * mi;
+            const float* q = part + (((int64_t)t * NSEG) * m + i) * ldp + c;
+            float4 v[NSEG];
+#pragma unroll
+            for (int g = 0; g < NSEG; ++g) v[g] = *reinterpret_cast<const float4*>(q + (int64_t)g * m * ldp);
+            float4 sg = make_float4(0.f, 0.f, 0.f, 0.f);
+#pragma unroll
+            for (int g = 0; g < NSEG; ++g) { sg.x += v[g].x; sg.y += v[g].y; sg.z += v[g].z; sg.w += v[g].w; }
+            acc.x = __fadd_rn(acc.x, c4 * sg.x); acc.y = __fadd_rn(acc.y, c4 * sg.y);
+            acc.z = __fadd_rn(acc.z, c4 * sg.z); acc.w = __fadd_rn(acc.w, c4 * sg.w);
+        }
+        if (mask_s) acc = relu_keep_bwd(*reinterpret_cast<const float4*>(mask_s + r * d + c), acc, mscale_s);
+        *reinterpret_cast<float4*>(gsrc + r * d + c) = acc;
+        return;
+    }
+    const int64_t r0 = (int64_t)blockIdx.x * SC_ROWS;
+    if (r0 >= A.ldT) return;
+    const bool live = c < d;
+    const uint64_t st = (uint64_t)A.step[0];
+    const uint32_t thresh = dropout_thresh(A.p);
+    {
+        const int64_t rr = r0 + grp;
+        const bool in = live && rr < n_tgt_rows;
+        const int32_t b = in ? t_rowptr[rr] : 0, e = in ? t_rowptr[rr + 1] : 0;
+        int32_t pn = b < e ? t_col[b] : 0;
+        bool kept[4] = {false, false, false, false};
+        float x[4] = {0.f, 0.f, 0.f, 0.f};
+        if (b < e) {
+            uint32_t rn[4];
+            dropout_draw(A.seed, st, A.site, (uint64_t)((rr * d + c) >> 2), rn);
+            const float* col = A.xT + c * A.ldT + rr;
+#pragma unroll
+            for (int v = 0; v < 4; ++v) {
+                kept[v] = dropout_kept(rn[v], thresh);
+                if (kept[v]) x[v] = col[v * A.ldT];
+            }
+        }
+        float4 acc = make_float4(0.f, 0.f, 0.f, 0.f);
+        for (int32_t k = b; k < e; ++k) {
+            const int p = pn;
+            if (k + 1 < e) pn = t_col[k + 1];
+            const int t = p / mi, i = p - t * mi;
+            const float* q = part + (((int64_t)t * NSEG) * m + i) * ldp + c;
+            float4 v[NSEG];
+#pragma unroll
+            for (int g = 0; g < NSEG; ++g) v[g] = *reinterpret_cast<const float4*>(q + (int64_t)g * m * ldp);
+            float4 sg = make_float4(0.f, 0.f, 0.f, 0.f);
+#pragma unroll
+            for (int g = 0; g < NSEG; ++g) { sg.x += v[g].x; sg.y += v[g].y; sg.z += v[g].z; sg.w += v[g].w; }
+            acc.x = __fadd_rn(acc.x, c4 * sg.x); acc.y = __fadd_rn(acc.y, c4 * sg.y);
+            acc.z = __fadd_rn(acc.z, c4 * sg.z); acc.w = __fadd_rn(acc.w, c4 * sg.w);
+        }
+        float4 o;
+        o.x = (x[0] > 0.f && kept[0]) ? acc.x * A.scale : 0.f;
+        o.y = (x[1] > 0.f && kept[1]) ? acc.y * A.scale : 0.f;
+        o.z = (x[2] > 0.f && kept[2]) ? acc.z * A.scale : 0.f;
+        o.w = (x[3] > 0.f && kept[3]) ? acc.w * A.scale : 0.f;
+        if (live) *reinterpret_cast<float4*>(&tile[grp][c]) = o;
+    }
+    __syncthreads();
+    const int j = threadIdx.x % 4;
+    if (r0 + 4 * j >= A.ldT) return;
+    for (int cc = threadIdx.x / 4; cc < d; cc += SC_TB / 4) {
+        const float4 o = make_float4(tile[4 * j + 0][cc], tile[4 * j + 1][cc], tile[4 * j + 2][cc], tile[4 * j + 3][cc]);
+        *reinterpret_cast<float4*>(gxT + (int64_t)cc * A.ldT + r0 + 4 * j) = o;
+    }
+}
 
 struct MmdWs {
     double* kpartial; double* part_s1; float* part_col; float* bwd_part; float* norms;
@@ -903,7 +993,11 @@
 
 template <int NB>
 static int launch_fused(hipStream_t stream, const Rows& Rin, float* rows_src, float* rows_tgt, int64_t m, int64_t d, const MmdWs& ws,
-                        const FusedPlan& fp, int times, float* bandwidth, float* grad_part) {
+                        const FusedPlan& fp, int times, float* bandwidth, float* grad_part, const ActCM* act_cm = nullptr) {
+    if (act_cm) {
+        GDA_UNLESS_SKIPPED("k_tile_split") k_tile_split_cm<NB><<<dim3((unsigned)fp.ntiles, (unsigned)times), TB, 0, stream>>>(
+            Rin, *act_cm, m, ws.part_s1, ws.part_col, ws.part_max, rows_src, rows_tgt, ws.images);
+    } else
     GDA_UNLESS_SKIPPED("k_tile_split") k_tile_split<NB><<<dim3((unsigned)fp.ntiles, (unsigned)times), TB, 0, stream>>>(Rin, m, ws.part_s1, ws.part_col, ws.part_max,
                                                                                rows_src, rows_tgt, ws.images);
     GDA_LAUNCH_CHECK();
@@ -959,6 +1053,85 @@
     }
     if (st != GDA_OK) return st;
     GDA_UNLESS_SKIPPED("k_finalize") k_finalize<<<1, TB, 0, stream>>>(ws.kpartial, fp.njb * fp.nseg, times, n, scale, add, loss);
+    GDA_LAUNCH_CHECK();
+    return GDA_OK;
+}
+
+extern "C" int gda_mmd_fused_fwd_act_cm_f32(const float* src, int64_t ld_src, const float* tgtT, int64_t ldT, int64_t n_tgt_rows,
+                                            int64_t d, const int64_t* src_idx, const int64_t* tgt_idx,
+                                            int times, int64_t n, float kernel_mul, int kernel_num, float fix_sigma,
+                                            float scale, const float* add, float* rows_src, float* rows_tgt,
+                                            float* loss, float* bandwidth, float* grad_part, int nseg,
+                                            float p, uint64_t seed, const int64_t* step, uint32_t site,
+                                            void* workspace, size_t workspace_bytes, gda_stream_t stream_) {
+    if (!src || !tgtT) return GDA_E_NULL;
+    if (d <= 0 || n <= 0 || times <= 0 || ld_src < d || n_tgt_rows < 1 || ldT < n_tgt_rows || !(p >= 0.f && p < 1.f)) return GDA_E_SIZE;
+    if (2 * n >= 46340 * 2) return GDA_E_SIZE;
+    if (kernel_num < 1 || kernel_num > MAXQ) return GDA_E_UNSUPPORTED;
+    if (!loss || !bandwidth || !grad_part || !workspace || !step) return GDA_E_NULL;
+    if (!src_idx || !tgt_idx || !rows_src || !rows_tgt) return GDA_E_UNSUPPORTED;
+    if (rows_src == src || rows_src == rows_tgt) return GDA_E_ALIAS;
+    FusedPlan fp;
+    if (!fused_plan(times, n, d, kernel_mul, kernel_num, &fp)) return GDA_E_UNSUPPORTED;
+    if (fix_sigma > 0.f) return GDA_E_UNSUPPORTED;
+    if (nseg != fp.nseg) return GDA_E_SIZE;
+    if (ld_src % 4 != 0 || ldT % 4 != 0 ||
+        ((uintptr_t)src | (uintptr_t)tgtT | (uintptr_t)rows_src | (uintptr_t)rows_tgt | (uintptr_t)grad_part) % 16 != 0)
+        return GDA_E_UNSUPPORTED;
+    MmdWs ws = carve(workspace, times, n, d);
+    if (workspace_bytes < ws.total) return GDA_E_WORKSPACE;
+    const int64_t m = 2 * n;
+    hipStream_t stream = (hipStream_t)stream_;
+    Rows R = make_rows(src, ld_src, tgtT, ldT, src_idx, tgt_idx, n);
+    const ActCM act{tgtT, ldT, p, 1.f / (1.f - p), seed, step, site};
+    int st;
+    switch (fp.nb) {
+        case 1: st = launch_fused<1>(stream, R, rows_src, rows_tgt, m, d, ws, fp, times, bandwidth, grad_part, &act); break;
+        case 2: st = launch_fused<2>(stream, R, rows_src, rows_tgt, m, d, ws, fp, times, bandwidth, grad_part, &act); break;
+        case 3: st = launch_fused<3>(stream, R, rows_src, rows_tgt, m, d, ws, fp, times, bandwidth, grad_part, &act); break;
+        default: st = launch_fused<4>(stream, R, rows_src, rows_tgt, m, d, ws, fp, times, bandwidth, grad_part, &act); break;
+    }
+    if (st != GDA_OK) return st;
+    GDA_UNLESS_SKIPPED("k_finalize") k_finalize<<<1, TB, 0, stream>>>(ws.kpartial, fp.njb * fp.nseg, times, n, scale, add, loss);
+    GDA_LAUNCH_CHECK();
+    return GDA_OK;
+}
+
+extern "C" int gda_mmd_fused_bwd_act_cm_f32(const float* grad_part, int nseg, int times, int64_t n, int64_t d,
+                                            const float* grad_loss, float scale,
+                                            const int32_t* sel_s_rowptr, const int32_t* sel_s_col, int64_t n_src_rows, float* gsrc,
+                                            const int32_t* sel_t_rowptr, const int32_t* sel_t_col, int64_t n_tgt_rows,
+                                            const float* tgtT, float* gxT, int64_t ldT,
+                                            float p, uint64_t seed, const int64_t* step, uint32_t site,
+                                            const float* mask_src, float p_src, gda_stream_t stream_) {
+    if (!grad_part || !grad_loss || !tgtT || !gxT || !gsrc || !step) return GDA_E_NULL;
+    if (!sel_s_rowptr || !sel_s_col || !sel_t_rowptr || !sel_t_col) return GDA_E_UNSUPPORTED;
+    if (times <= 0 || n <= 0 || d <= 0 || n_src_rows < 0 || n_tgt_rows < 1 || ldT < n_tgt_rows || ldT >= INT32_MAX ||
+        !(p >= 0.f && p < 1.f) || (mask_src && !(p_src >= 0.f && p_src < 1.f)))
+        return GDA_E_SIZE;
+    if (nseg < 1 || nseg > F_NSEG_MAX || d % 4 != 0 || d > 128 || ldT % 4 != 0) return GDA_E_UNSUPPORTED;
+    if (((uintptr_t)grad_part | (uintptr_t)gsrc | (uintptr_t)gxT | (uintptr_t)tgtT | (uintptr_t)mask_src) % 16 != 0) return GDA_E_UNSUPPORTED;
+    if (tgtT == gxT) return GDA_E_ALIAS;
+    hipStream_t stream = (hipStream_t)stream_;
+    const int64_t m = 2 * n;
+    const float cmul = scale / ((float)n * (float)n) / (float)times;
+    const int64_t bs = gda_cdiv(n_src_rows, SC_ROWS), bt = gda_cdiv(ldT, SC_ROWS);
+    const dim3 sg((unsigned)(bs > bt ? bs : bt), 2);
+    const ActCM act{tgtT, ldT, p, 1.f / (1.f - p), seed, step, site};
+    const float ms_s = mask_src ? 1.f / (1.f - p_src) : 1.f;
+#define GDA_SCATTER(NS) GDA_UNLESS_SKIPPED("k_bwd_scatter") k_bwd_scatter_cm<NS><<<sg, SC_TB, 0, stream>>>(grad_part, m, d, d, sel_s_rowptr, sel_s_col, n_src_rows, gsrc, \
+                                                                 sel_t_rowptr, sel_t_col, n_tgt_rows, gxT, act, grad_loss, cmul, mask_src, ms_s)
+    switch (nseg) {
+        case 1: GDA_SCATTER(1); break;
+        case 2: GDA_SCATTER(2); break;
+        case 3: GDA_SCATTER(3); break;
+        case 4: GDA_SCATTER(4); break;
+        case 5: GDA_SCATTER(5); break;
+        case 6: GDA_SCATTER(6); break;
+        case 7: GDA_SCATTER(7); break;
+        default: GDA_SCATTER(8); break;
+    }
+#undef GDA_SCATTER
     GDA_LAUNCH_CHECK();
     return GDA_OK;
 }
diff --git a/pygda_amd/csrc/gda_mmd_fused.inc b/pygda_amd/csrc/gda_mmd_fused.inc
--- a/pygda_amd/csrc/gda_mmd_fused.inc
+++ b/pygda_amd/csrc/gda_mmd_fused.inc
@@ -63,6 +63,157 @@
 #pragma unroll
             for (int e = 0; e < 8; ++e) {
                 v[q][e] = ok ? raw[e] : 0.f;
+                nq = fmaf(v[q][e], v[q][e], nq);
+                mx = fmaxf(mx, fabsf(v[q][e]));
+                csum[e] += v[q][e];
+            }
+            nrm[g][r16 + 16 * q] = nq;
+        }
+#pragma unroll
+        for (int e = 0; e < 8; ++e) {
+            float c = csum[e];
+            c += __shfl_xor(c, 1, 64); c += __shfl_xor(c, 2, 64); c += __shfl_xor(c, 4, 64); c += __shfl_xor(c, 8, 64);
+            csum[e] = c;
+        }
+        if (r16 == 0) {
+            float* pc = part_col + ((int64_t)t * gridDim.x + tau) * D + c8;
+            *reinterpret_cast<float4*>(pc) = make_float4(csum[0], csum[1], csum[2], csum[3]);
+            *reinterpret_cast<float4*>(pc + 4) = make_float4(csum[4], csum[5], csum[6], csum[7]);
+        }
+    }
+    for (int off = 32; off > 0; off >>= 1) mx = fmaxf(mx, __shfl_down(mx, off, 64));
+    if (lane == 0) redm[wave] = mx;
+    __syncthreads();
+    unsigned char* img = images + ((int64_t)t * gridDim.x + tau) * IMG;
+    if (tid < FT) {
+        float nv = 0.f;
+#pragma unroll
+        for (int k = 0; k < NG; ++k) nv += nrm[k][tid];
+        const int64_t row = (int64_t)FT * tau + tid;
+        reinterpret_cast<float*>(img + f_off_n(D))[tid] = row < m ? nv : INFINITY;
+        double s1 = (double)nv;
+        for (int off = 16; off > 0; off >>= 1) s1 += __shfl_down(s1, off, 64);
+        if (tid == 0) {
+            const float M = fmaxf(fmaxf(redm[0], redm[1]), fmaxf(redm[2], redm[3]));
+            int e = 0;
+            if (M > 0.f) { e = 13 - ilogbf(M); e = e < -60 ? -60 : (e > 60 ? 60 : e); }
+            const float xs = ldexpf(1.f, e);
+            xs_sh = xs;
+            reinterpret_cast<float*>(img + f_off_n(D))[F_OFF_XS] = xs;
+            part_s1[(int64_t)t * gridDim.x + tau] = s1;
+            part_max[(int64_t)t * gridDim.x + tau] = M;
+        }
+    }
+    __syncthreads();
+    if (!act) return;
+    const float xs = xs_sh;
+    half8 hi[2], lo[2];
+#pragma unroll
+    for (int q = 0; q < 2; ++q) {
+#pragma unroll
+        for (int e = 0; e < 8; ++e) {
+            const float x = v[q][e] * xs;
+            const _Float16 hh = (_Float16)x;
+            hi[q][e] = hh;
+            lo[q][e] = (_Float16)(x - (float)hh);
+        }
+        *reinterpret_cast<half8*>(img + (r16 + 16 * q) * RS + c8 * 2) = hi[q];
+        *reinterpret_cast<half8*>(img + f_off_rl(D) + (r16 + 16 * q) * RS + c8 * 2) = lo[q];
+    }
+#pragma unroll
+    for (int e = 0; e < 8; ++e) {
+        half2v ph, pl;
+        ph[0] = hi[0][e]; ph[1] = hi[1][e];
+        pl[0] = lo[0][e]; pl[1] = lo[1][e];
+        *reinterpret_cast<half2v*>(img + f_off_th(D) + (c8 + e) * F_TSTRIDE + 4 * r16) = ph;
+        *reinterpret_cast<half2v*>(img + f_off_tl(D) + (c8 + e) * F_TSTRIDE + 4 * r16) = pl;
+    }
+}
+
+struct ActCM {
+    const float* xT; int64_t ldT;
+    float p, scale; uint64_t seed; const int64_t* step; uint32_t site;
+};
+
+template <int NB>
+__global__ void __launch_bounds__(TB)
+k_tile_split_cm(Rows R, ActCM A, int64_t m, double* __restrict__ part_s1, float* __restrict__ part_col, float* __restrict__ part_max,
+                float* __restrict__ rows_src, float* __restrict__ rows_tgt, unsigned char* __restrict__ images) {
+    constexpr int D = 32 * NB, RS = f_rstride(D), IMG = f_img_bytes(D), NG = D / 8;
+    __shared__ float nrm[NG][FT];
+    __shared__ float redm[TB / 64];
+    __shared__ float xs_sh;
+    const int tid = threadIdx.x, lane = tid % 64, wave = tid / 64;
+    int t, tau;
+    {
+        const int ntiles = gridDim.x, first = (int)(R.n / FT), heavy = ntiles - first;
+        const int L = blockIdx.y * ntiles + blockIdx.x, nh = (int)gridDim.y * heavy;
+        if (L < nh) { t = L / heavy; tau = first + L % heavy; }
+        else { t = (L - nh) / first; tau = (L - nh) % first; }
+    }
+    const int r16 = tid & 15, g = tid >> 4, c8 = g * 8;
+    const bool act = c8 < D;
+    float v[2][8];
+    float mx = 0.f;
+    float csum[8] = {0.f, 0.f, 0.f, 0.f, 0.f, 0.f, 0.f, 0.f};
+    if (act) {
+        const float* pivot = R.src + R.src_idx[(int64_t)t * R.n] * R.ld_src + c8;
+        const uint64_t st = (uint64_t)A.step[0];
+        const uint32_t thresh = dropout_thresh(A.p);
+        int64_t gi[2];
+        bool ok[2], tg[2];
+#pragma unroll
+        for (int q = 0; q < 2; ++q) {
+            const int64_t row = (int64_t)FT * tau + r16 + 16 * q;
+            ok[q] = row < m;
+            const int64_t rr = ok[q] ? row : m - 1;
+            tg[q] = rr >= R.n;
+            gi[q] = tg[q] ? R.tgt_idx[(int64_t)t * R.n + (rr - R.n)] : R.src_idx[(int64_t)t * R.n + rr];
+        }
+        const float4 p0 = *reinterpret_cast<const float4*>(pivot), p1 = *reinterpret_cast<const float4*>(pivot + 4);
+        uint32_t rn[2][2][4];
+#pragma unroll
+        for (int q = 0; q < 2; ++q) {
+            if (tg[q]) {
+                const uint64_t quad = (uint64_t)((gi[q] * D + c8) >> 2);
+                dropout_draw(A.seed, st, A.site, quad, rn[q][0]);
+                dropout_draw(A.seed, st, A.site, quad + 1, rn[q][1]);
+            }
+        }
+        float raw8[2][8];
+#pragma unroll
+        for (int q = 0; q < 2; ++q) {
+            if (tg[q]) {
+                const float* col = A.xT + (int64_t)c8 * A.ldT + gi[q];
+#pragma unroll
+                for (int e = 0; e < 8; ++e)
+                    raw8[q][e] = dropout_kept(rn[q][e >> 2][e & 3], thresh) ? col[(int64_t)e * A.ldT] : 0.f;
+            } else {
+                const float* src = R.src + gi[q] * R.ld_src + c8;
+                const float4 a0 = *reinterpret_cast<const float4*>(src), a1 = *reinterpret_cast<const float4*>(src + 4);
+                raw8[q][0] = a0.x; raw8[q][1] = a0.y; raw8[q][2] = a0.z; raw8[q][3] = a0.w;
+                raw8[q][4] = a1.x; raw8[q][5] = a1.y; raw8[q][6] = a1.z; raw8[q][7] = a1.w;
+            }
+        }
+#pragma unroll
+        for (int q = 0; q < 2; ++q) {
+            const int64_t row = (int64_t)FT * tau + r16 + 16 * q;
+            float4 a0 = make_float4(raw8[q][0], raw8[q][1], raw8[q][2], raw8[q][3]);
+            float4 a1 = make_float4(raw8[q][4], raw8[q][5], raw8[q][6], raw8[q][7]);
+            if (tg[q]) {
+                a0 = relu_keep(a0, rn[q][0], thresh, A.scale);
+                a1 = relu_keep(a1, rn[q][1], thresh, A.scale);
+            }
+            if (ok[q]) {
+                float* dst = (row < R.n ? rows_src + ((int64_t)t * R.n + row) * D : rows_tgt + ((int64_t)t * R.n + (row - R.n)) * D) + c8;
+                *reinterpret_cast<float4*>(dst) = a0;
+                *reinterpret_cast<float4*>(dst + 4) = a1;
+            }
+            const float raw[8] = {a0.x - p0.x, a0.y - p0.y, a0.z - p0.z, a0.w - p0.w, a1.x - p1.x, a1.y - p1.y, a1.z - p1.z, a1.w - p1.w};
+            float nq = 0.f;
+#pragma unroll
+            for (int e = 0; e < 8; ++e) {
+                v[q][e] = ok[q] ? raw[e] : 0.f;
                 nq = fmaf(v[q][e], v[q][e], nq);
                 mx = fmaxf(mx, fabsf(v[q][e]));
                 csum[e] += v[q][e];
diff --git a/pygda_amd/models/a2gnn.py b/pygda_amd/models/a2gnn.py
--- a/pygda_amd/models/a2gnn.py
+++ b/pygda_amd/models/a2gnn.py
@@ -68,6 +68,15 @@
             loss = loss.detach()
         return loss, source_logits, source_features
 
+    def _target_features(self, net, h0_t, target_data, tb):
+        if not getattr(self, "_mmd_act_cm", False):
+            return net.feat_bottleneck_from(h0_t, target_data.edge_index, tb, self.t_pnums)
+        from ..ops import ColMajor, PreActCM, dropout_state
+        pre = net.feat_bottleneck_from(h0_t, target_data.edge_index, tb, self.t_pnums, preact_out=True)
+        if not isinstance(pre, ColMajor):
+            return pre
+        return PreActCM(pre, net.dropout if net.training else 0.0, dropout_state.generator(pre.t.device))
+
     def _target_branch(self, target_data, fork, h0_t=None):
         net = self.a2gnn
         tb = None if self.mode == 'node' else target_data.batch
@@ -81,10 +90,10 @@
             if self.compute_target_logits and fork:
                 ready = torch.cuda.Event()
                 ready.record()
-                target_features = net.feat_bottleneck_from(h0_t, target_data.edge_index, tb, self.t_pnums)
+                target_features = self._target_features(net, h0_t, target_data, tb)
                 pending = self._target_logits_async(net, target_data, h0_t, after=ready)
                 return h0_t, pending, target_features
-            target_features = net.feat_bottleneck_from(h0_t, target_data.edge_index, tb, self.t_pnums)
+            target_features = self._target_features(net, h0_t, target_data, tb)
         return h0_t, pending, target_features
 
     def _domain_loss(self, loss, source_features, target_features, alpha):
@@ -146,9 +155,16 @@
         from .. import ops as _ops
         sinks = (type(self) is A2GNN and not self.adv and self.mode == 'node' and source_data.x.is_cuda
                  and getattr(source_data, "n_id", None) is not None and getattr(target_data, "n_id", None) is not None)
-        with (_ops.grad_sinks() if sinks else _null()):
-            loss, source_logits, source_features, target_features, h0_t, pending, (sb, tb) = \
-                self._branches(source_data, target_data)
+        from .. import distributed
+        self._mmd_act_cm = (_ops.MMD_ACT_CM and type(self) is A2GNN and not self.adv and self.mode == 'node'
+                            and source_data.x.is_cuda and getattr(source_data, "n_id", None) is None
+                            and getattr(target_data, "n_id", None) is None and not distributed.active())
+        try:
+            with (_ops.grad_sinks() if sinks else _null()):
+                loss, source_logits, source_features, target_features, h0_t, pending, (sb, tb) = \
+                    self._branches(source_data, target_data)
+        finally:
+            self._mmd_act_cm = False
         net = self.a2gnn
         loss = self._domain_loss(loss, source_features, target_features, alpha)
         if pending is not None:
diff --git a/pygda_amd/ops.py b/pygda_amd/ops.py
--- a/pygda_amd/ops.py
+++ b/pygda_amd/ops.py
@@ -784,8 +784,11 @@
 class _MMD(torch.autograd.Function):
     @staticmethod
     def forward(ctx, src, tgt, src_idx, tgt_idx, times, n, kernel_mul, kernel_num, fix_sigma, sel=None, scale=1.0,
-                add=None):
+                add=None, act_cm=None):
         ctx.sel, ctx.scale, ctx.has_add = sel, float(scale), add is not None
+        ctx.act_cm = act_cm
+        if act_cm is not None:
+            return _mmd_forward_act_cm(ctx, src, tgt, src_idx, tgt_idx, times, n, kernel_mul, kernel_num, scale, add)
         ctx.sinks = (sink_of(src), sink_of(tgt))
         src, tgt = _f32c(src, "source_feat"), _f32c(tgt, "target_feat")
         d = src.size(1)
@@ -849,6 +852,8 @@
 
     @staticmethod
     def backward(ctx, gl):
+        if ctx.act_cm is not None:
+            return _mmd_backward_act_cm(ctx, gl)
         if ctx.one_pass:
             return _MMD._backward_one_pass(ctx, gl)
         src, tgt, src_idx, tgt_idx, bw, l2 = ctx.saved_tensors
@@ -919,6 +924,85 @@
 _MMD._backward_one_pass = staticmethod(_mmd_backward_one_pass)
 
 
+MMD_ACT_CM = True
+
+
+class PreActCM:
+    __slots__ = ("pre", "p", "gen")
+
+    def __init__(self, pre, p, gen):
+        self.pre, self.p, self.gen = pre, float(p), tuple(gen)
+
+    shape = property(lambda self: self.pre.shape)
+    device = property(lambda self: self.pre.t.device)
+    is_cuda = property(lambda self: self.pre.t.is_cuda)
+    dtype = property(lambda self: self.pre.t.dtype)
+
+    def size(self, k=None):
+        return self.pre.size(k)
+
+    def compose(self):
+        return _ReluDropoutT.apply(self.pre.t, self.pre.n, self.p, self.gen)
+
+
+def mmd_act_cm_ok(times, n, d, sel, ptrs=(), lds=(), fix_sigma=None, kernel_mul=2.0, kernel_num=5):
+    if not MMD_ACT_CM or fix_sigma or sel is None or len(sel) < 4 or any(s is None for s in sel[:4]):
+        return False
+    if d not in (32, 64, 96, 128) or any(int(a) % 16 for a in ptrs) or any(int(l) % 4 for l in lds):
+        return False
+    if mmd_chunked_plan(times, n, d, kernel_mul, kernel_num) is not None:
+        return False
+    return 1 <= mmd_one_pass_segments(times, n, d, kernel_mul, kernel_num) <= 8
+
+
+def _mmd_forward_act_cm(ctx, src, xT, src_idx, tgt_idx, times, n, kernel_mul, kernel_num, scale, add):
+    rows_t_total, p, seed, step, site = ctx.act_cm
+    ctx.sinks = (sink_of(src), None)
+    src = _f32c(src, "source_feat")
+    d, dev, m = src.size(1), src.device, 2 * n
+    ctx.feat_rows = (src.size(0), int(rows_t_total))
+    idx_s, idx_t = src_idx.contiguous(), tgt_idx.contiguous()
+    nseg = mmd_one_pass_segments(times, n, d, kernel_mul, kernel_num)
+    rows_s = torch.empty(times * n, d, dtype=torch.float32, device=dev)
+    rows_t = torch.empty(times * n, d, dtype=torch.float32, device=dev)
+    loss = torch.empty(1, dtype=torch.float32, device=dev)
+    bw = torch.empty(times, dtype=torch.float32, device=dev)
+    addc = None if add is None else add.detach().to(torch.float32).reshape(1).contiguous()
+    part = torch.empty(times, nseg, m, d, dtype=torch.float32, device=dev)
+    ws, _ = _lib.scratch("gda_mmd_workspace_bytes", dev, "mmd", times, n, d)
+    with profiler.region("mmd_fwd", 4, 0, times * 3 * 4 * m * m * d):
+        _lib.call("gda_mmd_fused_fwd_act_cm_f32", src, d, xT, xT.size(1), int(rows_t_total), d, idx_s, idx_t, times, n,
+                  float(kernel_mul), int(kernel_num), 0.0, float(scale), addc, rows_s, rows_t, loss, bw, part, nseg,
+                  float(p), seed, step, site, ws, ws.numel(), _lib.stream())
+    ctx.one_pass, ctx.ldp = nseg, d
+    ctx.save_for_backward(part, xT)
+    ctx.cfg = (times, n, d, float(kernel_mul), int(kernel_num))
+    return loss.reshape(())
+
+
+def _mmd_backward_act_cm(ctx, gl):
+    part, xT = ctx.saved_tensors
+    times, n, d, _, _ = ctx.cfg
+    _, p, seed, step, site = ctx.act_cm
+    dev = part.device
+    glc = gl.reshape(1).to(torch.float32).contiguous()
+    s_rp, s_ci, t_rp, t_ci = ctx.sel[:4]
+    ks = ctx.sinks[0]
+    if not (ks is not None and ctx.needs_input_grad[0] and ks.buf.shape == (ctx.feat_rows[0], d)
+            and ks.buf.data_ptr() % 16 == 0 and ks.y.data_ptr() % 16 == 0):
+        ks = None
+    gs = ks.buf if ks is not None else torch.empty(ctx.feat_rows[0], d, dtype=torch.float32, device=dev)
+    gxT = torch.empty_like(xT)
+    with profiler.region("mmd_bwd", 1, 0, 0):
+        _lib.call("gda_mmd_fused_bwd_act_cm_f32", part, ctx.one_pass, times, n, d, glc, ctx.scale, s_rp, s_ci,
+                  ctx.feat_rows[0], gs, t_rp, t_ci, ctx.feat_rows[1], xT, gxT, xT.size(1), float(p), seed, step, site,
+                  ks.y if ks is not None else None, ks.p if ks is not None else 0.0, _lib.stream())
+    if ks is not None:
+        ks.written = True
+    return (gs if ctx.needs_input_grad[0] else None, gxT if ctx.needs_input_grad[1] else None) + (None,) * 9 + \
+        (gl if ctx.has_add else None, None)
+
+
 class _PinnedRing:
 
     def __init__(self, slots=4):
@@ -1053,6 +1137,17 @@
             raise RuntimeError("source and target samples must both be [times, sampling_num]")
         times, n = src_idx.shape
         src_idx, tgt_idx = src_idx.contiguous(), tgt_idx.contiguous()
+    if isinstance(target_feat, PreActCM):
+        pre, xT = target_feat, target_feat.pre.t
+        if src_idx is not None and source_feat.is_cuda and xT.dtype == torch.float32 and xT.is_contiguous():
+            source_feat = _f32c(source_feat, "source_feat")
+            if (xT.size(0) == source_feat.size(1)
+                    and mmd_act_cm_ok(times, n, source_feat.size(1), sel, (source_feat.data_ptr(), xT.data_ptr()),
+                                      (xT.size(1),), fix_sigma, kernel_mul, kernel_num)
+                    and mmd_one_pass_ok(source_feat.device)):
+                return _MMD.apply(source_feat, xT, src_idx, tgt_idx, int(times), int(n), kernel_mul, kernel_num,
+                                  fix_sigma, sel, scale, add, (pre.pre.n, pre.p, *pre.gen))
+        target_feat = pre.compose()
     return _MMD.apply(source_feat, target_feat, src_idx, tgt_idx, int(times), int(n), kernel_mul,
                       kernel_num, fix_sigma, sel, scale, add)
 
@@ -1421,11 +1516,11 @@
 class _ReluDropoutT(torch.autograd.Function):
 
     @staticmethod
-    def forward(ctx, xT, n, p):
+    def forward(ctx, xT, n, p, gen=None):
         d, n_pad = xT.shape
         y = torch.empty(n, d, dtype=torch.float32, device=xT.device)
-        _lib.call("gda_relu_dropout_fwd_cm_f32", xT, n_pad, y, n, d, float(p), *dropout_state.generator(xT.device),
-                  _lib.stream())
+        _lib.call("gda_relu_dropout_fwd_cm_f32", xT, n_pad, y, n, d, float(p),
+                  *(dropout_state.generator(xT.device) if gen is None else gen), _lib.stream())
         ctx.save_for_backward(y)
         ctx.p, ctx.n_pad = float(p), n_pad
         return y
@@ -1433,7 +1528,7 @@
     @staticmethod
     def backward(ctx, gy):
         (y,) = ctx.saved_tensors
-        return _relu_dropout_t_backward(y, gy, ctx.p, ctx.n_pad), None, None
+        return _relu_dropout_t_backward(y, gy, ctx.p, ctx.n_pad), None, None, None
 
 
 def _relu_dropout_t_backward(y, gy, p, n_pad):
```

Measured after the change: 3.645 billion (median of 6 runs). 3.5% higher.
